# alibaba/TorchEasyRec

Measured on AMD Instinct MI355X. Metric: samples/sec DLRM-Criteo (examples/dlrm_criteo.config) training, batch 65536 global, higher is better.
Workload: dtype f32; 1 GPU; dlrm_criteo: 26 tables x dim 16 (204.2M rows, fp32), fused sparse adagrad + dense Adam, ids uniform; global_batch=65536, per_rank_batch=65536, parallelism=single GPU, all tables local (table-wise on one rank), row_layout=interleaved

## Files before the change

include/tzrec_hip.h:

```cpp
#ifndef TZREC_HIP_H_
#define TZREC_HIP_H_

#include <stddef.h>
#include <stdint.h>

#ifdef __cplusplus
extern "C" {
#endif

#define TZR_DT_F32 0
#define TZR_DT_F16 1

#define TZR_OK 0
#define TZR_ERR_INVALID (-1)
#define TZR_ERR_LAUNCH (-2)
#define TZR_ERR_WORKSPACE (-3)
#define TZR_ERR_UNSUPPORTED (-4)

#define TZR_MAX_DST 8
#define TZR_MAX_FEAT_DST 4

#define TZR_POOL_SUM 0
#define TZR_POOL_MEAN 1

// ... 442 lines not shown

#define TZR_DISTILL_MAX_PAIRS 8
#define TZR_DISTILL_MAX_W 1024
typedef struct TzrDistillLoss {
  int64_t B;
  int32_t P, C, cosine, pad_;
  int32_t W[TZR_DISTILL_MAX_PAIRS];
  uint64_t light[TZR_DISTILL_MAX_PAIRS];
  int64_t light_stride[TZR_DISTILL_MAX_PAIRS];
  uint64_t booster[TZR_DISTILL_MAX_PAIRS];
  int64_t booster_stride[TZR_DISTILL_MAX_PAIRS];
  uint64_t logits_light;
  uint64_t logits_booster;
  uint64_t w;
  uint64_t loss;
  uint64_t scale;
  uint64_t grad_sim[TZR_DISTILL_MAX_PAIRS];
  uint64_t grad_hint;
  uint64_t dlight[TZR_DISTILL_MAX_PAIRS];
  int64_t dlight_stride[TZR_DISTILL_MAX_PAIRS];
  uint64_t dlogits_light;
  uint64_t ws;
  uint64_t ws_bytes;
} TzrDistillLoss;
size_t tzr_distill_loss_workspace(const TzrDistillLoss* h_dst);
int tzr_distill_loss_fwd(const TzrDistillLoss* h_dst, void* stream);
int tzr_distill_loss_bwd(const TzrDistillLoss* h_dst, void* stream);

int tzr_skinny_linear_fwd(const float* d_x, int64_t x_stride, const float* d_w, int64_t w_stride, const float* d_bias,
                          int64_t B, int K, int n_out, float* d_y, int64_t y_stride, void* stream);
size_t tzr_skinny_linear_bwd_workspace(int64_t B, int K, int n_out);
int tzr_skinny_linear_bwd(const float* d_grad_y, int64_t grad_y_stride, const float* d_x, int64_t x_stride,
                          const float* d_w, int64_t w_stride, int64_t B, int K, int n_out, float* d_grad_x,
                          int64_t grad_x_stride, float* d_grad_wb, void* ws, size_t ws_bytes, void* stream);
int tzr_skinny_linear_bwd_parts(const float* d_grad_y, int64_t grad_y_stride, const float* d_x, int64_t x_stride,
                                const float* d_w, int64_t w_stride, int64_t B, int K, int n_out, float* d_grad_x,
                                int64_t grad_x_stride, void* ws, size_t ws_bytes, int* out_G, int* out_P, void* stream);

int tzr_linear_bwd_relu_supported(int K, int H);
size_t tzr_linear_bwd_relu_workspace(int64_t N, int H);
int tzr_linear_bwd_relu(const float* d_grad_in, int64_t grad_in_stride, const float* d_w, int64_t w_stride,
                        const float* d_y, int64_t y_stride, int64_t N, int K, int H, float* d_grad_out,
                        int64_t grad_out_stride, float* d_colsum, void* ws, size_t ws_bytes, void* stream);

int tzr_linear_rows_supported(int K, int H);
int tzr_linear_rows(const float* d_in, int64_t in_stride, const float* d_w, int64_t w_stride, int w_out_major,
                    const float* d_bias, const float* d_rowvec, int64_t rowvec_stride, const int32_t* d_row_index, int relu,
                    int64_t N, int K, int H, float* d_out, int64_t out_stride, void* stream);
int tzr_linear_rows_wgrad_supported(int H, int K);
size_t tzr_linear_rows_wgrad_workspace(int64_t N, int H, int K);
int tzr_linear_rows_wgrad(const float* d_g, int64_t g_stride, const float* d_x, int64_t x_stride, int64_t N, int H, int K,
                          float* d_dw, int64_t dw_stride, int accumulate, void* ws, size_t ws_bytes, void* stream);

#define TZR_ADAM_MAX_TENSORS 32
typedef struct TzrAdamTensor {
  uint64_t param, grad, exp_avg, exp_avg_sq;
  uint64_t state;
  int64_t numel;
} TzrAdamTensor;

int tzr_dense_adam(const TzrAdamTensor* h_tensors, int n_tensors, const float* d_lr, float lr,
                   float beta1, float beta2, float eps, float weight_decay, void* stream);

#define TZR_ADAM_FUSED_STATE 40
#define TZR_ADAM_SRC_TENSOR 0
#define TZR_ADAM_SRC_ROWS 1
#define TZR_ADAM_SRC_WGRAD 2
typedef struct TzrAdamSource {
  int32_t kind, G, P, col;
  uint64_t parts;
  uint64_t reserved;
} TzrAdamSource;
typedef struct TzrWgradParts { uint64_t opaque[24]; } TzrWgradParts;
int tzr_dense_adam_fused(const TzrAdamTensor* h_tensors, const TzrAdamSource* h_sources, int n_tensors,
                         const TzrWgradParts* h_wgrad, const float* d_lr, float lr, float beta1, float beta2, float eps,
                         float weight_decay, void* stream);
typedef struct TzrPackedW1 {
  uint64_t param;
  uint64_t fwd_packed, bwd_packed;
} TzrPackedW1;
int tzr_dense_adam_fused_w1(const TzrAdamTensor* h_tensors, const TzrAdamSource* h_sources, int n_tensors,
                            const TzrWgradParts* h_wgrad, const float* d_lr, float lr, float beta1, float beta2, float eps,
                            float weight_decay, const TzrPackedW1* h_w1, void* stream);
#define TZR_DENSE_OPT_SGD 0
#define TZR_DENSE_OPT_ADAGRAD 1
#define TZR_DENSE_OPT_ADAM 2
#define TZR_DENSE_OPT_ADAMW 3
#define TZR_DENSE_OPT_ADADELTA 4
#define TZR_DENSE_OPT_RMSPROP 5
#define TZR_DENSE_OPT_MAX_GROUPS 8
#define TZR_DENSE_OPT_NESTEROV 1
typedef struct TzrDenseOptTensor {
  uint64_t param, grad, state0, state1, state;
  int64_t numel;
  int32_t group, reserved;
} TzrDenseOptTensor;
typedef struct TzrDenseOptGroup {
  int32_t kind, flags;
  uint64_t d_lr;
  float lr, weight_decay, eps, hp0, hp1, reserved;
} TzrDenseOptGroup;
int tzr_dense_optim_fused(const TzrDenseOptTensor* h_tensors, const TzrAdamSource* h_sources, int n_tensors,
                          const TzrDenseOptGroup* h_groups, int n_groups, const TzrWgradParts* h_wgrad, void* stream);
int tzr_mlp2_bwd_parts(const float* d_dhb, int64_t dhb_stride, const float* d_hb, int64_t hb_stride, const float* d_ha,
                       int64_t ha_stride, const float* d_x, int64_t x_stride, int64_t B, int K0, int H1, int H2,
                       const float* d_Wb, void* ws, size_t ws_bytes, int* out_G, int* out_P, void* stream);
int tzr_dot_interaction_top_wgrad_parts(const float* d_dense, int64_t dense_stride, const float* d_sparse, int64_t sparse_stride,
                                        int F, int D, int64_t B, const float* d_g1, int64_t g1_stride, int H, const float* d_scale,
                                        void* d_ws, int64_t ws_bytes, TzrWgradParts* h_out, void* stream);


#define TZR_ZCH_EMPTY INT64_MAX
#define TZR_ZCH_TOMB (INT64_MAX - 1)

typedef struct TzrZchModule {
  int64_t* keys;
  int32_t* rows;
  int64_t* counts;
  int64_t* last_iter;
  int64_t capacity;
  int64_t zch_size;
  int64_t reserved[2];
} TzrZchModule;

int tzr_zch_remap(const TzrZchModule* d_modules, const int32_t* d_key_module, int n_keys,
                  const int64_t* d_values, const int64_t* d_offsets, int64_t B, int uniform_bag_len,
                  int64_t n_values, int64_t iter, int profile, int64_t* d_out_values,
                  int64_t* d_candidates, void* stream);

int tzr_zch_remap_ring(const TzrZchModule* d_modules, const int32_t* d_key_module, int n_keys,
                       const int64_t* d_values, int64_t B, int uniform_bag_len, int64_t n_values,
                       const int64_t* d_iter, int profile, int64_t* d_out_values, const int32_t* d_key_cand,
                       int n_cand_keys, int64_t* d_cand_ring, int64_t ring_slots, void* stream);

int tzr_zch_build(const TzrZchModule* h_module, const int64_t* d_ids, const int32_t* d_rows,
                  int64_t n, void* stream);

int tzr_zch_update(const TzrZchModule* h_module, const int64_t* d_old_ids, const int64_t* d_new_ids,
                   const int32_t* d_rows, int64_t n, void* stream);

int tzr_zch_select_hist(const TzrZchModule* h_module, const int64_t* d_row_ids, const int64_t* d_new_ids,
                        const int64_t* d_new_cnt, int64_t n_new, int64_t cur_iter, int policy,
                        double decay_exponent, int field, int shift, int bits, uint64_t t1, int t2,
                        uint64_t t3, uint64_t* d_bins, void* stream);
int tzr_zch_select_mark(const TzrZchModule* h_module, const int64_t* d_row_ids, const int64_t* d_new_ids,
                        const int64_t* d_new_cnt, int64_t n_new, int64_t cur_iter, int policy,
                        double decay_exponent, int drop_none, uint64_t t1, int t2, uint64_t t3,
                        uint8_t* d_row_kept, uint8_t* d_new_kept, void* stream);

size_t tzr_mlp_workspace(void);
int tzr_mlp2_fwd(const float* d_x, int64_t x_stride, int64_t B, int K0, const float* d_Wa, const float* d_ba, int H1,
                 const float* d_Wb, const float* d_bb, int H2, float* d_ha, int64_t ha_stride, float* d_hb,
                 int64_t hb_stride, void* stream);
int tzr_mlp2_bwd(const float* d_dhb, int64_t dhb_stride, const float* d_hb, int64_t hb_stride, const float* d_ha,
                 int64_t ha_stride, const float* d_x, int64_t x_stride, int64_t B, int K0, int H1, int H2,
                 const float* d_Wb, float* d_dWa, float* d_dba, float* d_dWb, float* d_dbb, void* ws, size_t ws_bytes,
                 void* stream);
int tzr_mlp_tail(const float* d_y1, int64_t y1_stride, const void* d_labels, int labels_itemsize, int labels_are_float,
                 int64_t B, int H1, const float* d_W2, const float* d_b2, int H2, const float* d_w3, const float* d_b3,
                 float* d_logits, float* d_g1, int64_t g1_stride, float* d_dW2, float* d_db2, float* d_dw3,
                 float* d_scalars, float* d_db1, void* ws, size_t ws_bytes, void* stream);


int tzr_jagged_to_padded_dense(const float* d_values, int64_t values_stride,
                               const int64_t* d_offsets, int64_t B, int64_t max_len, int dim,
                               float padding_value, float* d_out, void* stream);
int tzr_padded_dense_to_jagged(const float* d_dense, const int64_t* d_offsets, int64_t B,
                               int64_t max_len, int dim, float* d_values, int64_t values_stride,
                               void* stream);

int tzr_segment_reduce_fwd(const float* d_values, int64_t values_stride, const int64_t* d_offsets,
                           int64_t S, int dim, int mode, float* d_out, int64_t out_stride,
                           void* stream);
int tzr_segment_reduce_bwd(const float* d_grad_out, int64_t grad_out_stride,
                           const int64_t* d_offsets, int64_t S, int dim, int mode,
                           float* d_grad_values, int64_t grad_values_stride, void* stream);

int tzr_jagged_segment_ids(const int64_t* d_offsets, int64_t B, int64_t N, int32_t* d_seg, void* stream);
int tzr_din_assemble_fwd(const float* d_kv, int64_t kv_stride, const float* d_q, int64_t q_stride,
                         const int32_t* d_seg, int64_t B, int64_t N, int D, float* d_X, int64_t x_stride,
                         void* stream);
int tzr_din_assemble_bwd(const float* d_dX, int64_t x_stride, const float* d_kv, int64_t kv_stride,
                         const float* d_q, int64_t q_stride, const int32_t* d_seg, const int64_t* d_offsets,
                         int64_t B, int64_t N, int D, float* d_dkv, int64_t dkv_stride, int accumulate_dkv,
                         float* d_dq, int64_t dq_stride, void* stream);
int tzr_din_assemble2_fwd(const float* d_kv, int64_t kv_stride, const float* d_q, int64_t q_stride, const int32_t* d_seg, int64_t B,
                          int64_t N, int D, float* d_X, int64_t x_stride, void* stream);
int tzr_din_assemble2_bwd(const float* d_dX, int64_t x_stride, const float* d_kv, int64_t kv_stride, const float* d_q,
                          int64_t q_stride, const int32_t* d_seg, const int64_t* d_offsets, int64_t B, int64_t N, int D,
                          float* d_dkv, int64_t dkv_stride, int accumulate_dkv, const float* d_dq_add, int64_t dq_add_stride,
                          float* d_dq, int64_t dq_stride, void* stream);
int tzr_din_attn_fwd(const float* d_h, int64_t h_stride, int H, const float* d_w, const float* d_bias,
                     const float* d_kv, int64_t kv_stride, int D, const int64_t* d_offsets, int64_t B,
                     int64_t max_len, float* d_out, int64_t out_stride, float* d_p, void* stream);
int tzr_din_attn_bwd(const float* d_grad_out, int64_t grad_out_stride, const float* d_p, const float* d_kv,
                     int64_t kv_stride, int D, const int64_t* d_offsets, int64_t B, int64_t max_len, float* d_ds,
                     float* d_dkv, int64_t dkv_stride, void* stream);

int tzr_jagged_dot_attn_fwd(const float* d_kv, int64_t kv_stride, const float* d_q, int64_t q_stride, int D,
                            const int64_t* d_offsets, int64_t B, int64_t N, int64_t max_len, float* d_out,
                            int64_t out_stride, float* d_p, void* stream);
int tzr_jagged_dot_attn_bwd(const float* d_grad_out, int64_t grad_out_stride, const float* d_p, const float* d_kv,
                            int64_t kv_stride, const float* d_q, int64_t q_stride, int D, const int64_t* d_offsets,
                            int64_t B, int64_t N, int64_t max_len, float* d_dkv, int64_t dkv_stride, float* d_dq,
                            int64_t dq_stride, void* stream);
int tzr_jagged_pool_fwd(const float* d_kv, int64_t kv_stride, int D, const int64_t* d_offsets, int64_t B, int64_t N,
                        int64_t max_len, int mode, float* d_out, int64_t out_stride, void* stream);
int tzr_jagged_pool_bwd(const float* d_grad_out, int64_t grad_out_stride, int D, const int64_t* d_offsets, int64_t B,
                        int64_t N, int64_t max_len, int mode, float* d_dkv, int64_t dkv_stride, void* stream);

int tzr_cross_fwd(const float* d_x, int64_t x_stride, const float* const* h_w, const float* const* h_b, int L, int64_t B, int D,
                  float* d_y, int64_t y_stride, float* d_s, void* stream);
size_t tzr_cross_bwd_workspace(int64_t B, int D, int L);
int tzr_cross_bwd(const float* d_grad_y, int64_t gy_stride, const float* d_x, int64_t x_stride, const float* d_s,
                  const float* const* h_w, const float* const* h_b, int L, int64_t B, int D, float* d_dx, int64_t dx_stride,
                  float* d_dw, float* d_db, void* ws, size_t ws_size, void* stream);

int tzr_cross_v2_fwd(const float* d_x, int64_t x_stride, const float* const* h_u, const float* const* h_v, const float* const* h_c,
                     int L, int64_t B, int D, int R, float* d_y, int64_t y_stride, float* d_xs, float* d_t, void* stream);
size_t tzr_cross_v2_bwd_workspace(int64_t B, int D, int R, int L);
int tzr_cross_v2_bwd(const float* d_grad_y, int64_t gy_stride, const float* d_x, int64_t x_stride, const float* d_xs, const float* d_t,
                     const float* const* h_u, const float* const* h_v, const float* const* h_c, int L, int64_t B, int D, int R,
                     float* d_dx, int64_t dx_stride, float* d_du, float* d_dv, float* d_dc, void* ws, size_t ws_size, void* stream);

int tzr_ln_mask_fwd(const float* const* h_x, const int64_t* h_x_stride, const float* const* h_gamma, const float* const* h_beta,
                    const float* const* h_m, const int64_t* h_m_stride, float* const* h_out, const int64_t* h_out_stride, int n_out,
                    int shared_x, int relu, float eps, int64_t B, int D, float* d_stats, void* stream);
size_t tzr_ln_mask_bwd_workspace(int64_t B, int D, int n_out, int shared_x);
int tzr_ln_mask_bwd(const float* const* h_gout, const int64_t* h_gout_stride, const float* const* h_x, const int64_t* h_x_stride,
                    const float* const* h_gamma, const float* const* h_beta, const float* const* h_m, const int64_t* h_m_stride,
                    const float* d_stats, int n_out, int shared_x, int relu, int64_t B, int D, float* const* h_gx,
                    const int64_t* h_gx_stride, float* const* h_gm, const int64_t* h_gm_stride, float* d_dgamma, float* d_dbeta,
                    void* ws, size_t ws_size, void* stream);

int tzr_cin_fwd(const float* d_x, int64_t x_stride, const float* const* h_w, const float* const* h_c, const int* h_layers, int L,
                int64_t B, int F, int D, float* const* h_xs, float* d_y, int64_t y_stride, void* stream);
size_t tzr_cin_bwd_workspace(int64_t B, int F, int D, const int* h_layers, int L);
int tzr_cin_bwd(const float* d_grad_y, int64_t gy_stride, const float* d_x, int64_t x_stride, const float* const* h_w,
                const int* h_layers, int L, int64_t B, int F, int D, float* const* h_xs, float* d_gx, int64_t gx_stride,
                float* d_dwc, void* ws, size_t ws_size, void* stream);

int tzr_wukong_fm_fwd(const float* d_x, int64_t x_stride, const float* d_w, const float* d_gamma, const float* d_beta, float eps,
                      int64_t B, int F, int D, int k, float* d_out, int64_t out_stride, float* d_stats, void* stream);
size_t tzr_wukong_fm_bwd_workspace(int64_t B, int F, int D, int k);
int tzr_wukong_fm_bwd(const float* d_gout, int64_t gout_stride, const float* d_x, int64_t x_stride, const float* d_w,
                      const float* d_gamma, const float* d_stats, int64_t B, int F, int D, int k, float* d_gx, int64_t gx_stride,
                      float* d_dparams, void* ws, size_t ws_size, void* stream);
int tzr_wukong_mix_fwd(const float* d_x, int64_t x_stride, const float* d_fm, int64_t fm_stride, const float* d_wl, const float* d_wr,
                       const float* d_gamma, const float* d_beta, float eps, int64_t B, int F, int D, int Ff, int Fl, float* d_out,
                       int64_t out_stride, float* d_stats, void* stream);
size_t tzr_wukong_mix_bwd_workspace(int64_t B, int F, int D, int Ff, int Fl);
int tzr_wukong_mix_bwd(const float* d_gout, int64_t gout_stride, const float* d_x, int64_t x_stride, const float* d_fm, int64_t fm_stride,
                       const float* d_wl, const float* d_wr, const float* d_gamma, const float* d_stats, int64_t B, int F, int D, int Ff,
                       int Fl, float* d_gx, int64_t gx_stride, float* d_gfm, int64_t gfm_stride, float* d_dparams, void* ws,
                       size_t ws_size, void* stream);

int tzr_comm_available(const char* librccl_path);
int tzr_comm_version(const char* librccl_path);
int tzr_comm_unique_id(const char* librccl_path, void* out, size_t out_bytes);
int tzr_comm_create(const char* librccl_path, const void* unique_id, size_t id_bytes, int world, int rank,
                    void** out_comm);
int tzr_comm_destroy(void* comm);
int tzr_comm_all_to_all(void* comm, const void* d_send, void* d_recv, int64_t bytes_per_peer, void* stream);
int tzr_comm_all_reduce(void* comm, float* d_buf, int64_t count, int average, void* stream);
int tzr_step_create(void** out_program);
int tzr_step_destroy(void* program);
int tzr_step_add_graph(void* program, void* graph_exec );
int tzr_step_add_all_to_all(void* program, void* comm, const void* d_send, void* d_recv, int64_t bytes_per_peer, int sync);
int tzr_step_add_all_reduce(void* program, void* comm, float* d_buf, int64_t count, int average, int sync);
int tzr_step_add_wait(void* program, int collective_op);
int tzr_step_num_ops(void* program);
int tzr_step_run(void* program, void* stream);


int tzr_quantize_rows_q8f16(const void* d_w, int w_dtype, int64_t w_stride, int64_t rows, int dim,
                            uint8_t* d_out, int64_t* d_first_bad, void* stream);
int tzr_dequantize_rows_q8f16(const uint8_t* d_rows, int64_t rows, int dim, float* d_out,
                              int64_t out_stride, void* stream);


typedef struct TzrDeltaSeg {
  uint32_t* bitmap;
  int64_t rows;
  int32_t key;
  int32_t reserved;
} TzrDeltaSeg;

int tzr_delta_mark(const TzrDeltaSeg* d_segs, int n_segs, const int64_t* d_ids,
                   const int64_t* d_key_offsets, int64_t key_stride, int64_t uniform_len,
                   int64_t n_ids, int64_t* d_oob, void* stream);
size_t tzr_delta_collect_workspace(int64_t rows);
int tzr_delta_count(const uint32_t* d_bitmap, int64_t rows, int64_t* d_total, void* ws,
                    size_t ws_bytes, void* stream);
int tzr_delta_collect(uint32_t* d_bitmap, int64_t rows, int64_t id_base, int clear,
                      int64_t* d_out_ids, int64_t capacity, void* ws, size_t ws_bytes, void* stream);

int tzr_tune(const char* name, int value);


int tzr_dot_interaction_fwd(const float* d_dense, int64_t dense_stride, const float* d_sparse,
                            int64_t sparse_stride, int F, int D, int64_t B, float* d_out,
                            int64_t out_stride, int cat_dense, int cat_sparse, void* stream);
int tzr_dot_interaction_bwd(const float* d_dense, int64_t dense_stride, const float* d_sparse,
                            int64_t sparse_stride, int F, int D, int64_t B,
                            const float* d_grad_out, int64_t grad_out_stride, int cat_dense,
                            int cat_sparse, float* d_grad_dense, int64_t grad_dense_stride,
// ... 65 lines not shown
```

torcheasyrec_amd/_lib.py:

```python
from __future__ import annotations

import ctypes as C
import os
from typing import Optional

import numpy as np
import torch

_HERE = os.path.dirname(os.path.abspath(__file__))
LIB_PATH = os.path.join(_HERE, "libtzrec_hip.so")

TZR_OK = 0
TZR_ERR_INVALID, TZR_ERR_UNSUPPORTED = -1, -4
TZR_MAX_DST = 8
TZR_MAX_FEAT_DST = 4
METRIC_MAX_THRESHOLDS = 4096
POOL_SUM, POOL_MEAN = 0, 1
DT_F32, DT_F16 = 0, 1
FWD_MIXED_DTYPE = 1
OPT_SGD, OPT_ADAGRAD, OPT_ROWWISE_ADAGRAD, OPT_ACCUMULATE, OPT_ADAM = 0, 1, 2, 3, 4
OPT_PARTIAL_ROWWISE_ADAM, OPT_LAMB, OPT_PARTIAL_ROWWISE_LAMB, OPT_LARS_SGD = 5, 6, 7, 8
OPT_ADADELTA, OPT_RMSPROP = 9, 10
ABI_VERSION = 15
WD_NONE, WD_L2, WD_DECOUPLE = 0, 1, 2
# ... 128 lines not shown
        ("ws", C.c_uint64), ("ws_bytes", C.c_uint64),
    ]


assert C.sizeof(TzrCapsule) == 192
LABEL_ATTN_MAX_D, LABEL_ATTN_MAX_K = 256, 8
AMM_MAX_D = 256


class TzrAmmLoss(C.Structure):
    _fields_ = [
        ("B", C.c_int64), ("M", C.c_int64), ("D", C.c_int32), ("cosine", C.c_int32), ("c_u", C.c_float), ("c_i", C.c_float),
        ("ua", C.c_uint64), ("ua_stride", C.c_int64), ("ia", C.c_uint64), ("ia_stride", C.c_int64),
        ("ue", C.c_uint64), ("ue_stride", C.c_int64), ("ie", C.c_uint64), ("ie_stride", C.c_int64), ("w", C.c_uint64),
        ("loss", C.c_uint64), ("rows", C.c_uint64), ("scale", C.c_uint64), ("grad_u", C.c_uint64), ("grad_i", C.c_uint64),
        ("dua", C.c_uint64), ("dua_stride", C.c_int64), ("dia", C.c_uint64), ("dia_stride", C.c_int64),
        ("ws", C.c_uint64), ("ws_bytes", C.c_uint64),
    ]


assert C.sizeof(TzrAmmLoss) == 192
DISTILL_MAX_PAIRS, DISTILL_MAX_W, DISTILL_MAX_C = 8, 1024, 64


class TzrDistillLoss(C.Structure):
    _fields_ = [
        ("B", C.c_int64), ("P", C.c_int32), ("C", C.c_int32), ("cosine", C.c_int32), ("pad_", C.c_int32),
        ("W", C.c_int32 * DISTILL_MAX_PAIRS),
        ("light", C.c_uint64 * DISTILL_MAX_PAIRS), ("light_stride", C.c_int64 * DISTILL_MAX_PAIRS),
        ("booster", C.c_uint64 * DISTILL_MAX_PAIRS), ("booster_stride", C.c_int64 * DISTILL_MAX_PAIRS),
        ("logits_light", C.c_uint64), ("logits_booster", C.c_uint64), ("w", C.c_uint64), ("loss", C.c_uint64), ("scale", C.c_uint64),
        ("grad_sim", C.c_uint64 * DISTILL_MAX_PAIRS), ("grad_hint", C.c_uint64),
        ("dlight", C.c_uint64 * DISTILL_MAX_PAIRS), ("dlight_stride", C.c_int64 * DISTILL_MAX_PAIRS), ("dlogits_light", C.c_uint64),
        ("ws", C.c_uint64), ("ws_bytes", C.c_uint64),
    ]


assert C.sizeof(TzrDistillLoss) == 576


class TzrSparseOptim(C.Structure):
    _fields_ = [
        ("kind", C.c_int32),
        ("weight_decay_mode", C.c_int32),
        ("d_lr", C.c_uint64),
        ("eps", C.c_float),
        ("weight_decay", C.c_float),
        ("max_gradient", C.c_float),
        ("gradient_clipping", C.c_int32),
        ("beta1", C.c_float),
        ("beta2", C.c_float),
        ("d_adam", C.c_uint64),
    ]


class TzrAdamTensor(C.Structure):
    _fields_ = [("param", C.c_uint64), ("grad", C.c_uint64), ("exp_avg", C.c_uint64), ("exp_avg_sq", C.c_uint64),
                ("state", C.c_uint64), ("numel", C.c_int64)]


class TzrAdamSource(C.Structure):
    _fields_ = [("kind", C.c_int32), ("G", C.c_int32), ("P", C.c_int32), ("col", C.c_int32), ("parts", C.c_uint64), ("reserved", C.c_uint64)]


class TzrWgradParts(C.Structure):
    _fields_ = [("opaque", C.c_uint64 * 24)]


class TzrPackedW1(C.Structure):
    _fields_ = [("param", C.c_uint64), ("fwd_packed", C.c_uint64), ("bwd_packed", C.c_uint64)]


ADAM_SRC_TENSOR, ADAM_SRC_ROWS, ADAM_SRC_WGRAD = 0, 1, 2


class TzrDenseOptTensor(C.Structure):
    _fields_ = [("param", C.c_uint64), ("grad", C.c_uint64), ("state0", C.c_uint64), ("state1", C.c_uint64), ("state", C.c_uint64),
                ("numel", C.c_int64), ("group", C.c_int32), ("reserved", C.c_int32)]


class TzrDenseOptGroup(C.Structure):
    _fields_ = [("kind", C.c_int32), ("flags", C.c_int32), ("d_lr", C.c_uint64), ("lr", C.c_float), ("weight_decay", C.c_float),
                ("eps", C.c_float), ("hp0", C.c_float), ("hp1", C.c_float), ("reserved", C.c_float)]


DENSE_OPT_MAX_GROUPS = 8
DENSE_OPT_NESTEROV = 1


class TzrZchModule(C.Structure):
    _fields_ = [("keys", C.c_uint64), ("rows", C.c_uint64), ("counts", C.c_uint64), ("last_iter", C.c_uint64),
                ("capacity", C.c_int64), ("zch_size", C.c_int64), ("reserved", C.c_int64 * 2)]


DELTA_SEG_DT = np.dtype([("bitmap", "<u8"), ("rows", "<i8"), ("key", "<i4"), ("reserved", "<i4")])
assert DELTA_SEG_DT.itemsize == 24

ZCH_EMPTY = (1 << 63) - 1


class TzrError(RuntimeError):
    pass


_lib: Optional[C.CDLL] = None
_backend: Optional[str] = None

_vp, _i64, _i32, _sz = C.c_void_p, C.c_int64, C.c_int, C.c_size_t

_SIGNATURES = {
    "tzr_backend": (C.c_char_p, []),
    "tzr_abi_version": (_i32, []),
    "tzr_tune": (_i32, [C.c_char_p, _i32]),
    "tzr_lengths_to_offsets_workspace": (_sz, [_i64]),
    "tzr_lengths_to_offsets": (_i32, [_vp, _i32, _i64, _vp, _vp, _sz, _vp]),
    "tzr_bounds_check": (_i32, [_vp, _vp, _i32, _vp, _vp, _i64, _i32, _vp, _vp]),
    "tzr_kjt_permute_workspace": (_sz, [_i64, _i64]),
    "tzr_kjt_permute": (_i32, [_vp, _i32, _i32, _i64, _vp, _i32, _vp, _vp, _vp, _vp, _vp, _vp, _vp,
                               _i64, _vp, _sz, _vp]),
    "tzr_block_bucketize_workspace": (_sz, [_i64, _i64, _i32]),
    "tzr_block_bucketize": (_i32, [_vp, _vp, _i32, _i64, _i32, _vp, _vp, _vp, _i64, _vp, _i32, _vp, _vp,
                                   _vp, _vp, _vp, _sz, _vp]),
    "tzr_exchange_bucketize_workspace": (_sz, [_i32, _i64, _i32]),
    "tzr_exchange_bucketize": (_i32, [_vp, _i32, _vp, _vp, _i64, _i32, _i32, _vp, _vp, _vp, _vp, _vp, _sz, _vp]),
    "tzr_exchange_message_stride": (_i64, [_i32, _i64]),
    "tzr_exchange_bucketize_capped": (_i32, [_vp, _i32, _vp, _vp, _i64, _i32, _i32, _vp, _i64, _vp, _vp, _vp, _sz, _vp]),
    "tzr_exchange_pad": (_i32, [_vp, _i32, _i32, _i64, _vp, _vp, _i64, _vp, _vp, _vp]),
    "tzr_exchange_owner_segments": (_i32, [_vp, _i32, _i32, _i64, _vp, _vp, _vp]),
    "tzr_pooled_fwd": (_i32, [_vp, _vp, _i32, _vp, _i32, _vp, _vp, _vp, _i64, C.POINTER(TzrDst),
                              _i32, _i32, _vp]),
    "tzr_pooled_fwd_ex": (_i32, [_vp, _vp, _i32, _vp, _i32, _vp, _vp, _vp, _i64, C.POINTER(TzrDst),
                                 _i32, _i32, _i32, _vp]),
    "tzr_pooled_bwd_workspace": (_sz, [_i64, _i64, _i32, _i32, _i64, _i32]),
    "tzr_pooled_bwd_plan_view": (_i32, [_i64, _i64, _i32, _i32, _i32, _vp]),
    "tzr_pooled_bwd_plan": (_i32, [_vp, _i32, _vp, _i32, _i32, _i64, _i32, _vp, _vp, _i64, _i64, _i64,
                                   _i32, _vp, _sz, _vp]),
    "tzr_pooled_bwd_direct_supported": (_i32, [_i64, _i32, _i32, _i32, _i32]),
    "tzr_pooled_bwd_direct_workspace": (_sz, [_i64, _i32, _i32]),
    "tzr_pooled_bwd_direct": (_i32, [_vp, _i32, _vp, _i32, _i64, _i32, _vp, _vp, _vp, _i64, _i64, _i64, _i32, _i32,
                                     C.POINTER(TzrDst), _i32, C.POINTER(TzrSparseOptim), _vp, _sz, _vp]),
    "tzr_sparse_adam_tick": (_i32, [_vp, C.c_float, C.c_float, _vp]),
    "tzr_dense_rows_update": (_i32, [_vp, _i32, _vp, _i64, _vp, _i32, C.POINTER(TzrSparseOptim), _vp]),
    "tzr_dense_rows_update_clear": (_i32, [_vp, _i32, _vp, _i64, _vp, _i32, C.POINTER(TzrSparseOptim), _vp]),
    "tzr_rows_gather": (_i32, [_vp, _vp, _vp, _i32, _vp, _i64, _vp, _i64, _i32, _vp]),
    "tzr_lookup_grads": (_i32, [_vp, _i32, _vp, _vp, _i64, _i32, _vp, C.POINTER(TzrDst), _i32, _vp,
                                _i64, _i32, _vp]),
    "tzr_pooled_bwd_apply": (_i32, [_vp, _vp, _i32, _i32, _i32, _vp, _vp, _i64, _i64, _i64, _i32, _i32,
                                    C.POINTER(TzrDst), _i32, C.POINTER(TzrSparseOptim), _vp, _sz,
                                    _vp]),
    "tzr_bwd_cells_geometry": (_i32, [_vp, _i32, _vp, _i32, _i64, _i32, _vp, _sz, C.POINTER(C.c_int64)]),
    "tzr_pooled_bwd_cells_plan": (_i32, [_vp, _i32, _vp, _i32, _i32, _vp, _i64, _i64, _vp, _vp, _vp, _sz, _vp]),
    "tzr_pooled_fwd_cells_plan_supported": (_i32, [_i32, _i64]),
    "tzr_pooled_fwd_cells_plan": (_i32, [_vp, _vp, _i32, _vp, _i32, _vp, _i32, _vp, _i32, _vp, _i32, _i32, _vp, _i64, _i64, _vp, _vp, _vp, _sz, _vp]),
    "tzr_pooled_bwd_cells_apply": (_i32, [_vp, _vp, _i32, _i32, _i32, _vp, _i64, _i64, _i32, C.POINTER(TzrDst), _i32,
                                          C.POINTER(TzrSparseOptim), _vp, _vp, _vp, _sz, _vp]),
    "tzr_dense_adam_fused": (_i32, [C.POINTER(TzrAdamTensor), C.POINTER(TzrAdamSource), _i32, C.POINTER(TzrWgradParts), _vp, C.c_float,
                                    C.c_float, C.c_float, C.c_float, C.c_float, _vp]),
    "tzr_dense_adam_fused_w1": (_i32, [C.POINTER(TzrAdamTensor), C.POINTER(TzrAdamSource), _i32, C.POINTER(TzrWgradParts), _vp, C.c_float,
                                       C.c_float, C.c_float, C.c_float, C.c_float, C.POINTER(TzrPackedW1), _vp]),
    "tzr_dense_optim_fused": (_i32, [C.POINTER(TzrDenseOptTensor), C.POINTER(TzrAdamSource), _i32, C.POINTER(TzrDenseOptGroup), _i32,
                                     C.POINTER(TzrWgradParts), _vp]),
    "tzr_mlp2_bwd_parts": (_i32, [_vp, _i64, _vp, _i64, _vp, _i64, _vp, _i64, _i64, _i32, _i32, _i32, _vp, _vp, _sz, C.POINTER(C.c_int),
                                  C.POINTER(C.c_int), _vp]),
    "tzr_dot_interaction_top_wgrad_parts": (_i32, [_vp, _i64, _vp, _i64, _i32, _i32, _i64, _vp, _i64, _i32, _vp, _vp, _i64,
                                                   C.POINTER(TzrWgradParts), _vp]),
    "tzr_dot_interaction_fwd": (_i32, [_vp, _i64, _vp, _i64, _i32, _i32, _i64, _vp, _i64, _i32,
                                       _i32, _vp]),
    "tzr_dot_interaction_bwd": (_i32, [_vp, _i64, _vp, _i64, _i32, _i32, _i64, _vp, _i64, _i32,
                                       _i32, _vp, _i64, _vp, _i64, _vp]),
    "tzr_dot_interaction_top_supported": (_i32, [_i32, _i32, _i32, _i32]),
    "tzr_dot_interaction_top_fwd": (_i32, [_vp, _i64, _vp, _i64, _i32, _i32, _i64, _vp, _i64, _vp, _i32, _i32, _vp, _i64,
                                           _vp, _i64, _vp]),
    "tzr_dot_interaction_top_bwd": (_i32, [_vp, _i64, _vp, _i64, _i32, _i32, _i64, _vp, _i64, _i32, _vp, _i64, _vp, _vp,
                                           _i64, _vp, _i64, _vp]),
    "tzr_ia_top_packed_floats": (_i32, []),
    "tzr_ia_top_pack_w1": (_i32, [_vp, _i64, _i32, _vp, _vp, _vp]),
    "tzr_dot_interaction_top_fwd_packed": (_i32, [_vp, _i64, _vp, _i64, _i32, _i32, _i64, _vp, _i64, _vp, _i32, _i32, _vp, _i64,
                                                  _vp, _i64, _vp, _vp]),
    "tzr_dot_interaction_top_bwd_packed": (_i32, [_vp, _i64, _vp, _i64, _i32, _i32, _i64, _vp, _i64, _i32, _vp, _i64, _vp, _vp,
                                                  _i64, _vp, _i64, _vp, _vp]),
    "tzr_dot_interaction_top_fwd_mlp2": (_i32, [_vp, _i64, _i64, _i32, _vp, _vp, _i32, _vp, _vp, _i32, _vp, _i64, _vp, _i64,
                                                _vp, _i64, _vp, _i64, _i32, _i32, _vp, _i64, _vp, _i32, _i32, _vp, _i64,
                                                _vp, _i64, _vp, _vp]),
    "tzr_dot_interaction_top_bwd_wgrad_parts": (_i32, [_vp, _i64, _vp, _i64, _i32, _i32, _i64, _vp, _i64, _i32, _vp, _i64, _vp, _vp,
                                                       _i64, _vp, _i64, _vp, _vp, _i64, C.POINTER(TzrWgradParts), _vp]),
    "tzr_dot_interaction_top_wgrad_workspace": (_i64, [_i32, _i32, _i32, _i32]),
    "tzr_dot_interaction_top_wgrad": (_i32, [_vp, _i64, _vp, _i64, _i32, _i32, _i64, _vp, _i64, _i32, _vp, _vp, _i64, _vp,
                                             _i64, _vp]),
    "tzr_jagged_to_padded_dense": (_i32, [_vp, _i64, _vp, _i64, _i64, _i32, C.c_float, _vp, _vp]),
    "tzr_padded_dense_to_jagged": (_i32, [_vp, _vp, _i64, _i64, _i32, _vp, _i64, _vp]),
    "tzr_quantize_rows_q8f16": (_i32, [_vp, _i32, _i64, _i64, _i32, _vp, _vp, _vp]),
    "tzr_dequantize_rows_q8f16": (_i32, [_vp, _i64, _i32, _vp, _i64, _vp]),
    "tzr_segment_reduce_fwd": (_i32, [_vp, _i64, _vp, _i64, _i32, _i32, _vp, _i64, _vp]),
    "tzr_segment_reduce_bwd": (_i32, [_vp, _i64, _vp, _i64, _i32, _i32, _vp, _i64, _vp]),
    "tzr_jagged_segment_ids": (_i32, [_vp, _i64, _i64, _vp, _vp]),
    "tzr_din_assemble_fwd": (_i32, [_vp, _i64, _vp, _i64, _vp, _i64, _i64, _i32, _vp, _i64, _vp]),
    "tzr_din_assemble_bwd": (_i32, [_vp, _i64, _vp, _i64, _vp, _i64, _vp, _vp, _i64, _i64, _i32, _vp, _i64, _i32, _vp, _i64, _vp]),
    "tzr_din_assemble2_fwd": (_i32, [_vp, _i64, _vp, _i64, _vp, _i64, _i64, _i32, _vp, _i64, _vp]),
    "tzr_din_assemble2_bwd": (_i32, [_vp, _i64, _vp, _i64, _vp, _i64, _vp, _vp, _i64, _i64, _i32, _vp, _i64, _i32, _vp, _i64, _vp, _i64, _vp]),
    "tzr_din_attn_fwd": (_i32, [_vp, _i64, _i32, _vp, _vp, _vp, _i64, _i32, _vp, _i64, _i64, _vp, _i64, _vp, _vp]),
    "tzr_din_attn_bwd": (_i32, [_vp, _i64, _vp, _vp, _i64, _i32, _vp, _i64, _i64, _vp, _vp, _i64, _vp]),
    "tzr_jagged_dot_attn_fwd": (_i32, [_vp, _i64, _vp, _i64, _i32, _vp, _i64, _i64, _i64, _vp, _i64, _vp, _vp]),
    "tzr_jagged_dot_attn_bwd": (_i32, [_vp, _i64, _vp, _vp, _i64, _vp, _i64, _i32, _vp, _i64, _i64, _i64, _vp, _i64, _vp, _i64, _vp]),
    "tzr_jagged_pool_fwd": (_i32, [_vp, _i64, _i32, _vp, _i64, _i64, _i64, _i32, _vp, _i64, _vp]),
    "tzr_jagged_pool_bwd": (_i32, [_vp, _i64, _i32, _vp, _i64, _i64, _i64, _i32, _vp, _i64, _vp]),
    "tzr_cross_fwd": (_i32, [_vp, _i64, _vp, _vp, _i32, _i64, _i32, _vp, _i64, _vp, _vp]),
    "tzr_cross_bwd_workspace": (_sz, [_i64, _i32, _i32]),
    "tzr_cross_bwd": (_i32, [_vp, _i64, _vp, _i64, _vp, _vp, _vp, _i32, _i64, _i32, _vp, _i64, _vp, _vp, _vp, _sz, _vp]),
    "tzr_cross_v2_fwd": (_i32, [_vp, _i64, _vp, _vp, _vp, _i32, _i64, _i32, _i32, _vp, _i64, _vp, _vp, _vp]),
    "tzr_cross_v2_bwd_workspace": (_sz, [_i64, _i32, _i32, _i32]),
    "tzr_cross_v2_bwd": (_i32, [_vp, _i64, _vp, _i64, _vp, _vp, _vp, _vp, _vp, _i32, _i64, _i32, _i32, _vp, _i64, _vp, _vp, _vp, _vp, _sz,
                                _vp]),
    "tzr_cin_fwd": (_i32, [_vp, _i64, _vp, _vp, _vp, _i32, _i64, _i32, _i32, _vp, _vp, _i64, _vp]),
    "tzr_cin_bwd_workspace": (_sz, [_i64, _i32, _i32, _vp, _i32]),
    "tzr_cin_bwd": (_i32, [_vp, _i64, _vp, _i64, _vp, _vp, _i32, _i64, _i32, _i32, _vp, _vp, _i64, _vp, _vp, _sz, _vp]),
    "tzr_ln_mask_fwd": (_i32, [_vp, _vp, _vp, _vp, _vp, _vp, _vp, _vp, _i32, _i32, _i32, C.c_float, _i64, _i32, _vp, _vp]),
    "tzr_ln_mask_bwd_workspace": (_sz, [_i64, _i32, _i32, _i32]),
    "tzr_ln_mask_bwd": (_i32, [_vp, _vp, _vp, _vp, _vp, _vp, _vp, _vp, _vp, _i32, _i32, _i32, _i64, _i32, _vp, _vp, _vp, _vp, _vp, _vp,
                               _vp, _sz, _vp]),
    "tzr_wukong_fm_fwd": (_i32, [_vp, _i64, _vp, _vp, _vp, C.c_float, _i64, _i32, _i32, _i32, _vp, _i64, _vp, _vp]),
    "tzr_wukong_fm_bwd_workspace": (_sz, [_i64, _i32, _i32, _i32]),
    "tzr_wukong_fm_bwd": (_i32, [_vp, _i64, _vp, _i64, _vp, _vp, _vp, _i64, _i32, _i32, _i32, _vp, _i64, _vp, _vp, _sz, _vp]),
    "tzr_wukong_mix_fwd": (_i32, [_vp, _i64, _vp, _i64, _vp, _vp, _vp, _vp, C.c_float, _i64, _i32, _i32, _i32, _i32, _vp, _i64, _vp, _vp]),
    "tzr_wukong_mix_bwd_workspace": (_sz, [_i64, _i32, _i32, _i32, _i32]),
    "tzr_wukong_mix_bwd": (_i32, [_vp, _i64, _vp, _i64, _vp, _i64, _vp, _vp, _vp, _vp, _i64, _i32, _i32, _i32, _i32, _vp, _i64, _vp, _i64,
                                  _vp, _vp, _sz, _vp]),
    "tzr_comm_available": (_i32, [C.c_char_p]),
    "tzr_comm_version": (_i32, [C.c_char_p]),
    "tzr_comm_unique_id": (_i32, [C.c_char_p, _vp, _sz]),
    "tzr_comm_create": (_i32, [C.c_char_p, _vp, _sz, _i32, _i32, C.POINTER(C.c_void_p)]),
    "tzr_comm_destroy": (_i32, [_vp]),
    "tzr_comm_all_to_all": (_i32, [_vp, _vp, _vp, _i64, _vp]),
    "tzr_comm_all_reduce": (_i32, [_vp, _vp, _i64, _i32, _vp]),
    "tzr_step_create": (_i32, [C.POINTER(C.c_void_p)]),
    "tzr_step_destroy": (_i32, [_vp]),
    "tzr_step_add_graph": (_i32, [_vp, _vp]),
    "tzr_step_add_all_to_all": (_i32, [_vp, _vp, _vp, _vp, _i64, _i32]),
    "tzr_step_add_all_reduce": (_i32, [_vp, _vp, _vp, _i64, _i32, _i32]),
    "tzr_step_add_wait": (_i32, [_vp, _i32]),
    "tzr_step_num_ops": (_i32, [_vp]),
    "tzr_step_run": (_i32, [_vp, _vp]),
    "tzr_bce_logits_workspace": (_sz, [_i64]),
    "tzr_bce_logits": (_i32, [_vp, _vp, _i32, _i32, _vp, _i64, _vp, _vp, _vp, _sz, _vp]),
    "tzr_loss_pointwise_workspace": (_sz, [_i64]),
    "tzr_loss_pointwise": (_i32, [_i32, C.c_float, C.c_float, _vp, _vp, _i32, _i32, _vp, _vp, _i32, _i32, C.c_float, C.c_float,
                                  C.c_float, _i64, _vp, _vp, _vp, _vp, _sz, _vp]),
    "tzr_softmax_ce_workspace": (_sz, [_i64, _i32]),
    "tzr_softmax_ce": (_i32, [_vp, _i64, _i32, _vp, _i32, _i32, C.c_float, _vp, _vp, _i32, _i32, C.c_float, C.c_float, C.c_float,
                              _i64, _vp, _vp, _vp, _vp, _vp, _sz, _vp]),
    "tzr_jrc_loss_workspace": (_sz, [_i64]),
    "tzr_jrc_loss": (_i32, [_vp, _vp, _i32, _i32, _vp, _vp, C.c_float, _vp, _vp, _i32, _i32, C.c_float, C.c_float, C.c_float,
                            _i64, _vp, _vp, _vp, _vp, _sz, _vp]),
    "tzr_relu_bwd_colsum_workspace": (_sz, [_i64, _i32]),
    "tzr_relu_bwd_colsum": (_i32, [_vp, _i64, _vp, _i64, _i64, _i32, _vp, _i64, _vp, _vp, _sz, _vp]),
    "tzr_relu_bwd_colsum_parts": (_i32, [_vp, _i64, _vp, _i64, _i64, _i32, _vp, _i64, _vp, _sz, _vp, _vp]),
    "tzr_head_bwd_workspace": (_sz, [_i64, _i32]),
    "tzr_head_bwd": (_i32, [_vp, _i64, _vp, _i64, _vp, _i64, _i32, _vp, _i64, _vp, _vp, _sz, _vp]),
    "tzr_head_bwd_relu_workspace": (_sz, [_i64, _i32]),
    "tzr_head_bwd_relu": (_i32, [_vp, _i64, _vp, _i64, _vp, _i64, _i32, _vp, _i64, _vp, _vp, _sz, _vp]),
    "tzr_moe_mix_fwd": (_i32, [_vp, _vp]),
    "tzr_moe_mix_bwd": (_i32, [_vp, _vp]),
    "tzr_cgc_mix_fwd": (_i32, [_vp, _vp]),
    "tzr_cgc_mix_bwd": (_i32, [_vp, _vp]),
    "tzr_gate_scale_fwd": (_i32, [_vp, _vp]),
    "tzr_gate_scale_bwd_workspace": (_sz, [_i64, _i32, _i32]),
    "tzr_gate_scale_bwd": (_i32, [_vp, _vp]),
    "tzr_relation_chain_fwd": (_i32, [_vp, _vp]),
    "tzr_relation_chain_bwd_workspace": (_sz, [_vp]),
    "tzr_relation_chain_bwd": (_i32, [_vp, _vp]),
    "tzr_match_softmax_workspace": (_sz, [_vp]),
    "tzr_match_softmax_fwd": (_i32, [_vp, _vp]),
    "tzr_match_softmax_bwd": (_i32, [_vp, _vp]),
    "tzr_capsule_workspace": (_sz, [_vp]),
    "tzr_capsule_fwd": (_i32, [_vp, _vp]),
    "tzr_capsule_bwd": (_i32, [_vp, _vp]),
    "tzr_label_attn_fwd": (_i32, [_vp, _i64, _vp, _i64, _vp, _i64, _i32, _i32, C.c_float, _vp, _i64, _vp, _vp]),
    "tzr_label_attn_bwd": (_i32, [_vp, _i64, _vp, _i64, _vp, _i64, _vp, _vp, _i64, _i32, _i32, C.c_float, _vp, _i64, _vp, _i64, _vp]),
    "tzr_amm_loss_workspace": (_sz, [_vp]),
    "tzr_amm_loss_fwd": (_i32, [_vp, _vp]),
    "tzr_amm_loss_bwd": (_i32, [_vp, _vp]),
    "tzr_distill_loss_workspace": (_sz, [_vp]),
    "tzr_distill_loss_fwd": (_i32, [_vp, _vp]),
    "tzr_distill_loss_bwd": (_i32, [_vp, _vp]),
    "tzr_skinny_linear_fwd": (_i32, [_vp, _i64, _vp, _i64, _vp, _i64, _i32, _i32, _vp, _i64, _vp]),
    "tzr_skinny_linear_bwd_workspace": (_sz, [_i64, _i32, _i32]),
    "tzr_skinny_linear_bwd": (_i32, [_vp, _i64, _vp, _i64, _vp, _i64, _i64, _i32, _i32, _vp, _i64, _vp, _vp, _sz, _vp]),
    "tzr_skinny_linear_bwd_parts": (_i32, [_vp, _i64, _vp, _i64, _vp, _i64, _i64, _i32, _i32, _vp, _i64, _vp, _sz, _vp, _vp, _vp]),
    "tzr_linear_rows_supported": (_i32, [_i32, _i32]),
    "tzr_linear_rows": (_i32, [_vp, _i64, _vp, _i64, _i32, _vp, _vp, _i64, _vp, _i32, _i64, _i32, _i32, _vp, _i64, _vp]),
    "tzr_linear_rows_wgrad_supported": (_i32, [_i32, _i32]),
    "tzr_linear_rows_wgrad_workspace": (_sz, [_i64, _i32, _i32]),
    "tzr_linear_rows_wgrad": (_i32, [_vp, _i64, _vp, _i64, _i64, _i32, _i32, _vp, _i64, _i32, _vp, _sz, _vp]),
    "tzr_linear_bwd_relu_supported": (_i32, [_i32, _i32]),
    "tzr_linear_bwd_relu_workspace": (_sz, [_i64, _i32]),
    "tzr_linear_bwd_relu": (_i32, [_vp, _i64, _vp, _i64, _vp, _i64, _i64, _i32, _i32, _vp, _i64, _vp, _vp, _sz, _vp]),
    "tzr_mlp_workspace": (_sz, []),
    "tzr_mlp2_fwd": (_i32, [_vp, _i64, _i64, _i32, _vp, _vp, _i32, _vp, _vp, _i32, _vp, _i64, _vp, _i64, _vp]),
    "tzr_mlp2_bwd": (_i32, [_vp, _i64, _vp, _i64, _vp, _i64, _vp, _i64, _i64, _i32, _i32, _i32, _vp, _vp, _vp, _vp, _vp,
                            _vp, _sz, _vp]),
    "tzr_mlp_tail": (_i32, [_vp, _i64, _vp, _i32, _i32, _i64, _i32, _vp, _vp, _i32, _vp, _vp, _vp, _vp, _i64, _vp, _vp, _vp,
                            _vp, _vp, _vp, _sz, _vp]),
    "tzr_dense_adam": (_i32, [_vp, _i32, _vp, C.c_float, C.c_float, C.c_float, C.c_float, C.c_float, _vp]),
    "tzr_zch_remap": (_i32, [_vp, _vp, _i32, _vp, _vp, _i64, _i32, _i64, _i64, _i32, _vp, _vp, _vp]),
    "tzr_zch_remap_ring": (_i32, [_vp, _vp, _i32, _vp, _i64, _i32, _i64, _vp, _i32, _vp, _vp, _i32, _vp, _i64, _vp]),
    "tzr_zch_build": (_i32, [_vp, _vp, _vp, _i64, _vp]),
    "tzr_zch_update": (_i32, [_vp, _vp, _vp, _vp, _i64, _vp]),
# ... 210 lines not shown
```

torcheasyrec_amd/csrc/mlp2_fwd16_body.h:

```cpp
#pragma once
#include "tzr_common.h"

#define MM_TS 16
#define MT_H1 64
#define MT_P1 (MT_H1 + 4)

typedef float mm_f32x4 __attribute__((ext_vector_type(4)));

#define MB_H1 64
#define MB_H2 16
#define MB_PX 20

__device__ __forceinline__ void mb_fwd16_tiles(
    const float* __restrict__ x, int64_t xs, int64_t B, int K0, const float* __restrict__ Wa, const float* __restrict__ ba,
    const float* __restrict__ Wb, const float* __restrict__ bb, float* __restrict__ ha, int64_t has, float* __restrict__ hb,
    int64_t hbs, float* T1, int lane, int64_t t0, int64_t step) {
  const int r = lane & 15, q = lane >> 4;
  float Wfa[4][4], Wfb[16], bav[4];
#pragma unroll
  for (int hbk = 0; hbk < 4; ++hbk) {
#pragma unroll
    for (int ks = 0; ks < 4; ++ks) {
      const int k = 4 * ks + q;
      const float w = Wa[(16 * hbk + r) * K0 + (k < K0 ? k : 0)];
      Wfa[hbk][ks] = k < K0 ? w : 0.f;
    }
    bav[hbk] = ba ? ba[16 * hbk + r] : 0.f;
  }
#pragma unroll
  for (int i = 0; i < 4; ++i) {
    const float4 v = tzr_ld4(Wb + r * MB_H1 + 16 * q + 4 * i);
    Wfb[4 * i] = v.x; Wfb[4 * i + 1] = v.y; Wfb[4 * i + 2] = v.z; Wfb[4 * i + 3] = v.w;
  }
  const float bbv = bb ? bb[r] : 0.f;
  const int64_t tiles = (B + MM_TS - 1) / MM_TS;
  for (int64_t t = t0; t < tiles; t += step) {
    const int64_t b0 = t * MM_TS;
    float xa[4];
    {
      const int64_t b = b0 + r < B ? b0 + r : B - 1;
#pragma unroll
      for (int ks = 0; ks < 4; ++ks) {
        const int k = 4 * ks + q;
        const float v = x[b * xs + (k < K0 ? k : 0)];
        xa[ks] = (k < K0 && b0 + r < B) ? v : 0.f;
      }
    }
    mm_f32x4 acc[4];
#pragma unroll
    for (int hbk = 0; hbk < 4; ++hbk) acc[hbk] = mm_f32x4{0.f, 0.f, 0.f, 0.f};
#pragma unroll
    for (int ks = 0; ks < 4; ++ks)
#pragma unroll
      for (int hbk = 0; hbk < 4; ++hbk) acc[hbk] = __builtin_amdgcn_mfma_f32_16x16x4f32(xa[ks], Wfa[hbk][ks], acc[hbk], 0, 0, 0);
#pragma unroll
    for (int hbk = 0; hbk < 4; ++hbk)
#pragma unroll
      for (int j = 0; j < 4; ++j) T1[(4 * q + j) * MT_P1 + 16 * hbk + r] = fmaxf(acc[hbk][j] + bav[hbk], 0.f);
    __builtin_amdgcn_wave_barrier();
    mm_f32x4 acc2 = {0.f, 0.f, 0.f, 0.f};
#pragma unroll
    for (int i = 0; i < 4; ++i) {
      const int e = lane + TZR_WAVE * i, row = e >> 4, c4 = e & 15;
      if (b0 + row < B) tzr_st4(ha + (b0 + row) * has + 4 * c4, tzr_ld4(T1 + row * MT_P1 + 4 * c4));
      const float4 av = tzr_ld4(T1 + r * MT_P1 + 16 * q + 4 * i);
      acc2 = __builtin_amdgcn_mfma_f32_16x16x4f32(av.x, Wfb[4 * i], acc2, 0, 0, 0);
      acc2 = __builtin_amdgcn_mfma_f32_16x16x4f32(av.y, Wfb[4 * i + 1], acc2, 0, 0, 0);
      acc2 = __builtin_amdgcn_mfma_f32_16x16x4f32(av.z, Wfb[4 * i + 2], acc2, 0, 0, 0);
      acc2 = __builtin_amdgcn_mfma_f32_16x16x4f32(av.w, Wfb[4 * i + 3], acc2, 0, 0, 0);
    }
#pragma unroll
    for (int j = 0; j < 4; ++j)
      if (b0 + 4 * q + j < B) hb[(b0 + 4 * q + j) * hbs + r] = fmaxf(acc2[j] + bbv, 0.f);
    __builtin_amdgcn_wave_barrier();
  }
}

static inline bool mb_fwd16_fits(int K0, int H1, int H2, const float* d_Wb, const float* d_ha, int64_t ha_stride) {
  return K0 > 0 && K0 <= 16 && H1 == MB_H1 && H2 == MB_H2 && !(ha_stride & 3) && !(reinterpret_cast<uintptr_t>(d_ha) & 15) &&
         !(reinterpret_cast<uintptr_t>(d_Wb) & 15);
}
```

torcheasyrec_amd/csrc/pooled_bwd_cells.hip:

```cpp
#include <tzr_gfx950.h>

#include "pooled_fwd_u1.h"

#include <algorithm>
#include <cstring>
#include <vector>

#ifdef IT_PROF
#define CELLS_PROF_WGS 4096
__device__ uint64_t g_cells_prof[CELLS_PROF_WGS * 16];
#define CELLS_MARK(i) do { if (blockIdx.x < CELLS_PROF_WGS && threadIdx.x == 0) g_cells_prof[blockIdx.x * 16 + (i)] = wall_clock64(); } while (0)
#define CELLS_NOTE(i, v) do { if (blockIdx.x < CELLS_PROF_WGS && threadIdx.x == 0) g_cells_prof[blockIdx.x * 16 + (i)] = (uint64_t)(v); } while (0)
#define BWD_PROF_MARK(i) do { if ((i) == 2 && blockIdx.x < CELLS_PROF_WGS && (threadIdx.x & (TZR_WAVE - 1)) == 0) \
    g_cells_prof[blockIdx.x * 16 + 4 + threadIdx.x / TZR_WAVE] = wall_clock64(); } while (0)
extern "C" int tzr_cells_prof_dump(uint64_t* h_out, int n_wg) {
  (void)hipDeviceSynchronize();
  return hipMemcpyFromSymbol(h_out, HIP_SYMBOL(g_cells_prof), (size_t)std::min(n_wg, CELLS_PROF_WGS) * 16 * sizeof(uint64_t)) == hipSuccess ? 0 : -1;
}
#else
#define CELLS_MARK(i)
#define CELLS_NOTE(i, v)
#endif

#include "pooled_bwd_apply.h"
#include "pooled_bwd_cells.h"
#include "pooled_bwd_sort.h"

namespace {

struct HostGeo {
  BwdCellsGeo g;
  std::vector<BwdCellChunk> chunks;
  std::vector<BwdCellUnit> units;
  std::vector<uint32_t> fstart;
  std::vector<int32_t> fkey, fbo;
  std::vector<uint16_t> bnd;
};

inline int64_t align256(int64_t x) { return (x + 255) & ~int64_t(255); }

inline void bucket_params_host(int64_t rows, int* nb, uint64_t* mult) {
  if (rows <= BWD_NB) {
    *nb = rows < 1 ? 1 : (int)rows;
    *mult = 1ull << 32;
  } else {
    *nb = BWD_NB;
    *mult = ((uint64_t)BWD_NB << 32) / (uint64_t)rows;
  }
}

int build_geometry(const TzrTable* tabs, int T, const TzrFeature* feats, int F, int64_t B, int max_dim, HostGeo& H) {
  if (T <= 0 || F <= 0 || B <= 0 || max_dim <= 0 || max_dim > BWD_MAXDIM || (max_dim & 3)) return TZR_ERR_INVALID;
  H.fstart.assign(F + 1, 0);
  H.fkey.assign(F, 0);
  H.fbo.assign(F, 0);
  std::vector<int> seen(F, 0);
  for (int f = 0; f < F; ++f) {
    const TzrFeature& ft = feats[f];
    if (ft.order < 0 || ft.order >= F || seen[ft.order]) return TZR_ERR_INVALID;
    seen[ft.order] = 1;
    H.fstart[ft.order] = ft.table < 0 ? 0u : (uint32_t)B;
    H.fkey[ft.order] = ft.key;
    H.fbo[ft.order] = f;
  }
  {
    uint64_t run = 0;
    for (int o = 0; o < F; ++o) {
      const uint32_t n = H.fstart[o];
      H.fstart[o] = (uint32_t)run;
      run += n;
    }
    if (run >= (1ull << 32)) return TZR_ERR_UNSUPPORTED;
    H.fstart[F] = (uint32_t)run;
  }
  const int64_t N = H.fstart[F];
  if (N == 0) return TZR_ERR_UNSUPPORTED;
  const int ch = bwd_pick_ch(N);
  int64_t n_chunks = 0;
  std::vector<int64_t> cfirst(T + 1, 0), nt(T, 0);
  for (int t = 0; t < T; ++t) {
    const TzrTable& tb = tabs[t];
    if (tb.n_feats < 0 || (tb.n_feats > 0 && (tb.first_order < 0 || tb.first_order + tb.n_feats > F))) return TZR_ERR_INVALID;
    const int64_t n = tb.n_feats > 0 ? (int64_t)H.fstart[tb.first_order + tb.n_feats] - (int64_t)H.fstart[tb.first_order] : 0;
    const int64_t C = (n + ch - 1) / ch;
    if (C > BWD_CELLS_MAXC) return TZR_ERR_UNSUPPORTED;
    if (n > 0 && (tb.rows <= 0 || tb.rows > (1LL << 32))) return TZR_ERR_UNSUPPORTED;
    nt[t] = n;
    cfirst[t] = n_chunks;
    n_chunks += C;
  }
  cfirst[T] = n_chunks;
  if (n_chunks > bwd_max_chunks(N, T, ch)) return TZR_ERR_UNSUPPORTED;

  const int64_t target = BWD_CELLS_TARGET;
  std::vector<int64_t> U(T, 0);
  for (int t = 0; t < T; ++t) {
    if (nt[t] == 0 || tabs[t].rows <= BWD_NB) continue;
    const int64_t per = (target * BWD_NB) / nt[t];
    if (per < 1) return TZR_ERR_UNSUPPORTED;
    U[t] = (BWD_NB + per - 1) / per;
  }

  int64_t n_recs = 0, n_counters = 0;
  for (int t = 0; t < T; ++t) {
    const TzrTable& tb = tabs[t];
    const int64_t C = cfirst[t + 1] - cfirst[t];
    if (C == 0) continue;
    const int64_t ts = H.fstart[tb.first_order], te = H.fstart[tb.first_order + tb.n_feats];
    const int64_t n = te - ts;
    int nb;
    uint64_t mult;
    bucket_params_host(tb.rows, &nb, &mult);
    const int64_t fbase = tb.n_feats == 1 ? (int64_t)H.fkey[tb.first_order] * B : -1;
    const int32_t bnd0 = (int32_t)H.bnd.size();
    BwdCellUnit u;
    std::memset(&u, 0, sizeof(u));
    u.tb = tb;
    u.feat = H.fbo[tb.first_order];
    u.ts = (uint32_t)ts;
    u.rec = u.rec0 = u.counter = -1;
    u.crel0 = 0;
    u.ncell = (int32_t)C;
    if (tb.rows > BWD_NB) {
      const int64_t Ut = U[t];
      for (int64_t j = 0; j <= Ut; ++j) H.bnd.push_back((uint16_t)(j * nb / Ut));
      for (int64_t j = 0; j < Ut; ++j) {
        u.b0 = (int32_t)(j * nb / Ut);
        u.i0 = bnd0 + (int32_t)j;
        u.i1 = u.i0 + 1;
        H.units.push_back(u);
      }
    } else {
      const int64_t e = (n + tb.rows - 1) / tb.rows;
      if (e > target) {
        for (int64_t r = 0; r <= tb.rows; ++r) H.bnd.push_back((uint16_t)r);
        const int64_t m = std::max<int64_t>(1, (target * tb.rows * C) / n);
        const int64_t K = std::min<int64_t>(C, (C + m - 1) / m);
        for (int64_t r = 0; r < tb.rows; ++r) {
          for (int64_t k = 0; k < K; ++k) {
            u.crel0 = (int32_t)(k * C / K);
            u.ncell = (int32_t)((k + 1) * C / K) - u.crel0;
            u.b0 = (int32_t)r;
            u.nrows = 0;
            u.i0 = bnd0 + (int32_t)r;
            u.i1 = u.i0 + 1;
            u.split = K > 1 ? (int32_t)K : 0;
            u.rec = K > 1 ? (int32_t)(n_recs + k) : -1;
            u.rec0 = K > 1 ? (int32_t)n_recs : -1;
            u.counter = K > 1 ? (int32_t)n_counters : -1;
            H.units.push_back(u);
          }
          if (K > 1) {
            n_recs += K;
            n_counters += 1;
          }
        }
      } else {
        const int64_t rpu = std::max<int64_t>(1, (target * tb.rows) / n);
        int32_t g = 0;
        for (int64_t r = 0; r < tb.rows; r += rpu, ++g) {
          H.bnd.push_back((uint16_t)r);
          u.b0 = (int32_t)r;
          u.i0 = bnd0 + g;
          u.i1 = u.i0 + 1;
          H.units.push_back(u);
        }
        H.bnd.push_back((uint16_t)tb.rows);
      }
    }
    const int32_t nbnd = (int32_t)H.bnd.size() - bnd0;
    for (int64_t c = 0; c < C; ++c) {
      BwdCellChunk cd;
      std::memset(&cd, 0, sizeof(cd));
      cd.t = t;
      cd.nb = nb;
      cd.s = ts + c * ch;
// ... 17 lines not shown
  g.max_dim = max_dim;
  g.ch = ch;
  g.n_positions = N;
  g.n_bnd = (int64_t)H.bnd.size();
  if (g.n_bnd * BWD_CELLS_MAXC * 2 > bwd_max_chunks(N, T, ch) * (int64_t)BWD_NB * 4) return TZR_ERR_UNSUPPORTED;
  int64_t off = align256(sizeof(BwdCellsGeo));
  g.off_chunks = off;
  off = align256(off + n_chunks * (int64_t)sizeof(BwdCellChunk));
  g.off_units = off;
  off = align256(off + g.n_units * (int64_t)sizeof(BwdCellUnit));
  g.off_fstart = off;
  off = align256(off + (F + 1) * 4);
  g.off_fkey = off;
  off = align256(off + F * 4);
  g.off_fbo = off;
  off = align256(off + F * 4);
  g.off_bnd = off;
  off = align256(off + g.n_bnd * 2);
  g.off_recs = off;
  off = align256(off + std::max<int64_t>(1, n_recs) * max_dim * 4);
  g.off_rcount = off;
  off = align256(off + std::max<int64_t>(1, n_recs) * 4);
  g.off_counters = off;
  off = align256(off + std::max<int64_t>(1, n_counters) * 4);
  g.off_overflow = off;
  off = align256(off + 4 * (BWD_CELLS_OVF_LIST + 2 * g.n_units));
  g.bytes = off;
  return TZR_OK;
}

}

extern "C" int tzr_bwd_cells_geometry(const TzrTable* h_tables, int n_tables, const TzrFeature* h_feats, int n_feats, int64_t B,
                                      int max_dim, void* h_out, size_t out_bytes, int64_t* out_info8) {
  if (!h_tables || !h_feats || !out_info8) return TZR_ERR_INVALID;
  HostGeo H;
  const int rc = build_geometry(h_tables, n_tables, h_feats, n_feats, B, max_dim, H);
  if (rc != TZR_OK) return rc;
  const BwdCellsGeo& g = H.g;
  out_info8[0] = g.bytes;
  out_info8[1] = g.n_chunks;
  out_info8[2] = g.n_units;
  out_info8[3] = g.n_positions;
  out_info8[4] = g.ch;
  out_info8[5] = g.n_recs;
  out_info8[6] = g.off_overflow;
  out_info8[7] = 0;
  if (!h_out) return TZR_OK;
  if ((int64_t)out_bytes < g.bytes) return TZR_ERR_WORKSPACE;
  char* b = static_cast<char*>(h_out);
  std::memset(b, 0, (size_t)g.bytes);
  std::memcpy(b, &g, sizeof(g));
  std::memcpy(b + g.off_chunks, H.chunks.data(), H.chunks.size() * sizeof(BwdCellChunk));
  std::memcpy(b + g.off_units, H.units.data(), H.units.size() * sizeof(BwdCellUnit));
  std::memcpy(b + g.off_fstart, H.fstart.data(), H.fstart.size() * 4);
  std::memcpy(b + g.off_fkey, H.fkey.data(), H.fkey.size() * 4);
  std::memcpy(b + g.off_fbo, H.fbo.data(), H.fbo.size() * 4);
  std::memcpy(b + g.off_bnd, H.bnd.data(), H.bnd.size() * 2);
  return TZR_OK;
}

struct BwdPartLds {
  BwdRankLds<BWD_NB> L;
  uint2 stage[BWD_CH];
};

__device__ __forceinline__ void bwd_cells_partition_body(const BwdCellsView& V, const TzrTable* __restrict__ tables, const BwdSrcArgs& A,
                                                         uint2* __restrict__ slab, uint16_t* __restrict__ bnd, int ch, unsigned chunk,
                                                         BwdPartLds& PL) {
  auto& L = PL.L;
  auto& stage = PL.stage;
  const BwdCellChunk cd = V.chunks[chunk];
  if (cd.t < 0) return;
  const int n = (int)(cd.e - cd.s);
  const int lane = threadIdx.x & (TZR_WAVE - 1);
  const int wv = threadIdx.x / TZR_WAVE;
  constexpr int kRounds = BWD_CH / BWD_THREADS;
  const int pw = bwd_wave_span(n);
  const int rounds = pw / TZR_WAVE;
  uint32_t kreg[kRounds], sreg[kRounds], dig[kRounds], dest[kRounds];
  uint32_t vmask = 0;
  if (cd.fbase >= 0) {
#pragma unroll
    for (int r = 0; r < kRounds; ++r) {
      const int lp = wv * pw + r * TZR_WAVE + lane;
      const int lc = lp < n ? lp : n - 1;
      const int64_t i = cd.fbase + (cd.s - cd.ts) + lc;
      int64_t id = A.values[i];
      if ((uint64_t)id >= (uint64_t)cd.rows) id = 0;
      kreg[r] = (uint32_t)id;
      sreg[r] = (uint32_t)i;
      dig[r] = bwd_bucket(kreg[r], cd.mult);
      vmask |= (r < rounds && lp < n) ? 1u << r : 0u;
    }
  } else {
    const TzrTable tb = tables[cd.t];
    BwdGeo G;
    G.fstart = V.fstart;
    G.fkey = V.fkey;
    G.tchunk = nullptr;
#pragma unroll
    for (int r = 0; r < kRounds; ++r) {
      const int lp = wv * pw + r * TZR_WAVE + lane;
      kreg[r] = sreg[r] = dig[r] = 0u;
      if (r < rounds && lp < n) {
        vmask |= 1u << r;
        int64_t kk;
        bwd_elem0(G, tb, A, cd.s + lp, &kreg[r], &sreg[r], &kk);
        dig[r] = bwd_bucket(kreg[r], cd.mult);
      }
    }
  }
  bwd_rank_tile<BWD_NB, kRounds>(dig, vmask, rounds, bwd_bits((uint32_t)cd.nb - 1u), L, dest);
#pragma unroll
  for (int r = 0; r < kRounds; ++r)
    if ((vmask >> r) & 1u) stage[dest[r]] = make_uint2(kreg[r], sreg[r]);
  {
    const int col = (int)((cd.s - cd.ts) / (cd.e > cd.s ? (int64_t)ch : 1));
    for (int i = threadIdx.x; i < cd.nbnd; i += BWD_THREADS)
      bnd[(size_t)(cd.bnd0 + i) * BWD_CELLS_MAXC + col] = L.lstart[V.bnd_bucket[cd.bnd0 + i]];
  }
  __syncthreads();
  uint2* out = slab + cd.s;
  for (int i = threadIdx.x; i < n; i += BWD_THREADS) out[i] = stage[i];
}

__global__ __launch_bounds__(BWD_THREADS) void tzr_bwd_cells_partition_kernel(
    BwdCellsView V, const TzrTable* __restrict__ tables, BwdSrcArgs A, uint2* __restrict__ slab, uint16_t* __restrict__ bnd, int ch) {
  __shared__ BwdPartLds PL;
  bwd_cells_partition_body(V, tables, A, slab, bnd, ch, blockIdx.x, PL);
}

static_assert(FWD_THREADS == BWD_THREADS, "one workgroup size for both kinds");
struct FwdPlanArgs {
  const TzrTable* ftables;
  const TzrFeature* ffeats;
  const TzrSlot* slots;
  const int64_t* values;
  int64_t B;
  int32_t n_slots, tile_b;
  uint32_t n_fwd, n_part;
  const TzrTable* btables;
  uint2* slab;
  uint16_t* bnd;
  int32_t ch;
};

#ifndef FWD_PLAN_WAVES
#define FWD_PLAN_WAVES 7
#endif
#ifndef FWD_PLAN_UNROLL
#define FWD_PLAN_UNROLL 4
#endif
union FwdPlanLds {
  Fwd1Lds f;
  BwdPartLds p;
};

__global__ __launch_bounds__(BWD_THREADS) TZR_WAVES_PER_EU(FWD_PLAN_WAVES) void tzr_pooled_fwd_u1_cells_plan_kernel(FwdPlanArgs a, FwdDsts dsts,
                                                                                                          BwdCellsView V, BwdSrcArgs A) {
  __shared__ FwdPlanLds S;
  const uint32_t i = blockIdx.x;
  const bool part = i >= a.n_fwd;
  const uint32_t idx = part ? i - a.n_fwd : i;
  if (part)
    bwd_cells_partition_body(V, a.btables, A, a.slab, a.bnd, a.ch, idx, S.p);
  else
    fwd_u1_body<FWD_PLAN_UNROLL>(a.ftables, a.ffeats, a.slots, a.n_slots, a.values, a.B, a.tile_b, dsts, idx, 0u, S.f);
}

union BwdCellsLds {
  BwdSortLds S;
  BwdUnitLds U;
};

#define BWD_CELLS_SM 264
#define BWD_CELLS_SM_WORDS (2 * BWD_WAVES + BWD_WAVES * TZR_WAVE)
static_assert(BWD_CELLS_SM >= BWD_THREADS + 1, "sm behind the histogram of bwd_cells_next_piece");
static_assert(offsetof(BwdSortLds, pre) == offsetof(BwdSortLds, gstart) + sizeof(unsigned) * (BWD_NB + 1),
              "pre / hb directly behind gstart");
static_assert(offsetof(BwdSortLds, gstart) + sizeof(unsigned) * (BWD_CELLS_SM + BWD_CELLS_SM_WORDS) <= offsetof(BwdSortLds, pk),
              "sm fits in gstart + pre / hb");
static_assert(sizeof(BwdRankLds<BWD_NB>) >= 4096, "red: 4 KB in S.L");

__device__ __forceinline__ uint2 bwd_cells_elem(const uint2* __restrict__ slab, const uint32_t* cpre, const uint32_t* cbase,
                                                int ncell, uint32_t i) {
  int lo = 0;
#pragma unroll
  for (int step = BWD_CELLS_MAXC / 2; step > 0; step >>= 1) {
    const int cand = lo + step;
    if (cand < ncell && cpre[cand] <= i) lo = cand;
  }
  return slab[cbase[lo] + (i - cpre[lo])];
}

template <int FAM>
__device__ __forceinline__ void bwd_cells_combine(const BwdCellUnit& u, const BwdCellsView& V, const BwdOpt& opt, float lr,
                                                  int max_dim, float4 sum, uint32_t count, int lane) {
  const int lg = u.tb.dim >> 2;
  if (lane < lg) bwd_publish4(V.recs + (size_t)u.rec * max_dim + 4 * lane, sum);
  if (lane == 0) tzr_publish_u32(V.rcount + u.rec, count);
  tzr_drain_stores();
  int last = 0;
  if (lane == 0) last = tzr_arrive(V.counters + u.counter) == (uint32_t)(u.split - 1) ? 1 : 0;
  last = __shfl(last, 0, TZR_WAVE);
  if (!last) return;
  if (lane == 0) tzr_publish_u32(V.counters + u.counter, 0u);
  const int gw = TZR_WAVE / lg;
  const int gi = lane / lg, c = lane - gi * lg;
  float4 tot = tzr_zero4();
  uint32_t cnt = 0;
  for (int k0 = 0; k0 < u.split; k0 += gw) {
    const int k = k0 + gi;
    const bool in = gi < gw && k < u.split;
    float4 v = tzr_zero4();
    uint32_t cn = 0;
    if (in) {
      v = bwd_consume4(V.recs + (size_t)(u.rec0 + k) * max_dim + 4 * c);
      cn = tzr_consume_u32(V.rcount + u.rec0 + k);
    }
    const int nk = min(gw, u.split - k0);
    for (int g = 0; g < nk; ++g) {
      const float4 piece = bwd_shfl4(v, g * lg + (lane < lg ? lane : 0));
      if (lane < lg) tot = tzr_add4(tot, piece);
      cnt += (uint32_t)__shfl((int)cn, g * lg, TZR_WAVE);
    }
  }
  if (cnt) bwd_apply_row_wave<FAM>(u.tb, opt, lr, (uint32_t)u.b0, tot, lane);
}

template <bool FAST>
__device__ __forceinline__ float4 bwd_cells_stream_row(
    const BwdCellUnit& u, const BwdCellsView& V, const uint2* __restrict__ slab, const uint32_t* cpre, const uint32_t* cbase,
    int ncell, int n, uint32_t row, const TzrFeature* __restrict__ feats, const float* __restrict__ weights, int64_t B,
    int grad_mode, const TzrDst* sG, float* red, uint32_t* sm, uint32_t* count_out) {
  constexpr int UF = 4;
  const TzrTable& tb = u.tb;
  const int lane = threadIdx.x & (TZR_WAVE - 1);
  const int wv = threadIdx.x / TZR_WAVE;
  const int lg = tb.dim >> 2, gw = TZR_WAVE / lg;
  const int gi = lane / lg, c = lane - gi * lg;
  const bool lane_on = gi < gw;
  const int groups = gw * BWD_WAVES, q = wv * gw + gi;
  const bool single = tb.n_feats == 1;
  const BwdSrc one = bwd_resolve(feats + V.feat_by_order[tb.first_order], sG);
  const float* const fgp = grad_mode == 1 ? reinterpret_cast<const float*>(sG[0].ptr) : one.gp0;
  const int64_t fgs = grad_mode == 1 ? sG[0].stride : one.gs0;
  const uint32_t fkb = grad_mode == 0 ? (uint32_t)feats[V.feat_by_order[tb.first_order]].key * (uint32_t)B : 0u;
  float4 acc = tzr_zero4();
  uint32_t cnt = 0;
  const int trips = (n + groups * UF - 1) / (groups * UF);
  uint2 e[UF];
#pragma unroll
  for (int k = 0; k < UF; ++k) {
    const int i = k * groups + q;
    e[k] = bwd_cells_elem(slab, cpre, cbase, ncell, (uint32_t)(i < n ? i : n - 1));
  }
  for (int j = 0; j < trips; ++j) {
    float4 g[UF];
#pragma unroll
    for (int k = 0; k < UF; ++k) {
      if constexpr (FAST) g[k] = tzr_ldg4(fgp + (int64_t)(e[k].y - fkb) * fgs + 4 * c);
      else g[k] = bwd_lookup_grad(feats, tb, V.feat_by_order, sG, one, single, grad_mode, nullptr, weights, nullptr, B, 1, e[k].y, c);
    }
    uint2 en[UF];
#pragma unroll
    for (int k = 0; k < UF; ++k) {
      const int i = ((j + 1) * UF + k) * groups + q;
      en[k] = bwd_cells_elem(slab, cpre, cbase, ncell, (uint32_t)(i < n ? i : n - 1));
    }
#pragma unroll
    for (int k = 0; k < UF; ++k) {
      const int i = (j * UF + k) * groups + q;
      if (lane_on && i < n && (row == BWD_SENT || e[k].x == row)) {
        acc = tzr_add4(acc, g[k]);
        cnt += 1;
      }
      e[k] = en[k];
    }
  }
  __syncthreads();
  if (lane_on) {
    float* r = red + (size_t)(q * lg + c) * 4;
    r[0] = acc.x; r[1] = acc.y; r[2] = acc.z; r[3] = acc.w;
    if (c == 0) sm[2 * BWD_WAVES + q] = cnt;
  }
  __syncthreads();
  float4 tot = tzr_zero4();
  uint32_t ct = 0;
  if (wv == 0) {
    for (int g2 = 0; g2 < groups; ++g2) {
      if (lane < lg) {
        const float* r = red + (size_t)(g2 * lg + lane) * 4;
        tot = tzr_add4(tot, make_float4(r[0], r[1], r[2], r[3]));
      }
      ct += sm[2 * BWD_WAVES + g2];
    }
  }
  *count_out = ct;
  return tot;
}

template <int FAM>
__device__ __forceinline__ int bwd_cells_next_piece(
    const BwdCellUnit& u, const BwdCellsView& V, const uint2* __restrict__ slab, const uint32_t* cpre, const uint32_t* cbase,
    int ncell, int n, uint32_t& cur, uint32_t khi, const TzrFeature* __restrict__ feats, const float* __restrict__ weights, int64_t B,
    int grad_mode, const BwdOpt& opt, float lr, BwdCellsLds& L, const TzrDst* sG) {
  const TzrTable& tb = u.tb;
  const int lane = threadIdx.x & (TZR_WAVE - 1);
  const int wv = threadIdx.x / TZR_WAVE;
  float* const red = reinterpret_cast<float*>(&L.S.L);
  uint32_t* const hist = L.S.gstart;
  uint32_t* const sm = L.S.gstart + BWD_CELLS_SM;
  constexpr int SB = BWD_THREADS;
  while (cur < khi) {
// ... 203 lines not shown
      const int rounds = pw / TZR_WAVE;
      uint32_t kreg[kRounds], sreg[kRounds];
      uint32_t vmask = 0, kmin = 0xFFFFFFFFu, kmax = 0u;
#pragma unroll
      for (int r = 0; r < kRounds; ++r) {
        const int lp = wv * pw + r * TZR_WAVE + lane;
        const bool in = r < rounds && lp < np;
        kreg[r] = in ? L.S.pk[lp] : 0u;
        sreg[r] = in ? L.S.ps[lp] : 0u;
        if (in) {
          vmask |= 1u << r;
          kmin = min(kmin, kreg[r]);
          kmax = max(kmax, kreg[r]);
        }
      }
      __syncthreads();
      bwd_cells_sort_reduce<FAM, 0, 1, kRounds>(u, V, kreg, sreg, vmask, kmin, kmax, np, ft_dst, feats, weights, B, grad_mode, opt, lr,
                                                 max_dim, L, sG);
      __syncthreads();
    }
  }
  if (threadIdx.x == 0 && tzr_arrive(ov + BWD_CELLS_OVF_DONE) == (uint32_t)BWD_CELLS_WORKERS - 1u) {
    if (len) atomicAdd(ov + BWD_CELLS_OVF_TOTAL, len);
    tzr_publish_u32(ov + BWD_CELLS_OVF_LEN, 0u);
    tzr_publish_u32(ov + BWD_CELLS_OVF_CURSOR, 0u);
    tzr_publish_u32(ov + BWD_CELLS_OVF_DONE, 0u);
    tzr_publish_u32(ov + BWD_CELLS_OVF_EPOCH, tzr_consume_u32(ov + BWD_CELLS_OVF_EPOCH) + 1u);
  }
}

template <int FAM, int FK, int NT>
__device__ __forceinline__ void bwd_cells_apply_body(
    BwdCellsView V, int n_units, const TzrFeature* __restrict__ feats, const float* __restrict__ weights, int64_t B, int grad_mode,
    const BwdGrads& G, const BwdOpt& opt, int max_dim, const uint2* __restrict__ slab, const uint16_t* __restrict__ bnd, int ch) {
  __shared__ BwdCellsLds L;
  __shared__ TzrDst sG[TZR_MAX_DST];
  __shared__ uint32_t xcell[2 * BWD_CELLS_MAXC + 8];
  if (threadIdx.x == 0) {
#pragma unroll
    for (int i = 0; i < TZR_MAX_DST; ++i) sG[i] = G.d[i];
  }
  if ((int)blockIdx.x >= n_units) {
    __syncthreads();
#ifndef CELLS_NO_WORKER
    bwd_cells_worker<FAM>(V, n_units, feats, weights, B, grad_mode, opt, max_dim, slab, bnd, ch, L, sG, xcell);
#endif
    return;
  }
  CELLS_MARK(0);
#ifndef CELLS_NO_PRIO
  tzr_prio_by_slot(blockIdx.x);
  if ((blockIdx.x >> 8) >= 4u) __builtin_amdgcn_s_sleep(64);
#endif
  const BwdCellUnit u = V.units[blockIdx.x];
  const uint32_t epoch = V.overflow[BWD_CELLS_OVF_EPOCH];
  const int lane = threadIdx.x & (TZR_WAVE - 1);
  const int wv = threadIdx.x / TZR_WAVE;
  const int ncell = u.ncell;
  const int ft_dst = feats[u.feat].n_dst;
  uint32_t* const cpre = xcell;
  uint32_t* const cbase = xcell + BWD_CELLS_MAXC + 8;
  const float lr = *opt.lr;
  const int n = bwd_cells_bounds(u, u.i0, u.i1, bnd, ch, cpre, cbase, L.S.wtot);
  CELLS_MARK(1);
  CELLS_NOTE(9, n);
  if (threadIdx.x == 0) {
    if (n > BWD_UMAX) {
      const uint32_t at = atomicAdd(V.overflow + BWD_CELLS_OVF_LEN, 1u);
      tzr_publish_u32(V.overflow + BWD_CELLS_OVF_LIST + at, (uint32_t)blockIdx.x);
      tzr_drain_stores();
    }
    tzr_publish_u32(V.overflow + BWD_CELLS_OVF_LIST + n_units + blockIdx.x, epoch + 1u);
  }
  if (n > BWD_UMAX || n == 0) return;
  constexpr int kRounds = BWD_UMAX / BWD_THREADS;
  const int pw = bwd_wave_span(n);
  const int rounds = pw / TZR_WAVE;
  uint32_t kreg[kRounds], sreg[kRounds];
  uint32_t vmask = 0, kmin = 0xFFFFFFFFu, kmax = 0u;
#pragma unroll
  for (int r = 0; r < kRounds; ++r) {
    const int lp = wv * pw + r * TZR_WAVE + lane;
    const bool in = r < rounds && lp < n;
#ifdef CELLS_EXP_CONTIG
    const uint2 v = slab[cbase[0] + (uint32_t)(lp < n ? lp : n - 1)];
#else
    const uint2 v = bwd_cells_elem(slab, cpre, cbase, ncell, (uint32_t)(lp < n ? lp : n - 1));
#endif
    kreg[r] = in ? v.x : 0u;
    sreg[r] = in ? v.y : 0u;
    if (in) {
      vmask |= 1u << r;
      kmin = min(kmin, v.x);
      kmax = max(kmax, v.x);
    }
  }
  CELLS_MARK(2);
  bwd_cells_sort_reduce<FAM, FK, NT, kRounds>(u, V, kreg, sreg, vmask, kmin, kmax, n, ft_dst, feats, weights, B, grad_mode, opt, lr,
                                               max_dim, L, sG);
  CELLS_MARK(8);
}

#define TZR_CELLS_APPLY_KERNEL(NAME, FAM_, FK_, ATTR)                                                                         \
  __global__ __launch_bounds__(BWD_THREADS) ATTR void NAME(BwdCellsView V, int n_units, const TzrFeature* __restrict__ feats,  \
                                                          const float* __restrict__ weights, int64_t B, int grad_mode,         \
                                                          BwdGrads G, BwdOpt opt, int max_dim, const uint2* __restrict__ slab, \
                                                          const uint16_t* __restrict__ bnd, int ch) {                          \
    bwd_cells_apply_body<FAM_, FK_, 1>(V, n_units, feats, weights, B, grad_mode, G, opt, max_dim, slab, bnd, ch);             \
  }
TZR_CELLS_APPLY_KERNEL(tzr_bwd_cells_apply_adagrad_kernel, BWD_FAM_LEGACY, TZR_OPT_ADAGRAD, TZR_WAVES_PER_EU(7))
TZR_CELLS_APPLY_KERNEL(tzr_bwd_cells_apply_rowwise_kernel, BWD_FAM_LEGACY, TZR_OPT_ROWWISE_ADAGRAD, TZR_WAVES_PER_EU(7))
TZR_CELLS_APPLY_KERNEL(tzr_bwd_cells_apply_sgd_kernel, BWD_FAM_LEGACY, TZR_OPT_SGD, TZR_WAVES_PER_EU(7))
TZR_CELLS_APPLY_KERNEL(tzr_bwd_cells_apply_general_kernel, BWD_FAM_LEGACY, 0, TZR_WAVES_PER_EU(7))
TZR_CELLS_APPLY_KERNEL(tzr_bwd_cells_apply_adam_kernel, BWD_FAM_ADAM, 0, )
TZR_CELLS_APPLY_KERNEL(tzr_bwd_cells_apply_norm_kernel, BWD_FAM_NORM, 0, )
TZR_CELLS_APPLY_KERNEL(tzr_bwd_cells_apply_elem_kernel, BWD_FAM_ELEM, 0, )

static int cells_common(const void* h_geo, void* d_geo, void* ws, size_t ws_bytes, int64_t n_values, int n_feats, int n_tables,
                        int max_dim, BwdCellsGeo* g, BwdCellsView* V, BwdPlan* P) {
  if (!h_geo || !d_geo || (reinterpret_cast<uintptr_t>(d_geo) & 255)) return TZR_ERR_INVALID;
  std::memcpy(g, h_geo, sizeof(BwdCellsGeo));
  if (g->n_feats != n_feats || g->max_dim != max_dim || g->n_chunks <= 0 || g->n_units <= 0) return TZR_ERR_INVALID;
  if (!ws || (reinterpret_cast<uintptr_t>(ws) & 255)) return TZR_ERR_WORKSPACE;
  if (bwd_layout(P, ws, n_values, g->n_positions, n_feats, n_tables, max_dim) > ws_bytes) return TZR_ERR_WORKSPACE;
  if (P->ch != (int)g->ch || g->n_chunks > P->max_chunks) return TZR_ERR_INVALID;
  *V = bwd_cells_view(d_geo, *g);
  return TZR_OK;
}

extern "C" int tzr_pooled_bwd_cells_plan(const TzrTable* d_tables, int n_tables, const TzrFeature* d_feats, int n_feats,
                                         int max_dim, const int64_t* d_values, int64_t n_values, int64_t B, const void* h_geo,
                                         void* d_geo, void* ws, size_t ws_bytes, void* stream) {
  if (!d_tables || !d_feats || n_tables <= 0 || n_feats <= 0 || n_values < 0 || B <= 0) return TZR_ERR_INVALID;
  BwdCellsGeo g;
  BwdCellsView V;
  BwdPlan P;
  const int rc = cells_common(h_geo, d_geo, ws, ws_bytes, n_values, n_feats, n_tables, max_dim, &g, &V, &P);
  if (rc != TZR_OK) return rc;
  if (!d_values) return TZR_ERR_INVALID;
  if (n_values >= (1LL << 32)) return TZR_ERR_UNSUPPORTED;
  BwdSrcArgs A;
  A.feats = d_feats;
  A.values = d_values;
  A.offsets = nullptr;
  A.B = B;
  A.uniform = 1;
  hipLaunchKernelGGL(tzr_bwd_cells_partition_kernel, dim3((unsigned)g.n_chunks), dim3(BWD_THREADS), 0, static_cast<hipStream_t>(stream), V,
                     d_tables, A, P.ks[1], reinterpret_cast<uint16_t*>(P.hist), (int)g.ch);
  TZR_CHECK_LAUNCH();
  return TZR_OK;
}

extern int g_tzr_fwd_tile_b;
int g_tzr_fwd_plan = 1;

extern "C" int tzr_pooled_fwd_cells_plan_supported(int n_slots, int64_t B) {
  return (g_tzr_fwd_plan != 0 && n_slots > 0 && n_slots <= FWD1_SLOTS && B > 0 && (B >= 32768 || g_tzr_fwd_plan == 2)) ? 1 : 0;
}

extern "C" int tzr_pooled_fwd_cells_plan(const TzrTable* d_ftables, const TzrFeature* d_ffeats, int n_ffeats, const TzrSlot* d_slots,
                                         int n_slots, const TzrDst* h_dsts, int n_dst, const TzrTable* d_tables, int n_tables,
                                         const TzrFeature* d_feats, int n_feats, int max_dim, const int64_t* d_values, int64_t n_values,
                                         int64_t B, const void* h_geo, void* d_geo, void* ws, size_t ws_bytes, void* stream) {
  if (!d_ftables || !d_ffeats || !d_slots || !h_dsts || n_ffeats <= 0 || n_slots <= 0 || n_dst <= 0 || n_dst > TZR_MAX_DST ||
      !d_tables || !d_feats || n_tables <= 0 || n_feats <= 0 || n_values < 0 || B <= 0)
    return TZR_ERR_INVALID;
  if (!tzr_pooled_fwd_cells_plan_supported(n_slots, B)) return TZR_ERR_UNSUPPORTED;
  BwdCellsGeo g;
  BwdCellsView V;
  BwdPlan P;
  const int rc = cells_common(h_geo, d_geo, ws, ws_bytes, n_values, n_feats, n_tables, max_dim, &g, &V, &P);
  if (rc != TZR_OK) return rc;
  if (!d_values) return TZR_ERR_INVALID;
  if (n_values >= (1LL << 32)) return TZR_ERR_UNSUPPORTED;
  FwdDsts dsts;
  for (int i = 0; i < TZR_MAX_DST; ++i) {
    dsts.d[i].ptr = 0;
    dsts.d[i].stride = 0;
  }
  for (int i = 0; i < n_dst; ++i) {
    if (!h_dsts[i].ptr || (h_dsts[i].stride & 3) || (h_dsts[i].ptr & 15)) return TZR_ERR_INVALID;
    if (h_dsts[i].stride > 0x7fffffffLL) return TZR_ERR_UNSUPPORTED;
    dsts.d[i] = h_dsts[i];
  }
  BwdSrcArgs A;
  A.feats = d_feats;
  A.values = d_values;
  A.offsets = nullptr;
  A.B = B;
  A.uniform = 1;
  FwdPlanArgs a;
  a.ftables = d_ftables;
  a.ffeats = d_ffeats;
  a.slots = d_slots;
  a.values = d_values;
  a.B = B;
  a.n_slots = n_slots;
  a.tile_b = g_tzr_fwd_tile_b > 0 ? g_tzr_fwd_tile_b : (B >= 32768 ? 64 : (B >= 8192 ? 16 : 8));
  a.n_fwd = (uint32_t)((B + a.tile_b - 1) / a.tile_b);
  a.n_part = (uint32_t)g.n_chunks;
  a.btables = d_tables;
  a.slab = P.ks[1];
  a.bnd = reinterpret_cast<uint16_t*>(P.hist);
  a.ch = (int)g.ch;
  hipLaunchKernelGGL(tzr_pooled_fwd_u1_cells_plan_kernel, dim3(a.n_fwd + a.n_part), dim3(BWD_THREADS), 0, static_cast<hipStream_t>(stream),
                     a, dsts, V, A);
  TZR_CHECK_LAUNCH();
  return TZR_OK;
}

extern "C" int tzr_pooled_bwd_cells_apply(const TzrTable* d_tables, const TzrFeature* d_feats, int n_feats, int n_tables, int max_dim,
                                          const float* d_weights, int64_t n_values, int64_t B, int grad_mode, const TzrDst* h_grads,
                                          int n_dst, const TzrSparseOptim* h_optim, const void* h_geo, void* d_geo, void* ws,
                                          size_t ws_bytes, void* stream) {
  if (!d_tables || !d_feats || !h_grads || !h_optim || n_tables <= 0 || n_feats <= 0 || n_values < 0 || B <= 0 || n_dst <= 0 ||
      n_dst > TZR_MAX_DST || max_dim <= 0 || max_dim > BWD_MAXDIM || (max_dim & 3) || (grad_mode != 0 && grad_mode != 1))
    return TZR_ERR_INVALID;
  BwdOpt opt;
  if (const int rc = bwd_opt_from(h_optim, true, &opt)) return rc;
  BwdCellsGeo g;
  BwdCellsView V;
  BwdPlan P;
  const int rc = cells_common(h_geo, d_geo, ws, ws_bytes, n_values, n_feats, n_tables, max_dim, &g, &V, &P);
  if (rc != TZR_OK) return rc;
  BwdGrads G;
  if (const int rc = bwd_grads_from(h_grads, n_dst, &G)) return rc;
  hipStream_t s = static_cast<hipStream_t>(stream);
  static constexpr decltype(&tzr_bwd_cells_apply_general_kernel) kernels[BWD_VAR_COUNT] = {
      tzr_bwd_cells_apply_general_kernel, tzr_bwd_cells_apply_sgd_kernel,  tzr_bwd_cells_apply_adagrad_kernel,
      tzr_bwd_cells_apply_rowwise_kernel, tzr_bwd_cells_apply_adam_kernel, tzr_bwd_cells_apply_norm_kernel,
      tzr_bwd_cells_apply_elem_kernel};
  hipLaunchKernelGGL(kernels[bwd_variant(opt.kind, !d_weights)], dim3((unsigned)g.n_units + BWD_CELLS_WORKERS),
                     dim3(BWD_THREADS), 0, s, V, (int)g.n_units, d_feats, d_weights, B, grad_mode, G, opt, max_dim,
                     (const uint2*)P.ks[1], (const uint16_t*)reinterpret_cast<uint16_t*>(P.hist), (int)g.ch);
  TZR_CHECK_LAUNCH();
  return TZR_OK;
}
```

torcheasyrec_amd/dense.py:

```python
from __future__ import annotations

import collections
import contextlib
import dataclasses
import os
import weakref
from typing import Iterable, List, Optional, Tuple

import ctypes as C

import torch

from . import _lib


class _BceLogitsFn(torch.autograd.Function):
    @staticmethod
    def forward(ctx, logits, labels, sample_weight):
        x = logits.contiguous().float()
        y = labels.contiguous()
        if y.dtype not in (torch.float32, torch.int32, torch.int64):
            y = y.float()
        loss = torch.empty((), dtype=torch.float32, device=x.device)
        grad = torch.empty_like(x)
# ... 540 lines not shown
    return fwd, bwd


def repack_w1(p: torch.Tensor) -> None:
    e = _packed_entry(p)
    if e is None:
        return
    q = e.ref()
    _lib.check(_lib.lib().tzr_ia_top_pack_w1(_lib.ptr(q.data), q.stride(0), 27, _lib.ptr(e.fwd), _lib.ptr(e.bwd), _lib.stream_ptr(q.device)),
               "tzr_ia_top_pack_w1")
    e.version = q._version


def _fresh_packed_w1(W1: torch.Tensor) -> Optional["_PackedW1"]:
    e = _packed_entry(W1)
    if e is None:
        return None
    if e.version != e.ref()._version:
        repack_w1(W1)
    return e


class _InteractionTopLossFn(torch.autograd.Function):

    @staticmethod
    def forward(ctx, dense, sparse, D, W1, b1, W2, b2, w3, b3, labels):
        B = sparse.shape[0]
        F = sparse.shape[1] // D
        sparse = sparse.contiguous()
        dense = dense.contiguous()
        n = F + 1
        width = n * (n - 1) // 2 + D * n
        H1 = W1.shape[0]
        dev = sparse.device
        y1 = torch.empty(B, H1, dtype=torch.float32, device=dev)
        z = None if _owned_wgrad(B, sparse.shape[1]) else torch.empty(B, width, dtype=torch.float32, device=dev)
        W1_, b1_ = _f32c(W1), _f32c(b1)
        pk = _fresh_packed_w1(W1_) if (n == 27 and D == 16 and H1 == 64) else None
        head, tail = _ia_top_fwd_args(dense, sparse, F, D, W1_, b1_, z, width, y1, pk)
        _lib.check(_lib.lib().tzr_dot_interaction_top_fwd_packed(*head, B, *tail, _lib.stream_ptr(dev)), "tzr_dot_interaction_top_fwd_packed")
        ctx.w1_packed = pk
        logits, g1, dW2, db2, dw3, scal, db1 = _mlp_tail(y1, labels, W2, b2, w3, b3)
        ctx.save_for_backward(dense, sparse, W1_, g1, dW2, db2, dw3, scal, db1)
        ctx.z = z
        ctx.cfg = (F, D)
        ctx.w1_ref = W1
        ctx.mark_non_differentiable(logits)
        ctx.set_materialize_grads(False)
        return scal[1], logits

    @staticmethod
    def backward(ctx, gl, _glogits):
        dense, sparse, W1, g1, dW2, db2, dw3, scal, db1 = ctx.saved_tensors
        F, D = ctx.cfg
        B = sparse.shape[0]
        root = _loss_is_root(gl)
        gl32 = None if root else gl.reshape(1).to(torch.float32)
        gd = gs = None
        if ctx.needs_input_grad[0] or ctx.needs_input_grad[1]:
            gs = torch.empty_like(sparse)
            gd = torch.empty_like(dense)
            _lib.check(_lib.lib().tzr_dot_interaction_top_bwd_packed(
                *_ia_top_bwd_args(dense, sparse, F, D, g1, W1, gl32, gd, gs, ctx.w1_packed), _lib.stream_ptr(sparse.device)),
                "tzr_dot_interaction_top_bwd_packed")
        if not ctx.needs_input_grad[3]:
            dW1 = None
        elif ctx.z is None:
            dW1 = interaction_top_wgrad(dense, sparse, D, g1, gl32, defer_for=(ctx.w1_ref,))
        else:
            dW1 = weight_grad(g1, ctx.z) if root else weight_grad(g1, ctx.z) * gl
        if root:
            return (gd, gs, None, dW1, db1, dW2, db2, dw3, scal[0:1], None)
        outs = torch._foreach_mul([db1, dW2, db2, dw3, scal[0:1]], gl)
        return (gd, gs, None, dW1, *outs, None)


def _ia_top_fwd_args(dense, sparse, F, D, W1_, b1_, z, width, y1, pk) -> Tuple[tuple, tuple]:
    return ((_lib.ptr(dense), dense.stride(0), _lib.ptr(sparse), sparse.stride(0), F, D),
            (_lib.ptr(W1_), W1_.stride(0), _lib.ptr(b1_), W1_.shape[0], 1, _lib.ptr(z), width, _lib.ptr(y1), y1.stride(0),
             _lib.ptr(pk.fwd) if pk is not None else None))


def _ia_top_bwd_args(dense, sparse, F, D, g1, W1, gl32, gd, gs, pk) -> tuple:
    return (_lib.ptr(dense), dense.stride(0), _lib.ptr(sparse), sparse.stride(0), F, D, sparse.shape[0], _lib.ptr(g1), g1.stride(0),
            g1.shape[1], _lib.ptr(W1), W1.stride(0), _lib.ptr(gl32), _lib.ptr(gd), gd.stride(0), _lib.ptr(gs), gs.stride(0),
            _lib.ptr(pk.bwd) if pk is not None else None)


def interaction_top_wgrad(dense: torch.Tensor, sparse: torch.Tensor, D: int, g1: torch.Tensor,
                          scale: Optional[torch.Tensor] = None, defer_for=None) -> torch.Tensor:
    B = sparse.shape[0]
    F = sparse.shape[1] // D
    n = F + 1
    width = n * (n - 1) // 2 + D * n
    H = g1.shape[1]
    if B == 0:
        return torch.zeros(H, width, dtype=torch.float32, device=sparse.device)
    dW = torch.empty(H, width, dtype=torch.float32, device=sparse.device)
    L = _lib.lib()
    ws = _lib.workspace(L.tzr_dot_interaction_top_wgrad_workspace(F, D, 1, H), sparse.device)
    if defer_for is not None and _defer_finish(sparse.device, defer_for):
        blob = _lib.TzrWgradParts()
        _lib.check(L.tzr_dot_interaction_top_wgrad_parts(
            _lib.ptr(dense), dense.stride(0), _lib.ptr(sparse), sparse.stride(0), F, D, B, _lib.ptr(g1), g1.stride(0), H,
            _lib.ptr(scale), _lib.ptr(ws), ws.numel(), C.byref(blob), _lib.stream_ptr(sparse.device)), "tzr_dot_interaction_top_wgrad_parts")
        _defer(dW, "wgrad", (ws, scale), blob, defer_for)
        return dW
    _lib.check(L.tzr_dot_interaction_top_wgrad(
        _lib.ptr(dense), dense.stride(0), _lib.ptr(sparse), sparse.stride(0), F, D, B, _lib.ptr(g1), g1.stride(0), H,
        _lib.ptr(scale), _lib.ptr(dW), dW.stride(0), _lib.ptr(ws), ws.numel(), _lib.stream_ptr(sparse.device)),
        "tzr_dot_interaction_top_wgrad")
    return dW


def interaction_top_fits(dense: torch.Tensor, sparse: torch.Tensor, D: int, first_linear) -> bool:
    if dense is None or dense.dim() != 2:
        return False
    return _ia_top_fits(dense.shape[1], dense.dtype, sparse, D, first_linear)


def _ia_top_fits(dense_width: int, dense_dtype, sparse: torch.Tensor, D: int, first_linear) -> bool:
    if sparse.dim() != 2 or dense_width != D or sparse.shape[1] % D:
        return False
    if sparse.dtype != torch.float32 or dense_dtype != torch.float32 or first_linear.weight.dtype != torch.float32:
        return False
    F = sparse.shape[1] // D
    n = F + 1
    if first_linear.in_features != n * (n - 1) // 2 + D * n or sparse.shape[0] > (1 << 30):
        return False
    return bool(_lib.lib().tzr_dot_interaction_top_supported(F, D, 1, first_linear.out_features))


def interaction_first_layer(dense, sparse, D, l1) -> torch.Tensor:
    B = sparse.shape[0]
    F = sparse.shape[1] // D
    sparse = sparse.detach().contiguous()
    dense = dense.detach().contiguous()
    W1, b1 = _f32c(l1.weight.detach()), _f32c(l1.bias.detach())
    y1 = torch.empty(B, W1.shape[0], dtype=torch.float32, device=sparse.device)
    _lib.check(_lib.lib().tzr_dot_interaction_top_fwd(
        _lib.ptr(dense), dense.stride(0), _lib.ptr(sparse), sparse.stride(0), F, D, B, _lib.ptr(W1), W1.stride(0), _lib.ptr(b1),
        W1.shape[0], 1, None, 0, _lib.ptr(y1), y1.stride(0), _lib.stream_ptr(sparse.device)), "tzr_dot_interaction_top_fwd")
    return y1


def interaction_top_loss(dense, sparse, D, l1, l2, out_linear, labels):
    return _InteractionTopLossFn.apply(dense, sparse, D, l1.weight, l1.bias, l2.weight, l2.bias, out_linear.weight,
                                       out_linear.bias, labels)


PHASE_MLP2_FWD = os.environ.get("TZR_PHASE_MLP2_FWD", "1") == "1"
PHASE_WGRAD = os.environ.get("TZR_PHASE_WGRAD", "1") == "1"
PHASE_LAUNCHES = [0, 0]


class _HeadLossFn(torch.autograd.Function):

    @staticmethod
    def forward(ctx, x, Wa, ba, Wb, bb, sparse, D, W1, b1, W2, b2, w3, b3, labels):
        xs, ha, hb, Wa_, ba_, Wb_, bb_ = _mlp2_operands(x, Wa, ba, Wb, bb)
        B = sparse.shape[0]
        F = sparse.shape[1] // D
        sparse = sparse.contiguous()
        n = F + 1
        width = n * (n - 1) // 2 + D * n
        H1 = W1.shape[0]
        dev = sparse.device
        y1 = torch.empty(B, H1, dtype=torch.float32, device=dev)
        z = None if _owned_wgrad(B, sparse.shape[1]) else torch.empty(B, width, dtype=torch.float32, device=dev)
        W1_, b1_ = _f32c(W1), _f32c(b1)
        pk = _fresh_packed_w1(W1_) if (n == 27 and D == 16 and H1 == 64) else None
        L = _lib.lib()
        mlp2_args = _mlp2_fwd_args(xs, ha, hb, Wa_, ba_, Wb_, bb_)
        head, tail = _ia_top_fwd_args(hb, sparse, F, D, W1_, b1_, z, width, y1, pk)
        rc = _lib.TZR_ERR_UNSUPPORTED
        if PHASE_MLP2_FWD and pk is not None and z is None:
            rc = L.tzr_dot_interaction_top_fwd_mlp2(*mlp2_args, *head, *tail, _lib.stream_ptr(dev))
        if rc == _lib.TZR_ERR_UNSUPPORTED:
            _lib.check(L.tzr_mlp2_fwd(*mlp2_args, _lib.stream_ptr(dev)), "tzr_mlp2_fwd")
            _lib.check(L.tzr_dot_interaction_top_fwd_packed(*head, B, *tail, _lib.stream_ptr(dev)), "tzr_dot_interaction_top_fwd_packed")
        else:
            _lib.check(rc, "tzr_dot_interaction_top_fwd_mlp2")
            PHASE_LAUNCHES[0] += 1
        logits, g1, dW2, db2, dw3, scal, db1 = _mlp_tail(y1, labels, W2, b2, w3, b3)
        ctx.save_for_backward(xs, ha, hb, Wb_, sparse, W1_, g1, dW2, db2, dw3, scal, db1)
        ctx.z = z
        ctx.cfg = (F, D)
        ctx.w1_packed = pk
        ctx.w1_ref = W1
        ctx.bottom_refs = (Wa, ba, Wb, bb)
        ctx.mark_non_differentiable(logits)
        ctx.set_materialize_grads(False)
        return scal[1], logits

    @staticmethod
    def backward(ctx, gl, _glogits):
        xs, ha, hb, Wb_, sparse, W1, g1, dW2, db2, dw3, scal, db1 = ctx.saved_tensors
        F, D = ctx.cfg
        B = sparse.shape[0]
        dev = sparse.device
        root = _loss_is_root(gl)
        gl32 = None if root else gl.reshape(1).to(torch.float32)
        need_bottom = any(ctx.needs_input_grad[1:5])
        need_x = need_bottom or ctx.needs_input_grad[5]
        need_w1 = ctx.needs_input_grad[7]
        gd = gs = dW1 = None
        L = _lib.lib()
        if need_x:
            gs = torch.empty_like(sparse)
            gd = torch.empty_like(hb)
        one = (PHASE_WGRAD and need_x and need_w1 and ctx.z is None and B > 0 and F == 26 and D == 16 and g1.shape[1] == 64
               and _defer_finish(dev, (ctx.w1_ref,)))
        if one:
            dW1 = torch.empty(g1.shape[1], W1.shape[1], dtype=torch.float32, device=dev)
            ws = _lib.workspace(L.tzr_dot_interaction_top_wgrad_workspace(F, D, 1, g1.shape[1]), dev)
            blob = _lib.TzrWgradParts()
            _lib.check(L.tzr_dot_interaction_top_bwd_wgrad_parts(
                *_ia_top_bwd_args(hb, sparse, F, D, g1, W1, gl32, gd, gs, ctx.w1_packed), _lib.ptr(ws), ws.numel(), C.byref(blob),
                _lib.stream_ptr(dev)), "tzr_dot_interaction_top_bwd_wgrad_parts")
            _defer(dW1, "wgrad", (ws, gl32), blob, (ctx.w1_ref,))
            PHASE_LAUNCHES[1] += 1
        else:
            if need_x:
                _lib.check(L.tzr_dot_interaction_top_bwd_packed(
                    *_ia_top_bwd_args(hb, sparse, F, D, g1, W1, gl32, gd, gs, ctx.w1_packed), _lib.stream_ptr(dev)),
                    "tzr_dot_interaction_top_bwd_packed")
            if need_w1 and ctx.z is None:
                dW1 = interaction_top_wgrad(hb, sparse, D, g1, gl32, defer_for=(ctx.w1_ref,))
            elif need_w1:
                dW1 = weight_grad(g1, ctx.z) if root else weight_grad(g1, ctx.z) * gl
        bottom = _mlp2_backward(xs, ha, hb, Wb_, ctx.bottom_refs, gd) if need_bottom else (None, None, None, None)
        if root:
            return (None, *bottom, gs, None, dW1, db1, dW2, db2, dw3, scal[0:1], None)
        outs = torch._foreach_mul([db1, dW2, db2, dw3, scal[0:1]], gl)
        return (None, *bottom, gs, None, dW1, *outs, None)


def head_phases_fit(x: torch.Tensor, bottom_linears, sparse: torch.Tensor, D: int, first_linear) -> bool:
    if not (PHASE_MLP2_FWD or PHASE_WGRAD) or not mlp2_fits(x, bottom_linears) or bottom_linears[1].out_features != D:
        return False
    return x.shape[0] == sparse.shape[0] and _ia_top_fits(D, torch.float32, sparse, D, first_linear)


def head_phases_loss(x, a, b, sparse, D, l1, l2, out_linear, labels):
    return _HeadLossFn.apply(x, a.weight, a.bias, b.weight, b.bias, sparse, D, l1.weight, l1.bias, l2.weight, l2.bias,
                             out_linear.weight, out_linear.bias, labels)


def _register_fused(opt, fuse_finish: bool) -> torch.device:
    if fuse_finish:
        global FUSE_FINISH
        FUSE_FINISH = True
    name = type(opt).__name__
    if not opt.params:
        raise ValueError("no parameters")
    _OPTIMIZERS.add(opt)
    if fuse_finish:
        me = weakref.ref(opt)
        for k in [k for k, e in _FUSED_OWNER.items() if e[0]() is None or e[1]() is None]:
            del _FUSED_OWNER[k]
        for p in opt.params:
            _FUSED_OWNER[id(p)] = (weakref.ref(p), me)
    dev = opt.params[0].device
    for p in opt.params:
        if p.dtype != torch.float32 or p.device != dev or not p.is_contiguous():
            raise ValueError(f"{name} needs contiguous float32 parameters on one device")
    return dev


def _zero_grad(params, set_to_none: bool = True) -> None:
    _forget({id(p) for p in params if _DEFERRED.pop(id(p), None) is not None})
    for p in params:
        if set_to_none:
            p.grad = None
        elif p.grad is not None:
            p.grad.zero_()


def _check_lr_synced(opt, stale: bool) -> None:
    if not (opt.device.type == "cuda" and torch.cuda.is_current_stream_capturing()):
        opt.sync_lr()
    elif stale:
        raise RuntimeError("learning rate changed since the last sync and a hipGraph capture is open: call "
                           "dense.sync_learning_rates(model, optimizer) before capturing / replaying (INTEGRATION.md)")


def _launch_fused(rows, tables, launch) -> None:
    for base in range(0, len(rows), 32):
        part = rows[base:base + 32]
        grads = [r.grad for r in part]
        materialize_pending(grads[_one_launch(grads):])
        tab, src, wg, keep = tables(part)
        launch(tab, src, wg)
        del keep


def _after_fused_step(opt, packed_written=()) -> None:
    name = type(opt).__name__
    for p in opt.params:
        _DEFERRED.pop(id(p), None)
    if _W1_PACKED:
        for p in opt.params:
            e = _W1_PACKED.get(p.data_ptr())
            if e is not None and e not in packed_written:
                e.version = -1
    if any(e.owner == id(opt) and e.generation == _GENERATION[0] for e in _PENDING.values()):
        raise RuntimeError(f"{name}(fuse_finish=True): a gradient left as partial sums did not reach its parameter's .grad "
                           "as the tensor the backward returned (it was copied on the way); construct the optimizer with "
                           "fuse_finish=False for this model")
    if _PENDING:
        _GENERATION[0] += 1
        for ptr in [q for q, e in _PENDING.items() if e.generation < _GENERATION[0] - 2]:
            del _PENDING[ptr]


class FusedDenseAdam:

    def __init__(self, params: Iterable[torch.nn.Parameter], lr: float = 1e-3, betas=(0.9, 0.999), eps: float = 1e-8,
                 weight_decay: float = 0.0, fuse_finish: bool = False) -> None:
        self.params: List[torch.nn.Parameter] = [p for p in params]
        dev = _register_fused(self, fuse_finish)
        self.param_groups = [{"lr": float(lr), "betas": tuple(betas), "eps": float(eps), "weight_decay": float(weight_decay),
                              "params": self.params}]
        self.device = dev
        self.exp_avg = [torch.zeros_like(p) for p in self.params]
        self.exp_avg_sq = [torch.zeros_like(p) for p in self.params]
        self._state = torch.zeros(len(self.params), 40, dtype=torch.float32, device=dev)
        self._lr_dev = torch.full((1,), float(lr), dtype=torch.float32, device=dev)
        self._lr_host = float(lr)
        for p in self.params:
            register_packed_w1(p)

    def zero_grad(self, set_to_none: bool = True) -> None:
        _zero_grad(self.params, set_to_none)

    def sync_lr(self) -> None:
        g = self.param_groups[0]
        if g["lr"] != self._lr_host:
            self._lr_dev.fill_(g["lr"])
            self._lr_host = g["lr"]

    def step(self, grads: Optional[List[torch.Tensor]] = None) -> None:
        g = self.param_groups[0]
        _check_lr_synced(self, g["lr"] != self._lr_host)
        rows = [_Row(self.params[i].data, gr, self.exp_avg[i], self.exp_avg_sq[i], self._state[i]) for i, gr in _step_grads(self.params, grads)]
        if not rows:
            return
        b1, b2 = g["betas"]
        written = []

        def launch(tab, src, wg):
            w1 = None
            if _W1_PACKED:
                for i in range(len(tab)):
                    e = _W1_PACKED.get(tab[i].param) if tab[i].param else None
                    if e is not None and e.ref() is not None and e.ref().data_ptr() == tab[i].param:
                        w1 = _lib.TzrPackedW1(tab[i].param, _lib.ptr(e.fwd), _lib.ptr(e.bwd))
                        written.append(e)
                        break
            _lib.check(_lib.lib().tzr_dense_adam_fused_w1(
                tab, src, len(tab), C.byref(wg) if wg is not None else None, _lib.ptr(self._lr_dev), g["lr"], b1, b2, g["eps"],
                g["weight_decay"], C.byref(w1) if w1 is not None else None, _lib.stream_ptr(self.device)), "tzr_dense_adam_fused_w1")

        _launch_fused(rows, _adam_tables, launch)
        for e in written:
            torch.autograd.graph.increment_version(e.ref())
            e.version = e.ref()._version
        _after_fused_step(self, written)

    def state_dict(self) -> dict:
        return {"state": {i: {"step": self._state[i, 0].clone(), "exp_avg": m, "exp_avg_sq": v}
                          for i, (m, v) in enumerate(zip(self.exp_avg, self.exp_avg_sq))},
                "param_groups": [{k: v for k, v in self.param_groups[0].items() if k != "params"}]}

    def load_state_dict(self, sd: dict) -> None:
        self._state[:, 1:].zero_()
        for i, st in sd["state"].items():
            self.exp_avg[int(i)].copy_(st["exp_avg"])
            self.exp_avg_sq[int(i)].copy_(st["exp_avg_sq"])
            self._state[int(i), 0] = float(st["step"])
        for k, v in sd["param_groups"][0].items():
            self.param_groups[0][k] = v


def lr_sync_targets(model, optimizer=None) -> list:
    out, seen = [], set()

    def add(o):
        if o is not None and id(o) not in seen and hasattr(o, "sync_lr"):
            seen.add(id(o))
            out.append(o)

    for m in (list(model.modules()) if hasattr(model, "modules") else []):
        try:
            add(getattr(m, "fused_optimizer", None))
        except Exception:
            pass
        for lane in ("local", "replica"):
            sub = getattr(m, lane, None)
# ... 23 lines not shown
```

torcheasyrec_amd/dlrm.py:

```python
from __future__ import annotations

from typing import Dict, List, Optional, Sequence

import torch
from torch import nn

from . import _lib
from .embedding import EmbeddingBagCollection, EmbeddingBagConfig, SparseOptimizerConfig
from .interaction import FactorizationMachine, dot_interaction
from .sparse import KeyedJaggedTensor


import os

_GEMV_OUTPUT = os.environ.get("TZR_OUTPUT_GEMV", "1") == "1"
_FUSED_HEAD_BWD = os.environ.get("TZR_FUSED_HEAD_BWD", "1") == "1"
_FUSED_RELU_BWD = os.environ.get("TZR_MLP_FUSED_RELU_BWD", "1") == "1"
_FUSED_RELU = os.environ.get("TZR_MLP_FUSED_RELU", "1") == "1"
_FUSED_MLP2 = os.environ.get("TZR_FUSED_MLP2", "1") == "1"
_FUSED_TOP_LOSS = os.environ.get("TZR_FUSED_TOP_LOSS", "1") == "1"
_FUSED_IA_TOP = os.environ.get("TZR_FUSED_IA_TOP", "1") == "1"
_FUSED_IA_TOP_MIN_B = int(os.environ.get("TZR_FUSED_IA_TOP_MIN_B", "0"))


# ... 13 lines not shown
            from .dense import relu_bwd_colsum

            g, gb = relu_bwd_colsum(gy, y, defer_for=(ctx.bias_ref,))
        else:
            g = torch.ops.aten.threshold_backward(gy, y, 0.0)
            gb = g.sum(0)
        gx = g @ weight if ctx.needs_input_grad[0] else None
        from .dense import weight_grad

        return gx, weight_grad(g, x), gb


class _Linear1Fn(torch.autograd.Function):

    @staticmethod
    def forward(ctx, x, weight, bias):
        ctx.save_for_backward(x, weight)
        return torch.nn.functional.linear(x, weight, bias)

    @staticmethod
    def backward(ctx, gy):
        x, weight = ctx.saved_tensors
        if _FUSED_HEAD_BWD and x.shape[1] % 4 == 0 and x.shape[1] <= 1024 and x.dtype == torch.float32:
            from .dense import head_bwd

            return head_bwd(gy, x, weight, ctx.needs_input_grad[0])
        gx = gy @ weight if ctx.needs_input_grad[0] else None
        return gx, (x * gy).sum(0, keepdim=True), gy.sum(0)


class _SkinnyLinearFn(torch.autograd.Function):

    @staticmethod
    def forward(ctx, x, weight, bias):
        from .dense import skinny_linear_fwd

        ctx.save_for_backward(x, weight)
        ctx.has_bias = bias is not None
        ctx.param_refs = (weight, bias) if bias is not None else None
        return skinny_linear_fwd(x, weight.detach(), None if bias is None else bias.detach())

    @staticmethod
    def backward(ctx, gy):
        from .dense import skinny_linear_bwd

        x, weight = ctx.saved_tensors
        gx, gw, gb = skinny_linear_bwd(gy.float(), x, weight, ctx.needs_input_grad[0], defer_for=ctx.param_refs)
        return gx, gw, (gb if ctx.has_bias else None)


_SKINNY_LINEAR = os.environ.get("TZR_SKINNY_LINEAR", "1") == "1"


class OutputLinear(nn.Linear):

    def forward(self, x: torch.Tensor) -> torch.Tensor:
        if _SKINNY_LINEAR and (x.is_cuda or _lib.emulated()) and x.dim() == 2:
            from .dense import skinny_linear_ok

            if skinny_linear_ok(x, self.weight):
                return _SkinnyLinearFn.apply(x, self.weight, self.bias)
        if _GEMV_OUTPUT and self.out_features == 1 and x.is_cuda and x.dim() == 2 and self.bias is not None:
            return _Linear1Fn.apply(x, self.weight, self.bias)
        return super().forward(x)


def _activation(name: Optional[str]) -> Optional[nn.Module]:
    if not name:
        return None
    cls = getattr(nn, name[3:], None) if name.startswith("nn.") else None
    if cls is None:
        raise NotImplementedError(f"MLP activation {name!r}: only torch.nn activations (\"nn.ReLU\", \"nn.GELU\", ...) are built")
    return cls()


class MLP(nn.Module):

    def __init__(self, in_features: int, hidden_units: Sequence[int], bias: bool = True, activation: Optional[str] = "nn.ReLU",
                 use_bn: bool = False, dropout_ratio=None, use_ln: bool = False, return_hidden_layer_feature: bool = False) -> None:
        super().__init__()
        self.hidden_units = list(hidden_units)
        self.return_hidden_layer_feature = bool(return_hidden_layer_feature)
        if use_bn and use_ln:
            raise ValueError("Could not use_bn and use_ln at the same time in Perceptron.")
        if dropout_ratio is None or (isinstance(dropout_ratio, (list, tuple)) and len(dropout_ratio) == 0):
            drops = [0.0] * len(self.hidden_units)
        elif isinstance(dropout_ratio, (list, tuple)):
            drops = [float(x) for x in dropout_ratio]
            if len(drops) == 1:
                drops = drops * len(self.hidden_units)
            if len(drops) != len(self.hidden_units):
                raise ValueError("length of dropout_ratio and hidden_units must be same")
        else:
            drops = [float(dropout_ratio)] * len(self.hidden_units)
        self._plain = bias and activation == "nn.ReLU" and not use_bn and not use_ln and not any(d > 0 for d in drops)
        layers: List[nn.Module] = []
        ends: List[int] = []
        d = in_features
        for h, dr in zip(self.hidden_units, drops):
            layers.append(nn.Linear(d, h, bias=False if use_bn else bias))
            if use_bn:
                layers.append(nn.BatchNorm1d(h))
            if use_ln:
                layers.append(nn.LayerNorm(h))
            act = _activation(activation)
            if act is not None:
                layers.append(act)
            if dr > 0.0:
                layers.append(nn.Dropout(dr))
            d = h
            ends.append(len(layers))
        self.mlp = nn.Sequential(*layers)
        self._layer_ends = ends

    def output_dim(self) -> int:
        return self.hidden_units[-1]

    def linears(self) -> List[nn.Linear]:
        return [m for m in self.mlp if isinstance(m, nn.Linear)]

    def _hidden_features(self, x: torch.Tensor) -> Dict[str, torch.Tensor]:
        fused = self._plain and _FUSED_RELU and x.is_cuda and x.dim() == 2
        out: Dict[str, torch.Tensor] = {}
        start = 0
        for i, end in enumerate(self._layer_ends):
            if fused:
                x = _LinearReluFn.apply(x, self.mlp[start].weight, self.mlp[start].bias)
            else:
                for m in self.mlp[start:end]:
                    x = m(x)
            out[f"hidden_layer{i}"] = x
            start = end
        if self._layer_ends:
            out["hidden_layer_end"] = x
        return out

    def forward(self, x: torch.Tensor):
        if self.return_hidden_layer_feature:
            return self._hidden_features(x)
        if self._plain and _FUSED_MLP2 and x.dim() == 2 and (x.is_cuda or _lib.emulated()):
            from .dense import mlp2, mlp2_fits

            lin = self.linears()
            if mlp2_fits(x, lin):
                return mlp2(x, lin[0].weight, lin[0].bias, lin[1].weight, lin[1].bias)
        if self._plain and _FUSED_RELU and x.is_cuda and x.dim() == 2:
            for m in self.mlp:
                if isinstance(m, nn.Linear):
                    x = _LinearReluFn.apply(x, m.weight, m.bias)
            return x
        return self.mlp(x)


def head_loss(model, dense: torch.Tensor, sparse: torch.Tensor, labels: torch.Tensor, d: Optional[torch.Tensor] = None):
    fused = _FUSED_TOP_LOSS and model.final_mlp._plain and (sparse.is_cuda or _lib.emulated())
    if (d is None and fused and _FUSED_IA_TOP and _FUSED_MLP2 and model.arch_with_sparse and sparse.shape[0] >= _FUSED_IA_TOP_MIN_B
            and getattr(model.dense_mlp, "_plain", False) and dense.dim() == 2 and (dense.is_cuda or _lib.emulated())):
        from .dense import head_phases_fit, head_phases_loss, top_loss_fits

        bot, lin = model.dense_mlp.linears(), model.final_mlp.linears()
        if head_phases_fit(dense, bot, sparse, model.dim, lin[0]) and top_loss_fits(sparse, lin, model.output_mlp):
            return head_phases_loss(dense, bot[0], bot[1], sparse, model.dim, lin[0], lin[1], model.output_mlp, labels)
    if d is None:
        d = model.dense_mlp(dense)
    if fused and _FUSED_IA_TOP and model.arch_with_sparse and sparse.shape[0] >= _FUSED_IA_TOP_MIN_B:
        from .dense import interaction_top_fits, interaction_top_loss, top_loss_fits

        lin = model.final_mlp.linears()
        if interaction_top_fits(d, sparse, model.dim, lin[0]) and top_loss_fits(sparse, lin, model.output_mlp):
            return interaction_top_loss(d, sparse, model.dim, lin[0], lin[1], model.output_mlp, labels)
    allf = dot_interaction(d, sparse, model.dim, cat_dense=True, cat_sparse=model.arch_with_sparse)
    if fused:
        from .dense import top_loss, top_loss_fits

        lin = model.final_mlp.linears()
        if top_loss_fits(allf, lin, model.output_mlp):
            return top_loss(allf, lin[0], lin[1], model.output_mlp, labels)
    logits = model.output_mlp(model.final_mlp(allf)).squeeze(1)
    return bce_with_logits(logits, labels), logits.detach()


class DLRM(nn.Module):

    def __init__(
        self,
        tables: Sequence[EmbeddingBagConfig],
        sparse_features: Sequence[str],
        dense_dim: int,
        dense_mlp: Sequence[int] = (64, 16),
        final_mlp: Sequence[int] = (64, 32),
        arch_with_sparse: bool = True,
        num_class: int = 1,
        device: Optional[torch.device] = None,
        sparse_optimizer: Optional[SparseOptimizerConfig] = None,
        row_layout: str = "interleaved",
    ) -> None:
        super().__init__()
        dims = {f: t.embedding_dim for t in tables for f in t.feature_names}
        dset = {dims[f] for f in sparse_features}
        if len(dset) != 1:
            raise ValueError(f"sparse group feature dims must be the same, but we find {dset}")
        self.dim = dset.pop()
        if dense_mlp[-1] != self.dim:
            raise ValueError("dense mlp last hidden_unit must be the same sparse feature dim")
        self.num_sparse = len(sparse_features)
        self.arch_with_sparse = arch_with_sparse
        self.ebc = EmbeddingBagCollection(
            tables, device=device, optimizer=sparse_optimizer, groups={"sparse": list(sparse_features)},
            row_layout=row_layout,
        )
        self.dense_mlp = MLP(dense_dim, dense_mlp)
        n = self.num_sparse + 1
        feat = n * (n - 1) // 2 + self.dim + (self.num_sparse * self.dim if arch_with_sparse else 0)
        self.final_mlp = MLP(feat, final_mlp)
        self.output_mlp = OutputLinear(self.final_mlp.output_dim(), num_class)
        if device is not None:
            self.dense_mlp.to(device)
            self.final_mlp.to(device)
            self.output_mlp.to(device)

    def dense_parameters(self):
        for m in (self.dense_mlp, self.final_mlp, self.output_mlp):
            yield from m.parameters()

    def predict_from_embeddings(self, dense: torch.Tensor, sparse: torch.Tensor) -> torch.Tensor:
        d = self.dense_mlp(dense)
        if (not torch.is_grad_enabled() and _FUSED_IA_TOP and self.final_mlp._plain and self.arch_with_sparse
                and (sparse.is_cuda or _lib.emulated()) and sparse.shape[0] >= _FUSED_IA_TOP_MIN_B):
            from .dense import interaction_first_layer, interaction_top_fits

            lin = self.final_mlp.linears()
            if interaction_top_fits(d, sparse, self.dim, lin[0]):
                y = interaction_first_layer(d, sparse, self.dim, lin[0])
                for l in lin[1:]:
                    y = torch.relu(l(y))
                return self.output_mlp(y).squeeze(1)
        allf = dot_interaction(d, sparse, self.dim, cat_dense=True, cat_sparse=self.arch_with_sparse)
        return self.output_mlp(self.final_mlp(allf)).squeeze(1)

    def forward(self, dense: torch.Tensor, sparse_features: KeyedJaggedTensor) -> torch.Tensor:
        sparse = self.ebc.forward_grouped(sparse_features)["sparse"]
        return self.predict_from_embeddings(dense, sparse)

    def loss_from_embeddings(self, dense: torch.Tensor, sparse: torch.Tensor, labels: torch.Tensor):
        return head_loss(self, dense, sparse, labels)

    def forward_loss(self, dense: torch.Tensor, sparse_features: KeyedJaggedTensor, labels: torch.Tensor):
        sparse = self.ebc.forward_grouped(sparse_features)["sparse"]
        return self.loss_from_embeddings(dense, sparse, labels)


class DeepFM(nn.Module):

    def __init__(
        self,
        tables: Sequence[EmbeddingBagConfig],
        groups: Dict[str, List[str]],
        dense_dim: int,
        fm_dim: int,
        deep_mlp: Sequence[int] = (512, 256, 128),
        final_mlp: Optional[Sequence[int]] = (64,),
        num_class: int = 1,
        device: Optional[torch.device] = None,
        sparse_optimizer: Optional[SparseOptimizerConfig] = None,
    ) -> None:
        super().__init__()
        self.ebc = EmbeddingBagCollection(tables, device=device, optimizer=sparse_optimizer, groups=groups)
        self.has_fm_group = "fm" in groups
        self.fm_dim = fm_dim
        dims = self.ebc._out_dim
        deep_in = sum(dims[k] for k in groups["deep"]) + dense_dim
        self.deep_mlp = MLP(deep_in, deep_mlp)
        self.fm = FactorizationMachine()
        final_dim = self.deep_mlp.output_dim()
        self.final_mlp = None
        if final_mlp:
            self.final_mlp = MLP(1 + fm_dim + final_dim, final_mlp)
            final_dim = self.final_mlp.output_dim()
        self.output_mlp = OutputLinear(final_dim, num_class)
        if device is not None:
            self.to(device)

    def dense_parameters(self):
        mods = [self.deep_mlp, self.output_mlp] + ([self.final_mlp] if self.final_mlp is not None else [])
        for m in mods:
            yield from m.parameters()

    def forward(self, dense: torch.Tensor, sparse_features: KeyedJaggedTensor) -> torch.Tensor:
        g = self.ebc.forward_grouped(sparse_features)
        y_wide = g["wide"].sum(dim=1, keepdim=True)
        deep = torch.cat([dense, g["deep"]], dim=1)
        y_deep = self.deep_mlp(deep)
        fm_in = g["fm"] if self.has_fm_group else g["deep"]
        y_fm = self.fm(fm_in.reshape(fm_in.shape[0], -1, self.fm_dim))
        if self.final_mlp is not None:
            y = self.output_mlp(self.final_mlp(torch.cat([y_wide, y_fm, y_deep], dim=1)))
        else:
            y = y_wide + y_fm.sum(dim=1, keepdim=True) + self.output_mlp(y_deep)
        return y.squeeze(1)


def bce_with_logits(logits: torch.Tensor, labels: torch.Tensor) -> torch.Tensor:
    from .dense import bce_with_logits as fused

    return fused(logits, labels)
```

torcheasyrec_amd/embedding.py:

```python
from __future__ import annotations

import math
import os
from dataclasses import dataclass, field
from typing import Callable, Dict, List, Optional, Sequence, Tuple

import numpy as np
import torch
from torch import nn

from . import _lib, opt_kinds
from .sparse import KeyedJaggedTensor, KeyedTensor
from .sparse_bwd import SparseBackward, cells_geometry, direct_supported, grad_dsts


@dataclass
class EmbeddingBagConfig:

    name: str
    embedding_dim: int
    num_embeddings: int
    feature_names: List[str] = field(default_factory=list)
    pooling: str = "sum"
    init_fn: Optional[Callable[[torch.Tensor], None]] = None
# ... 57 lines not shown

    def adam_state(self, device: torch.device) -> torch.Tensor:
        if self._adam is None or self._adam.device != device:
            self._adam = torch.zeros(4, dtype=torch.float32, device=device)
        return self._adam

    def begin_step(self, device: torch.device) -> None:
        if self.cfg.kind in TICKING_KINDS:
            _lib.check(_lib.lib().tzr_sparse_adam_tick(_lib.ptr(self.adam_state(device)), self.cfg.beta1, self.cfg.beta2,
                                                       _lib.stream_ptr(device)), "tzr_sparse_adam_tick")

    def optim_struct(self, device: torch.device, kind: Optional[int] = None) -> "_lib.TzrSparseOptim":
        cfg = self.cfg
        opt = _lib.TzrSparseOptim()
        opt.kind = _OPT_KIND[cfg.kind] if kind is None else kind
        opt.weight_decay_mode = _WD_MODE[cfg.weight_decay_mode.lower()]
        opt.d_lr = _lib.ptr(self.lr_device(device))
        opt.eps, opt.weight_decay, opt.max_gradient = cfg.eps, cfg.weight_decay, cfg.max_gradient
        opt.gradient_clipping = 1 if cfg.gradient_clipping else 0
        opt.beta1, opt.beta2 = (getattr(cfg, name) for name in opt_kinds.of(cfg.kind).slots)
        opt.d_adam = _lib.ptr(self.adam_state(device)) if cfg.kind in TICKING_KINDS else 0
        return opt

    @property
    def params(self) -> Dict[str, torch.Tensor]:
        return self._ebc.table_weights()

    def lr_device(self, device: torch.device) -> torch.Tensor:
        capturing = device.type == "cuda" and torch.cuda.is_current_stream_capturing()
        if self._lr_dev is None or self._lr_dev.device != device:
            if capturing:
                raise RuntimeError("the fused sparse optimizer's device learning rate does not exist yet: run one eager step "
                                   "(or call fused_optimizer.sync_lr(device)) before capturing a graph with update kernels")
            lr = float(self.param_groups[0]["lr"])
            self._lr_dev = torch.full((1,), lr, dtype=torch.float32, device=device)
            self._lr_host = lr
        elif not capturing:
            self.sync_lr(device)
        elif float(self.param_groups[0]["lr"]) != self._lr_host:
            raise RuntimeError("learning rate changed since the last sync and a hipGraph capture is open: call "
                               "dense.sync_learning_rates(model, optimizer) before capturing / replaying (INTEGRATION.md)")
        return self._lr_dev

    def sync_lr(self, device: Optional[torch.device] = None) -> None:
        if self._lr_dev is None:
            if device is None:
                return
            self.lr_device(device)
            return
        lr = float(self.param_groups[0]["lr"])
        if lr != self._lr_host:
            self._lr_dev.fill_(lr)
            self._lr_host = lr

    def zero_grad(self, set_to_none: bool = True) -> None:
        pass

    def step(self, closure=None) -> None:
        pass

    def state_dict(self) -> Dict[str, object]:
        return {
            "state": {n: {"momentum1": s} for n, s in self._ebc.table_states().items()},
            "param_groups": [{"lr": self.param_groups[0]["lr"]}],
            "adam_step": None if self._adam is None else float(self._adam[0]),
        }

    def load_state_dict(self, sd: Dict[str, object]) -> None:
        for n, st in sd.get("state", {}).items():
            dst = self._ebc.table_states().get(n)
            if dst is not None:
                dst.copy_(st["momentum1"])
        if sd.get("param_groups"):
            self.param_groups[0]["lr"] = sd["param_groups"][0]["lr"]
        if sd.get("adam_step") is not None and self.cfg.kind in TICKING_KINDS:
            self.set_adam_step(float(sd["adam_step"]))

    def set_adam_step(self, t: float, device: Optional[torch.device] = None) -> None:
        st = self.adam_state(device or self._ebc._device)
        st.copy_(torch.tensor([t, 1.0 - self.cfg.beta1 ** t, 1.0 - self.cfg.beta2 ** t, 0.0], dtype=torch.float32))


class _Table(nn.Module):
    def __init__(self, weight: torch.Tensor) -> None:
        super().__init__()
        self.weight = nn.Parameter(weight, requires_grad=False)


@dataclass
class _Lookup:
    key: str
    table: int
    out_key: str


class _Meta:

    def __init__(self) -> None:
        self.tables_np = self.feats_np = self.slots_np = None
        self.d_tables = self.d_feats = self.d_slots = None
        self.d_bwd_tables = self.d_bwd_feats = None
        self.bwd_tables_np = self.bwd_feats_np = None
        self.n_keys = 0
        self.cells: Dict[int, Optional["_CellsGeo"]] = {}


class _CellsGeo:

    def __init__(self, image: np.ndarray, info, device: torch.device) -> None:
        self.h_img = image
        self.h_ptr = image.ctypes.data
        self.n_chunks, self.n_units = int(info[1]), int(info[2])
        self.d_img = _lib.workspace(image.nbytes, device)[:image.nbytes]
        self.d_img.copy_(torch.from_numpy(image))
        off = int(info[6])
        self.d_overflow = self.d_img[off:off + 4].view(torch.int32)
        pin = device.type == "cuda"
        self.h_overflow = torch.zeros(1, dtype=torch.int32, pin_memory=pin)
        self.seen = 0
        self.copied = None
        self.launches = 0
        self.demoted = False


@dataclass(slots=True)
class _Plan:

    owner: int
    dst_names: Tuple[str, ...]
    ws: torch.Tensor
    ready: Optional["torch.cuda.Event"]
    geo: Optional[_CellsGeo]
    origin: str


def mask_frozen_descriptors(tables: np.ndarray, feats: np.ndarray, frozen: Sequence[bool]):
    bt, bf = tables.copy(), feats.copy()
    by_order = np.argsort(feats["order"], kind="stable")
    live = [int(i) for i in by_order if feats[i]["table"] >= 0 and not frozen[int(feats[i]["table"])]]
    dead = [int(i) for i in by_order if not (feats[i]["table"] >= 0 and not frozen[int(feats[i]["table"])])]
    for o, i in enumerate(live + dead):
        bf[i]["order"] = o
    for i in dead:
        bf[i]["table"] = -1
    for t in range(len(bt)):
        mine = [i for i in live if int(feats[i]["table"]) == t]
        bt[t]["first_order"] = int(bf[mine[0]]["order"]) if mine else 0
        bt[t]["n_feats"] = len(mine)
    return bt, bf


class _PooledLookupFn(torch.autograd.Function):
    @staticmethod
    def forward(ctx, ebc, kjt, dst_names, hook):
        outs = ebc._launch_forward(kjt, dst_names, with_plan=True)
        ctx.ebc, ctx.kjt, ctx.dst_names = ebc, kjt, dst_names
        return tuple(outs)

    @staticmethod
    def backward(ctx, *grads):
        ctx.ebc._launch_backward(ctx.kjt, ctx.dst_names, grads)
        return None, None, None, None


class EmbeddingBagCollection(nn.Module):

    def __init__(
        self,
        tables: Sequence[EmbeddingBagConfig],
        device: Optional[torch.device] = None,
        optimizer: Optional[SparseOptimizerConfig] = None,
        groups: Optional[Dict[str, List[str]]] = None,
        row_layout: str = "interleaved",
    ) -> None:
        super().__init__()
        device = torch.device(device) if device is not None else torch.device("cpu")
        self._device = device
        self._configs = list(tables)
        self._opt_cfg = optimizer
        self._row_layout = row_layout
        self.embedding_bags = nn.ModuleDict()
        self._storage: List[torch.Tensor] = []
        self._states: Dict[str, torch.Tensor] = {}
        self._lookups: List[_Lookup] = []
        names = set()
        feat_tables: Dict[str, List[int]] = {}
        for t, cfg in enumerate(self._configs):
            if cfg.name in names:
                raise ValueError(f"duplicate table name {cfg.name}")
            names.add(cfg.name)
            if cfg.embedding_dim % 4 or cfg.embedding_dim > 256:
                raise ValueError(f"{cfg.name}: embedding_dim must be a multiple of 4, <= 256")
            for f in cfg.feature_names:
                feat_tables.setdefault(f, []).append(t)
        for t, cfg in enumerate(self._configs):
            for f in cfg.feature_names:
                out_key = f if len(feat_tables[f]) == 1 else f"{f}@{cfg.name}"
                self._lookups.append(_Lookup(f, t, out_key))
        self._out_dim = {lk.out_key: self._configs[lk.table].embedding_dim for lk in self._lookups}
        self._allocate()
        self._has_fp16 = any(m.weight.dtype == torch.float16 for m in self.embedding_bags.values())
        self._groups = groups
        self._dst_layouts: Dict[Tuple[str, ...], List[Tuple[str, List[str]]]] = {}
        self._meta_cache: Dict[Tuple, _Meta] = {}
        self.fused_optimizer = FusedSparseOptimizer(optimizer, self) if optimizer is not None else None
        self._hook = torch.zeros(0, requires_grad=True, device=device)
        self._timers = None
        self._side_stream = None
        self._lookup_trackers: list = []
        self._track_segs: Dict[Tuple[str, ...], tuple] = {}
        self.async_plan = False
        self.forward_plan = os.environ.get("TZR_FWD_PLAN", "1") != "0"
        self.forward_plans = 0
        self.expect_hot_rows = False
        self._dims = (max(c.num_embeddings for c in self._configs), max(c.embedding_dim for c in self._configs))
        self._direct_ws: Dict[int, torch.Tensor] = {}
        self.plan_mode = os.environ.get("TZR_BWD_PLAN", "auto")
        if self.plan_mode not in ("auto", "cells", "exact"):
            raise ValueError("TZR_BWD_PLAN: auto | cells | exact")

    CELLS_PROBATION = 4

    def _cells_geometry(self, meta: _Meta, B: int) -> Optional[_CellsGeo]:
        if B in meta.cells:
            return meta.cells[B]
        made = cells_geometry(meta.bwd_tables_np, meta.bwd_feats_np, B, self._bwd_dims()[1])
        geo = None if made is None else _CellsGeo(*made, self._device)
        meta.cells[B] = geo
        return geo

    def reset_plan_mode(self) -> None:
        for meta in self._meta_cache.values():
            for geo in meta.cells.values():
                if geo is not None:
                    if geo.copied is not None:
                        geo.copied.synchronize()
                    geo.seen, geo.demoted, geo.launches = int(geo.h_overflow[0]), False, 0

    def _cells_for(self, kjt: KeyedJaggedTensor, meta: _Meta) -> Optional[_CellsGeo]:
        if self.plan_mode == "exact" or kjt.uniform_length() != 1 or kjt.weights_or_none() is not None:
            return None
        geo = self._cells_geometry(meta, kjt.stride())
        if geo is None or self.plan_mode == "cells":
            return geo
        if geo.demoted:
            return None
        capturing = self._device.type == "cuda" and torch.cuda.is_current_stream_capturing()
        if geo.copied is not None and geo.launches <= self.CELLS_PROBATION and not capturing:
            geo.copied.synchronize()
        if int(geo.h_overflow[0]) != geo.seen:
            geo.demoted = True
            return None
        return geo

    def _allocate(self) -> None:
        kind = self._opt_cfg.kind if self._opt_cfg is not None else None
        init_m = self._opt_cfg.initial_accumulator_value if self._opt_cfg is not None else 0.0
        for cfg in self._configs:
            rows, D = cfg.num_embeddings, cfg.embedding_dim
            dt = cfg.data_type.upper()
            if dt not in ("FP32", "FP16"):
                raise ValueError(f"{cfg.name}: data_type {cfg.data_type!r} not supported (FP32 | FP16)")
            shape = _state_shape(kind, rows, D)
            if shape is not None:
                store = torch.empty(rows, D, dtype=torch.float16 if dt == "FP16" else torch.float32, device=self._device)
                weight = store
                state = torch.zeros(*shape, dtype=torch.float32, device=self._device)
            elif dt == "FP16":
                store = torch.empty(rows, D, dtype=torch.float16, device=self._device)
                weight = store
                state = (torch.full((rows, D), init_m, dtype=torch.float32, device=self._device) if kind == "adagrad"
                         else torch.zeros(rows, dtype=torch.float32, device=self._device) if kind == "rowwise_adagrad"
                         else None)
            elif kind == "adagrad" and self._row_layout == "interleaved":
                store = torch.empty(rows, 2 * D, dtype=torch.float32, device=self._device)
                weight, state = store[:, :D], store[:, D:]
                state.fill_(init_m)
            elif kind == "rowwise_adagrad" and self._row_layout == "interleaved":
                store = torch.zeros(rows, 2 * D, dtype=torch.float32, device=self._device)
                weight, state = store[:, :D], store[:, D]
            else:
                store = torch.empty(rows, D, dtype=torch.float32, device=self._device)
                weight = store
                if kind == "adagrad":
                    state = torch.full((rows, D), init_m, dtype=torch.float32, device=self._device)
                elif kind == "rowwise_adagrad":
                    state = torch.zeros(rows, dtype=torch.float32, device=self._device)
                else:
                    state = None
            if cfg.init_fn is not None:
                cfg.init_fn(weight)
            else:
                a = math.sqrt(1.0 / max(rows, 1))
                weight.uniform_(-a, a)
            self._storage.append(store)
            self.embedding_bags[cfg.name] = _Table(weight)
            if state is not None:
                self._states[cfg.name] = state

    def table_weights(self) -> Dict[str, torch.Tensor]:
        return {n: m.weight for n, m in self.embedding_bags.items()}

    def table_states(self) -> Dict[str, torch.Tensor]:
        return self._states

    def embedding_bag_configs(self) -> List[EmbeddingBagConfig]:
        return self._configs

    @property
    def device(self) -> torch.device:
        return self._device

    def _default_layout(self) -> List[Tuple[str, List[str]]]:
        return [("__all__", [lk.out_key for lk in self._lookups])]

    def _meta(self, kjt_keys: Sequence[str], layout: List[Tuple[str, List[str]]]) -> _Meta:
        ck = (tuple(kjt_keys), tuple((n, tuple(ks)) for n, ks in layout),
              tuple(m.weight.data_ptr() for m in self.embedding_bags.values()))
        meta = self._meta_cache.get(ck)
        if meta is not None:
            return meta
        if len(layout) > _lib.TZR_MAX_DST:
            raise ValueError(f"at most {_lib.TZR_MAX_DST} feature groups per lookup")
        key_index = {k: i for i, k in enumerate(kjt_keys)}
        T, Fn = len(self._configs), len(self._lookups)
        feats = np.zeros(Fn, dtype=_lib.FEATURE_DT)
        feats["dst"] = -1
        by_out = {lk.out_key: i for i, lk in enumerate(self._lookups)}
        for i, lk in enumerate(self._lookups):
            if lk.key not in key_index:
                raise KeyError(f"KeyedJaggedTensor has no key {lk.key!r} needed by table "
                               f"{self._configs[lk.table].name!r}")
            feats[i]["table"] = lk.table
            feats[i]["key"] = key_index[lk.key]
            feats[i]["pooling"] = _lib.POOL_MEAN if self._configs[lk.table].pooling.lower() == "mean" else _lib.POOL_SUM
        feats["order"] = np.arange(Fn, dtype=np.int32)
        slots = []
        for d, (_, out_keys) in enumerate(layout):
            col = 0
            for ok in out_keys:
                i = by_out[ok]
                n = int(feats[i]["n_dst"])
                if n >= _lib.TZR_MAX_FEAT_DST:
                    raise ValueError(f"{ok}: a lookup can be copied into at most {_lib.TZR_MAX_FEAT_DST} groups")
                feats[i]["dst"][n] = d
                feats[i]["col"][n] = col
                feats[i]["n_dst"] = n + 1
                D = self._configs[self._lookups[i].table].embedding_dim
                for c in range(D // 4):
                    slots.append((i, c, d, col + 4 * c))
                col += D
        tables = np.zeros(T, dtype=_lib.TABLE_DT)
        kind = self._opt_cfg.kind if self._opt_cfg is not None else None
        for t, cfg in enumerate(self._configs):
            w = self.embedding_bags[cfg.name].weight
            st = self._states.get(cfg.name)
            tables[t]["w"] = w.data_ptr()
            tables[t]["m"] = st.data_ptr() if st is not None else 0
            tables[t]["rows"] = cfg.num_embeddings
            tables[t]["dim"] = cfg.embedding_dim
            tables[t]["w_stride"] = w.stride(0)
            tables[t]["w_dtype"] = _lib.DT_F16 if w.dtype == torch.float16 else _lib.DT_F32
            tables[t]["m_stride"] = st.stride(0) if st is not None else 0
            if st is not None:
                check_state_stride(kind, cfg.embedding_dim, st.stride(0))
            mine = [i for i, lk in enumerate(self._lookups) if lk.table == t]
            tables[t]["first_order"] = mine[0] if mine else 0
            tables[t]["n_feats"] = len(mine)
        meta = _Meta()
        meta.tables_np, meta.feats_np = tables, feats
        meta.slots_np = np.array(slots, dtype=_lib.SLOT_DT)
        meta.d_tables = _lib.upload_struct(tables, self._device)
        meta.d_feats = _lib.upload_struct(feats, self._device)
        frozen = [not cfg.trainable for cfg in self._configs]
        meta.d_bwd_tables, meta.d_bwd_feats = meta.d_tables, meta.d_feats
        meta.bwd_tables_np, meta.bwd_feats_np = tables, feats
        if any(frozen):
            bt, bf = mask_frozen_descriptors(tables, feats, frozen)
            meta.bwd_tables_np, meta.bwd_feats_np = bt, bf
            meta.d_bwd_tables = _lib.upload_struct(bt, self._device)
            meta.d_bwd_feats = _lib.upload_struct(bf, self._device)
        meta.d_slots = _lib.upload_struct(meta.slots_np, self._device)
        meta.n_keys = len(kjt_keys)
        self._meta_cache[ck] = meta
        return meta

    def _layout_for(self, dst_names: Tuple[str, ...]) -> List[Tuple[str, List[str]]]:
        if dst_names == ("__all__",):
            return self._default_layout()
        assert self._groups is not None
        return [(g, self._groups[g]) for g in dst_names]

    def _kjt_args(self, kjt: KeyedJaggedTensor):
        uniform = kjt.uniform_length() == 1
        offsets = None if uniform else kjt.offsets()
        return uniform, offsets

    def _forward_carries_plan(self, kjt: KeyedJaggedTensor, meta: _Meta) -> Optional[Tuple["_CellsGeo", SparseBackward]]:
        if not self.forward_plan or self._has_fp16 or kjt.uniform_length() != 1 or kjt.weights_or_none() is not None:
            return None
        left = getattr(kjt, "_tzr_plan", None)
        if left is not None and left.origin == "caller":
            return None
        p = self._problem(kjt, meta)
        if p.direct_supported():
            return None
        if not _lib.lib().tzr_pooled_fwd_cells_plan_supported(len(meta.slots_np), kjt.stride()):
            return None
        geo = self._cells_for(kjt, meta)
        return None if geo is None else (geo, p)

    def _launch_forward(self, kjt: KeyedJaggedTensor, dst_names: Tuple[str, ...], with_plan: bool = False) -> List[torch.Tensor]:
        layout = self._layout_for(dst_names)
        meta = self._meta(kjt.keys(), layout)
        B = kjt.stride()
        uniform, offsets = self._kjt_args(kjt)
        widths = [sum(self._out_dim[k] for k in ks) for _, ks in layout]
        outs = [torch.empty(B, w, dtype=torch.float32, device=self._device) for w in widths]
        dsts = grad_dsts(outs)
        carried = None
        if with_plan:
            left = getattr(kjt, "_tzr_plan", None)
            if left is not None and left.origin == "forward" and left.owner == id(self):
                kjt._tzr_plan = None
            carried = self._forward_carries_plan(kjt, meta)
        if carried is not None:
            geo, p = carried
            ws = _lib.workspace(p.plan_bytes(), self._device)
            ev = self._timers.start("fwd+plan") if self._timers is not None else None
            rc = _lib.lib().tzr_pooled_fwd_cells_plan(
                _lib.ptr(meta.d_tables), _lib.ptr(meta.d_feats), len(self._lookups), _lib.ptr(meta.d_slots), len(meta.slots_np), dsts,
                len(outs), _lib.ptr(p.d_tables), p.n_tables, _lib.ptr(p.d_feats), p.n_feats, p.max_dim,
                _lib.ptr(p.values), p.n_values, p.B, geo.h_ptr, _lib.ptr(geo.d_img), _lib.ptr(ws), ws.numel(), _lib.stream_ptr(self._device))
            if rc != _lib.TZR_ERR_UNSUPPORTED:
                if ev is not None:
                    ev.record()
                _lib.check(rc, "tzr_pooled_fwd_cells_plan")
                if self._device.type == "cuda" and not torch.cuda.is_current_stream_capturing():
                    ws.record_stream(torch.cuda.current_stream(self._device))
                kjt._tzr_plan = _Plan(id(self), dst_names, ws, None, geo, "forward")
                self.forward_plans += 1
                return outs
            if self._timers is not None:
                self._timers.pairs["fwd+plan"].pop()
        ev = self._timers.start("fwd") if self._timers is not None else None
        rc = _lib.lib().tzr_pooled_fwd_ex(
            _lib.ptr(meta.d_tables), _lib.ptr(meta.d_feats), len(self._lookups),
            _lib.ptr(meta.d_slots), len(meta.slots_np), _lib.ptr(kjt.values()), _lib.ptr(offsets),
            _lib.ptr(kjt.weights_or_none()), B, dsts, len(outs), 1 if uniform else 0,
            _lib.FWD_MIXED_DTYPE if self._has_fp16 else 0, _lib.stream_ptr(self._device),
        )
        if ev is not None:
            ev.record()
        _lib.check(rc, "tzr_pooled_fwd")
        return outs

    def _bwd_dims(self) -> Tuple[int, int]:
        return self._dims

    def _n_positions(self, kjt: KeyedJaggedTensor) -> int:
        if kjt.uniform_length() is not None:
            return len(self._lookups) * kjt.stride() * kjt.uniform_length()
        mult: Dict[str, int] = {}
        for lk in self._lookups:
            mult[lk.key] = mult.get(lk.key, 0) + 1
        return kjt.values().numel() * max(mult.values())

    def _problem(self, kjt: KeyedJaggedTensor, meta: _Meta) -> SparseBackward:
        _, offsets = self._kjt_args(kjt)
        max_rows, max_dim = self._bwd_dims()
        values = kjt.values()
        return SparseBackward(self._device, meta.d_bwd_tables, meta.d_bwd_feats, len(self._configs), len(self._lookups), meta.n_keys,
                              max_rows, max_dim, values, offsets, kjt.weights_or_none(), values.numel(), self._n_positions(kjt),
                              kjt.stride())

    def _direct_workspace(self, p: SparseBackward) -> torch.Tensor:
        ws = self._direct_ws.get(p.n_positions)
        if ws is None:
            ws = self._direct_ws[p.n_positions] = _lib.zeroed_workspace(p.direct_bytes(), self._device)
        return ws

    def backward_is_direct(self, kjt: KeyedJaggedTensor) -> bool:
        return direct_supported(self._n_positions(kjt), len(self._lookups), len(self._configs), kjt.uniform_length() == 1)

    def backward_form(self, kjt: KeyedJaggedTensor, dst_names: Tuple[str, ...] = ("__all__",)) -> str:
        if self.backward_is_direct(kjt):
            return "direct"
        meta = self._meta(kjt.keys(), self._layout_for(dst_names))
        return "cells" if self._cells_for(kjt, meta) is not None else "exact"

    def _plan(self, kjt: KeyedJaggedTensor, meta: _Meta, p: SparseBackward) -> Tuple[torch.Tensor, Optional[_CellsGeo]]:
        ws = _lib.workspace(p.plan_bytes(), self._device)
        geo = self._cells_for(kjt, meta)
        ev = self._timers.start("plan") if self._timers is not None else None
        if geo is not None:
            p.cells_plan(geo, ws)
        else:
            p.plan(ws)
        if ev is not None:
            ev.record()
        if self._device.type == "cuda" and not torch.cuda.is_current_stream_capturing():
            ws.record_stream(torch.cuda.current_stream(self._device))
        return ws, geo

    def plan_backward(self, kjt: KeyedJaggedTensor, dst_names: Tuple[str, ...] = ("__all__",)) -> Optional[torch.Tensor]:
        meta = self._meta(kjt.keys(), self._layout_for(dst_names))
        p = self._problem(kjt, meta)
        if p.direct_supported():
            return None
        ws, geo = self._plan(kjt, meta, p)
        kjt._tzr_plan = _Plan(id(self), dst_names, ws, None, geo, "caller")
        return ws

    def plan_backward_async(self, kjt: KeyedJaggedTensor, dst_names: Tuple[str, ...] = ("__all__",)) -> None:
        if self._device.type != "cuda" or self.backward_is_direct(kjt):
            self.plan_backward(kjt, dst_names)
            return
        if self._side_stream is None:
            self._side_stream = torch.cuda.Stream(device=self._device)
        cur = torch.cuda.current_stream(self._device)
        self._side_stream.wait_stream(cur)
        with torch.cuda.stream(self._side_stream):
            self.plan_backward(kjt, dst_names)
            ev = torch.cuda.Event()
            ev.record()
        if not torch.cuda.is_current_stream_capturing():
            for t in (kjt.values(), kjt.offsets_or_none()):
                if t is not None:
                    t.record_stream(self._side_stream)
        kjt._tzr_plan.ready = ev

    def _claim(self, kjt: KeyedJaggedTensor, dst_names: Tuple[str, ...], use: bool = True) -> Optional[_Plan]:
        plan = getattr(kjt, "_tzr_plan", None)
        kjt._tzr_plan = None
        if not use or plan is None or plan.owner != id(self) or plan.dst_names != dst_names:
            return None
        if plan.ready is not None:
            cur = torch.cuda.current_stream(self._device)
            cur.wait_event(plan.ready)
            if not torch.cuda.is_current_stream_capturing():
                plan.ws.record_stream(cur)
        return plan

    def _launch_backward(self, kjt: KeyedJaggedTensor, dst_names: Tuple[str, ...], grads) -> None:
        if self.fused_optimizer is None:
            return
        layout = self._layout_for(dst_names)
        meta = self._meta(kjt.keys(), layout)
        p = self._problem(kjt, meta)
        direct = p.direct_supported()
        plan = self._claim(kjt, dst_names, use=not direct)
        if plan is not None:
            ws, geo = plan.ws, plan.geo
        else:
            ws, geo = (None, None) if direct else self._plan(kjt, meta, p)
        widths = [sum(self._out_dim[k] for k in ks) for _, ks in layout]
        gl = []
        for g, w in zip(grads, widths):
            if g is None:
                g = torch.zeros(p.B, w, dtype=torch.float32, device=self._device)
            g = g.contiguous()
            if g.dtype != torch.float32:
                g = g.float()
            gl.append(g)
        gd = grad_dsts(gl)
        self.fused_optimizer.begin_step(self._device)
        opt = self.fused_optimizer.optim_struct(self._device)
        ev = self._timers.start("apply") if self._timers is not None else None
        if direct:
            p.direct(self._direct_workspace(p), gd, opt, hot_rows=self.expect_hot_rows)
        elif geo is not None:
            p.cells_apply(geo, ws, gd, opt)
        else:
            p.apply(ws, gd, opt)
        if ev is not None:
            ev.record()
        if geo is not None and self.plan_mode == "auto":
            geo.launches += 1
            geo.h_overflow.copy_(geo.d_overflow, non_blocking=True)
            if self._device.type == "cuda" and not torch.cuda.is_current_stream_capturing():
                geo.copied = torch.cuda.Event()
                geo.copied.record(torch.cuda.current_stream(self._device))

    def register_post_lookup_tracker_fn(self, fn) -> None:
        self._lookup_trackers.append(fn)

    def _notify_trackers(self, kjt: KeyedJaggedTensor) -> None:
        keys = tuple(kjt.keys())
        segs = self._track_segs.get(keys)
        if segs is None:
            index = {k: i for i, k in enumerate(keys)}
            segs = tuple((self._configs[lk.table].name, index[lk.key]) for lk in self._lookups if lk.key in index)
            self._track_segs[keys] = segs
        uniform, offsets = self._kjt_args(kjt)
        for fn in self._lookup_trackers:
            fn(self, segs, kjt.values(), offsets, kjt.stride(), 1 if uniform else 0)

    def _run(self, kjt: KeyedJaggedTensor, dst_names: Tuple[str, ...]) -> List[torch.Tensor]:
        if kjt.uniform_length() is None and getattr(kjt, "_uniform_keys", None):
            view = kjt.uniform_prefix([lk.key for lk in self._lookups])
            if view is not None:
                kjt = view
        if self._lookup_trackers:
            self._notify_trackers(kjt)
        if torch.is_grad_enabled() and self.fused_optimizer is not None and self.training:
            if self.async_plan and getattr(kjt, "_tzr_plan", None) is None:
                self.plan_backward_async(kjt, dst_names)
            return list(_PooledLookupFn.apply(self, kjt, dst_names, self._hook))
        return self._launch_forward(kjt, dst_names)

    def forward(self, features: KeyedJaggedTensor) -> KeyedTensor:
        (out,) = self._run(features, ("__all__",))
        keys = [lk.out_key for lk in self._lookups]
        return KeyedTensor(keys, [self._out_dim[k] for k in keys], out)

    def forward_grouped(self, features: KeyedJaggedTensor, group_names: Optional[Sequence[str]] = None) -> Dict[str, torch.Tensor]:
        if self._groups is None:
            raise ValueError("EmbeddingBagCollection was built without groups")
        names = tuple(group_names) if group_names is not None else tuple(self._groups)
        outs = self._run(features, names)
        return dict(zip(names, outs))

    def bounds_check(self, features: KeyedJaggedTensor, mode: int = _lib.BOUNDS_WARNING) -> torch.Tensor:
        meta = self._meta(features.keys(), self._default_layout())
        cnt = torch.zeros(1, dtype=torch.int64, device=self._device)
        rc = _lib.lib().tzr_bounds_check(
            _lib.ptr(meta.d_tables), _lib.ptr(meta.d_feats), len(self._lookups),
            _lib.ptr(features.values()), _lib.ptr(features.offsets()), features.stride(), mode,
            _lib.ptr(cnt), _lib.stream_ptr(self._device),
        )
        _lib.check(rc, "tzr_bounds_check")
        return cnt
```

Before: 144.6 million samples/s.

## Run bottom MLP forward inside embedding forward+plan kernel as extra workgroups

Adds extra workgroups to the pooled embedding forward/backward-plan kernel that compute the two-layer bottom MLP (dense features to 64 to 16) with MFMA. Wb and the biases are staged in LDS that the union already reserves. The head then reuses the precomputed ha/hb instead of launching a separate MLP2 forward. This removes one kernel launch and lets the compute-bound MLP overlap with the memory-bound embedding gather, at the cost of more coupling between the embedding and head paths and extra workgroups competing for the GPU.

```diff
diff --git a/include/tzrec_hip.h b/include/tzrec_hip.h
--- a/include/tzrec_hip.h
+++ b/include/tzrec_hip.h
@@ -618,6 +618,13 @@
 int tzr_mlp2_fwd(const float* d_x, int64_t x_stride, int64_t B, int K0, const float* d_Wa, const float* d_ba, int H1,
                  const float* d_Wb, const float* d_bb, int H2, float* d_ha, int64_t ha_stride, float* d_hb,
                  int64_t hb_stride, void* stream);
+int tzr_pooled_fwd_cells_plan_mlp2(const TzrTable* d_ftables, const TzrFeature* d_ffeats, int n_ffeats, const TzrSlot* d_slots,
+                                   int n_slots, const TzrDst* h_dsts, int n_dst, const TzrTable* d_tables, int n_tables,
+                                   const TzrFeature* d_feats, int n_feats, int max_dim, const int64_t* d_values, int64_t n_values,
+                                   int64_t B, const void* h_geo, void* d_geo, void* ws, size_t ws_bytes, const float* d_x,
+                                   int64_t x_stride, int K0, const float* d_Wa, const float* d_ba, int H1, const float* d_Wb,
+                                   const float* d_bb, int H2, float* d_ha, int64_t ha_stride, float* d_hb, int64_t hb_stride,
+                                   void* stream);
 int tzr_mlp2_bwd(const float* d_dhb, int64_t dhb_stride, const float* d_hb, int64_t hb_stride, const float* d_ha,
                  int64_t ha_stride, const float* d_x, int64_t x_stride, int64_t B, int K0, int H1, int H2,
                  const float* d_Wb, float* d_dWa, float* d_dba, float* d_dWb, float* d_dbb, void* ws, size_t ws_bytes,
diff --git a/torcheasyrec_amd/_lib.py b/torcheasyrec_amd/_lib.py
--- a/torcheasyrec_amd/_lib.py
+++ b/torcheasyrec_amd/_lib.py
@@ -304,6 +304,8 @@
     "tzr_pooled_bwd_cells_plan": (_i32, [_vp, _i32, _vp, _i32, _i32, _vp, _i64, _i64, _vp, _vp, _vp, _sz, _vp]),
     "tzr_pooled_fwd_cells_plan_supported": (_i32, [_i32, _i64]),
     "tzr_pooled_fwd_cells_plan": (_i32, [_vp, _vp, _i32, _vp, _i32, _vp, _i32, _vp, _i32, _vp, _i32, _i32, _vp, _i64, _i64, _vp, _vp, _vp, _sz, _vp]),
+    "tzr_pooled_fwd_cells_plan_mlp2": (_i32, [_vp, _vp, _i32, _vp, _i32, _vp, _i32, _vp, _i32, _vp, _i32, _i32, _vp, _i64, _i64, _vp, _vp, _vp, _sz,
+                                              _vp, _i64, _i32, _vp, _vp, _i32, _vp, _vp, _i32, _vp, _i64, _vp, _i64, _vp]),
     "tzr_pooled_bwd_cells_apply": (_i32, [_vp, _vp, _i32, _i32, _i32, _vp, _i64, _i64, _i32, C.POINTER(TzrDst), _i32,
                                           C.POINTER(TzrSparseOptim), _vp, _vp, _vp, _sz, _vp]),
     "tzr_dense_adam_fused": (_i32, [C.POINTER(TzrAdamTensor), C.POINTER(TzrAdamSource), _i32, C.POINTER(TzrWgradParts), _vp, C.c_float,
diff --git a/torcheasyrec_amd/csrc/mlp2_fwd16_body.h b/torcheasyrec_amd/csrc/mlp2_fwd16_body.h
--- a/torcheasyrec_amd/csrc/mlp2_fwd16_body.h
+++ b/torcheasyrec_amd/csrc/mlp2_fwd16_body.h
@@ -11,12 +11,34 @@
 #define MB_H2 16
 #define MB_PX 20
 
-__device__ __forceinline__ void mb_fwd16_tiles(
+#define MB_WS_BIAS (MB_H2 * MT_P1)
+#define MB_WS_FLOATS (MB_WS_BIAS + MB_H1 + MB_H2)
+__device__ __forceinline__ void mb_stage_wb(const float* __restrict__ Wb, const float* __restrict__ ba, const float* __restrict__ bb,
+                                            float* Ws, int tid, int nthreads) {
+  for (int e = tid; e < MB_H2 * (MB_H1 / 4); e += nthreads) {
+    const int row = e >> 4, c4 = e & 15;
+    tzr_st4(Ws + row * MT_P1 + 4 * c4, tzr_ld4(Wb + row * MB_H1 + 4 * c4));
+  }
+  for (int e = tid; e < MB_H1 + MB_H2; e += nthreads) {
+    const float* b = e < MB_H1 ? ba : bb;
+    Ws[MB_WS_BIAS + e] = b ? b[e < MB_H1 ? e : e - MB_H1] : 0.f;
+  }
+}
+
+__device__ __forceinline__ int mb_lane_again(int lane) {
+#ifdef __AMDGCN__
+  asm volatile("" : "+v"(lane));
+#endif
+  return lane;
+}
+
+template <bool WB_LDS>
+__device__ __forceinline__ void mb_fwd16_tiles_t(
     const float* __restrict__ x, int64_t xs, int64_t B, int K0, const float* __restrict__ Wa, const float* __restrict__ ba,
     const float* __restrict__ Wb, const float* __restrict__ bb, float* __restrict__ ha, int64_t has, float* __restrict__ hb,
-    int64_t hbs, float* T1, int lane, int64_t t0, int64_t step) {
+    int64_t hbs, float* T1, const float* Ws, int lane, int64_t t0, int64_t step) {
   const int r = lane & 15, q = lane >> 4;
-  float Wfa[4][4], Wfb[16], bav[4];
+  float Wfa[4][4], Wfb[WB_LDS ? 1 : 16], bav[WB_LDS ? 1 : 4];
 #pragma unroll
   for (int hbk = 0; hbk < 4; ++hbk) {
 #pragma unroll
@@ -25,14 +47,17 @@
       const float w = Wa[(16 * hbk + r) * K0 + (k < K0 ? k : 0)];
       Wfa[hbk][ks] = k < K0 ? w : 0.f;
     }
-    bav[hbk] = ba ? ba[16 * hbk + r] : 0.f;
+    if constexpr (!WB_LDS) bav[hbk] = ba ? ba[16 * hbk + r] : 0.f;
   }
+  if constexpr (!WB_LDS) {
 #pragma unroll
-  for (int i = 0; i < 4; ++i) {
-    const float4 v = tzr_ld4(Wb + r * MB_H1 + 16 * q + 4 * i);
-    Wfb[4 * i] = v.x; Wfb[4 * i + 1] = v.y; Wfb[4 * i + 2] = v.z; Wfb[4 * i + 3] = v.w;
+    for (int i = 0; i < 4; ++i) {
+      const float4 v = tzr_ld4(Wb + r * MB_H1 + 16 * q + 4 * i);
+      Wfb[4 * i] = v.x; Wfb[4 * i + 1] = v.y; Wfb[4 * i + 2] = v.z; Wfb[4 * i + 3] = v.w;
+    }
   }
-  const float bbv = bb ? bb[r] : 0.f;
+  float bbv = 0.f;
+  if constexpr (!WB_LDS) bbv = bb ? bb[r] : 0.f;
   const int64_t tiles = (B + MM_TS - 1) / MM_TS;
   for (int64_t t = t0; t < tiles; t += step) {
     const int64_t b0 = t * MM_TS;
@@ -54,26 +79,42 @@
 #pragma unroll
       for (int hbk = 0; hbk < 4; ++hbk) acc[hbk] = __builtin_amdgcn_mfma_f32_16x16x4f32(xa[ks], Wfa[hbk][ks], acc[hbk], 0, 0, 0);
 #pragma unroll
-    for (int hbk = 0; hbk < 4; ++hbk)
+    for (int hbk = 0; hbk < 4; ++hbk) {
+      const float bv = WB_LDS ? Ws[MB_WS_BIAS + 16 * hbk + r] : bav[hbk];
 #pragma unroll
-      for (int j = 0; j < 4; ++j) T1[(4 * q + j) * MT_P1 + 16 * hbk + r] = fmaxf(acc[hbk][j] + bav[hbk], 0.f);
+      for (int j = 0; j < 4; ++j) T1[(4 * q + j) * MT_P1 + 16 * hbk + r] = fmaxf(acc[hbk][j] + bv, 0.f);
+    }
     __builtin_amdgcn_wave_barrier();
     mm_f32x4 acc2 = {0.f, 0.f, 0.f, 0.f};
+    const int sl = WB_LDS ? mb_lane_again(lane) : lane;
 #pragma unroll
     for (int i = 0; i < 4; ++i) {
-      const int e = lane + TZR_WAVE * i, row = e >> 4, c4 = e & 15;
+      const int e = sl + TZR_WAVE * i, row = e >> 4, c4 = e & 15;
       if (b0 + row < B) tzr_st4(ha + (b0 + row) * has + 4 * c4, tzr_ld4(T1 + row * MT_P1 + 4 * c4));
       const float4 av = tzr_ld4(T1 + r * MT_P1 + 16 * q + 4 * i);
-      acc2 = __builtin_amdgcn_mfma_f32_16x16x4f32(av.x, Wfb[4 * i], acc2, 0, 0, 0);
-      acc2 = __builtin_amdgcn_mfma_f32_16x16x4f32(av.y, Wfb[4 * i + 1], acc2, 0, 0, 0);
-      acc2 = __builtin_amdgcn_mfma_f32_16x16x4f32(av.z, Wfb[4 * i + 2], acc2, 0, 0, 0);
-      acc2 = __builtin_amdgcn_mfma_f32_16x16x4f32(av.w, Wfb[4 * i + 3], acc2, 0, 0, 0);
+      float4 wv;
+      if constexpr (WB_LDS)
+        wv = tzr_ld4(Ws + r * MT_P1 + 16 * q + 4 * i);
+      else
+        wv = make_float4(Wfb[4 * i], Wfb[4 * i + 1], Wfb[4 * i + 2], Wfb[4 * i + 3]);
+      acc2 = __builtin_amdgcn_mfma_f32_16x16x4f32(av.x, wv.x, acc2, 0, 0, 0);
+      acc2 = __builtin_amdgcn_mfma_f32_16x16x4f32(av.y, wv.y, acc2, 0, 0, 0);
+      acc2 = __builtin_amdgcn_mfma_f32_16x16x4f32(av.z, wv.z, acc2, 0, 0, 0);
+      acc2 = __builtin_amdgcn_mfma_f32_16x16x4f32(av.w, wv.w, acc2, 0, 0, 0);
     }
+    if constexpr (WB_LDS) bbv = Ws[MB_WS_BIAS + MB_H1 + r];
 #pragma unroll
     for (int j = 0; j < 4; ++j)
-      if (b0 + 4 * q + j < B) hb[(b0 + 4 * q + j) * hbs + r] = fmaxf(acc2[j] + bbv, 0.f);
+      if (b0 + 4 * (sl >> 4) + j < B) hb[(b0 + 4 * (sl >> 4) + j) * hbs + (sl & 15)] = fmaxf(acc2[j] + bbv, 0.f);
     __builtin_amdgcn_wave_barrier();
   }
+}
+
+__device__ __forceinline__ void mb_fwd16_tiles(
+    const float* __restrict__ x, int64_t xs, int64_t B, int K0, const float* __restrict__ Wa, const float* __restrict__ ba,
+    const float* __restrict__ Wb, const float* __restrict__ bb, float* __restrict__ ha, int64_t has, float* __restrict__ hb,
+    int64_t hbs, float* T1, int lane, int64_t t0, int64_t step) {
+  mb_fwd16_tiles_t<false>(x, xs, B, K0, Wa, ba, Wb, bb, ha, has, hb, hbs, T1, nullptr, lane, t0, step);
 }
 
 static inline bool mb_fwd16_fits(int K0, int H1, int H2, const float* d_Wb, const float* d_ha, int64_t ha_stride) {
diff --git a/torcheasyrec_amd/csrc/pooled_bwd_cells.hip b/torcheasyrec_amd/csrc/pooled_bwd_cells.hip
--- a/torcheasyrec_amd/csrc/pooled_bwd_cells.hip
+++ b/torcheasyrec_amd/csrc/pooled_bwd_cells.hip
@@ -22,6 +22,7 @@
 #define CELLS_NOTE(i, v)
 #endif
 
+#include "mlp2_fwd16_body.h"
 #include "pooled_bwd_apply.h"
 #include "pooled_bwd_cells.h"
 #include "pooled_bwd_sort.h"
@@ -345,15 +346,44 @@
 #ifndef FWD_PLAN_UNROLL
 #define FWD_PLAN_UNROLL 4
 #endif
+
+struct FwdMlpArgs {
+  const float *x, *Wa, *ba, *Wb, *bb;
+  float *ha, *hb;
+  int64_t xs, has, hbs;
+  int32_t K0;
+  uint32_t n_mlp, first;
+};
+#ifndef FWD_MLP_WGS
+#define FWD_MLP_WGS 256
+#endif
+#ifndef FWD_MLP_POS
+#define FWD_MLP_POS 0
+#endif
+static_assert(BWD_THREADS / TZR_WAVE == 4, "a rider is four waves, one ha tile each");
+
 union FwdPlanLds {
   Fwd1Lds f;
   BwdPartLds p;
+  float m[4 * MM_TS * MT_P1 + MB_WS_FLOATS];
 };
+static_assert(sizeof(FwdPlanLds) == sizeof(Fwd1Lds), "the riders' tiles fit in the forward's LDS: no byte more per workgroup");
 
 __global__ __launch_bounds__(BWD_THREADS) TZR_WAVES_PER_EU(FWD_PLAN_WAVES) void tzr_pooled_fwd_u1_cells_plan_kernel(FwdPlanArgs a, FwdDsts dsts,
-                                                                                                          BwdCellsView V, BwdSrcArgs A) {
-  __shared__ FwdPlanLds S;
-  const uint32_t i = blockIdx.x;
+                                                                                                          BwdCellsView V, BwdSrcArgs A,
+                                                                                                          FwdMlpArgs m) {
+  __shared__ __attribute__((aligned(16))) FwdPlanLds S;
+  uint32_t i = blockIdx.x;
+  if (i - m.first < m.n_mlp) {
+    float* Ws = S.m + 4 * MM_TS * MT_P1;
+    mb_stage_wb(m.Wb, m.ba, m.bb, Ws, (int)threadIdx.x, BWD_THREADS);
+    __syncthreads();
+    const int wv = __builtin_amdgcn_readfirstlane((int)(threadIdx.x / TZR_WAVE));
+    mb_fwd16_tiles_t<true>(m.x, m.xs, a.B, m.K0, m.Wa, m.ba, m.Wb, m.bb, m.ha, m.has, m.hb, m.hbs, S.m + wv * (MM_TS * MT_P1), Ws,
+                           (int)(threadIdx.x & (TZR_WAVE - 1)), (int64_t)(i - m.first) * 4 + wv, (int64_t)m.n_mlp * 4);
+    return;
+  }
+  if (i >= m.first) i -= m.n_mlp;
   const bool part = i >= a.n_fwd;
   const uint32_t idx = part ? i - a.n_fwd : i;
   if (part)
@@ -863,16 +893,18 @@
 }
 
 extern int g_tzr_fwd_tile_b;
+extern int g_tzr_mlp_mfma;
 int g_tzr_fwd_plan = 1;
 
 extern "C" int tzr_pooled_fwd_cells_plan_supported(int n_slots, int64_t B) {
   return (g_tzr_fwd_plan != 0 && n_slots > 0 && n_slots <= FWD1_SLOTS && B > 0 && (B >= 32768 || g_tzr_fwd_plan == 2)) ? 1 : 0;
 }
 
-extern "C" int tzr_pooled_fwd_cells_plan(const TzrTable* d_ftables, const TzrFeature* d_ffeats, int n_ffeats, const TzrSlot* d_slots,
-                                         int n_slots, const TzrDst* h_dsts, int n_dst, const TzrTable* d_tables, int n_tables,
-                                         const TzrFeature* d_feats, int n_feats, int max_dim, const int64_t* d_values, int64_t n_values,
-                                         int64_t B, const void* h_geo, void* d_geo, void* ws, size_t ws_bytes, void* stream) {
+static int fwd_cells_plan_launch(const TzrTable* d_ftables, const TzrFeature* d_ffeats, int n_ffeats, const TzrSlot* d_slots,
+                                 int n_slots, const TzrDst* h_dsts, int n_dst, const TzrTable* d_tables, int n_tables,
+                                 const TzrFeature* d_feats, int n_feats, int max_dim, const int64_t* d_values, int64_t n_values,
+                                 int64_t B, const void* h_geo, void* d_geo, void* ws, size_t ws_bytes, FwdMlpArgs m, bool ride,
+                                 void* stream) {
   if (!d_ftables || !d_ffeats || !d_slots || !h_dsts || n_ffeats <= 0 || n_slots <= 0 || n_dst <= 0 || n_dst > TZR_MAX_DST ||
       !d_tables || !d_feats || n_tables <= 0 || n_feats <= 0 || n_values < 0 || B <= 0)
     return TZR_ERR_INVALID;
@@ -914,10 +946,40 @@
   a.slab = P.ks[1];
   a.bnd = reinterpret_cast<uint16_t*>(P.hist);
   a.ch = (int)g.ch;
-  hipLaunchKernelGGL(tzr_pooled_fwd_u1_cells_plan_kernel, dim3(a.n_fwd + a.n_part), dim3(BWD_THREADS), 0, static_cast<hipStream_t>(stream),
-                     a, dsts, V, A);
+  m.n_mlp = m.first = 0u;
+  if (ride) {
+    const int64_t tiles = (B + MM_TS - 1) / MM_TS;
+    m.n_mlp = (uint32_t)std::min<int64_t>((tiles + 3) / 4, g_tzr_mlp_mfma > 0 ? std::min(g_tzr_mlp_mfma, FWD_MLP_WGS) : FWD_MLP_WGS);
+    m.first = FWD_MLP_POS == 0 ? 0u : (FWD_MLP_POS == 1 ? a.n_fwd : a.n_fwd + a.n_part);
+  }
+  hipLaunchKernelGGL(tzr_pooled_fwd_u1_cells_plan_kernel, dim3(a.n_fwd + a.n_part + m.n_mlp), dim3(BWD_THREADS), 0,
+                     static_cast<hipStream_t>(stream), a, dsts, V, A, m);
   TZR_CHECK_LAUNCH();
   return TZR_OK;
+}
+
+extern "C" int tzr_pooled_fwd_cells_plan(const TzrTable* d_ftables, const TzrFeature* d_ffeats, int n_ffeats, const TzrSlot* d_slots,
+                                         int n_slots, const TzrDst* h_dsts, int n_dst, const TzrTable* d_tables, int n_tables,
+                                         const TzrFeature* d_feats, int n_feats, int max_dim, const int64_t* d_values, int64_t n_values,
+                                         int64_t B, const void* h_geo, void* d_geo, void* ws, size_t ws_bytes, void* stream) {
+  return fwd_cells_plan_launch(d_ftables, d_ffeats, n_ffeats, d_slots, n_slots, h_dsts, n_dst, d_tables, n_tables, d_feats, n_feats, max_dim,
+                               d_values, n_values, B, h_geo, d_geo, ws, ws_bytes, FwdMlpArgs{}, false, stream);
+}
+
+extern "C" int tzr_pooled_fwd_cells_plan_mlp2(const TzrTable* d_ftables, const TzrFeature* d_ffeats, int n_ffeats, const TzrSlot* d_slots,
+                                              int n_slots, const TzrDst* h_dsts, int n_dst, const TzrTable* d_tables, int n_tables,
+                                              const TzrFeature* d_feats, int n_feats, int max_dim, const int64_t* d_values,
+                                              int64_t n_values, int64_t B, const void* h_geo, void* d_geo, void* ws, size_t ws_bytes,
+                                              const float* d_x, int64_t x_stride, int K0, const float* d_Wa, const float* d_ba, int H1,
+                                              const float* d_Wb, const float* d_bb, int H2, float* d_ha, int64_t ha_stride, float* d_hb,
+                                              int64_t hb_stride, void* stream) {
+  if (!d_x || !d_Wa || !d_Wb || !d_ha || !d_hb || K0 <= 0 || H1 <= 0 || H2 <= 0) return TZR_ERR_INVALID;
+  if (g_tzr_mlp_mfma < 0 || !mb_fwd16_fits(K0, H1, H2, d_Wb, d_ha, ha_stride)) return TZR_ERR_UNSUPPORTED;
+  FwdMlpArgs m{};
+  m.x = d_x; m.Wa = d_Wa; m.ba = d_ba; m.Wb = d_Wb; m.bb = d_bb; m.ha = d_ha; m.hb = d_hb;
+  m.xs = x_stride; m.has = ha_stride; m.hbs = hb_stride; m.K0 = K0;
+  return fwd_cells_plan_launch(d_ftables, d_ffeats, n_ffeats, d_slots, n_slots, h_dsts, n_dst, d_tables, n_tables, d_feats, n_feats, max_dim,
+                               d_values, n_values, B, h_geo, d_geo, ws, ws_bytes, m, true, stream);
 }
 
 extern "C" int tzr_pooled_bwd_cells_apply(const TzrTable* d_tables, const TzrFeature* d_feats, int n_feats, int n_tables, int max_dim,
diff --git a/torcheasyrec_amd/dense.py b/torcheasyrec_amd/dense.py
--- a/torcheasyrec_amd/dense.py
+++ b/torcheasyrec_amd/dense.py
@@ -716,13 +716,40 @@
 PHASE_MLP2_FWD = os.environ.get("TZR_PHASE_MLP2_FWD", "1") == "1"
 PHASE_WGRAD = os.environ.get("TZR_PHASE_WGRAD", "1") == "1"
 PHASE_LAUNCHES = [0, 0]
+FWD_RIDE_MLP2 = os.environ.get("TZR_FWD_RIDE_MLP2", "1") == "1"
+RIDE_LAUNCHES = [0]
+
+
+class Mlp2Rider:
+
+    __slots__ = ("x", "params", "batch", "ops", "taken")
+
+    def __init__(self, x, a, b):
+        self.x, self.params, self.batch = x, (a.weight, a.bias, b.weight, b.bias), x.shape[0]
+        self.ops = None
+        self.taken = False
+
+    def launch_args(self) -> tuple:
+        if self.ops is None:
+            self.ops = _mlp2_operands(self.x, *self.params)
+        a = _mlp2_fwd_args(*self.ops)
+        return a[:2] + a[3:]
+
+
+def mlp2_rider(x: torch.Tensor, bottom_linears, first_linear) -> Optional[Mlp2Rider]:
+    a, b = bottom_linears
+    if not FWD_RIDE_MLP2 or a.in_features > 16 or a.out_features != 64 or b.out_features != 16:
+        return None
+    if _packed_entry(first_linear.weight) is None:
+        return None
+    return Mlp2Rider(x, a, b)
 
 
 class _HeadLossFn(torch.autograd.Function):
 
     @staticmethod
-    def forward(ctx, x, Wa, ba, Wb, bb, sparse, D, W1, b1, W2, b2, w3, b3, labels):
-        xs, ha, hb, Wa_, ba_, Wb_, bb_ = _mlp2_operands(x, Wa, ba, Wb, bb)
+    def forward(ctx, x, Wa, ba, Wb, bb, sparse, D, W1, b1, W2, b2, w3, b3, labels, rider=None):
+        xs, ha, hb, Wa_, ba_, Wb_, bb_ = rider.ops if rider is not None else _mlp2_operands(x, Wa, ba, Wb, bb)
         B = sparse.shape[0]
         F = sparse.shape[1] // D
         sparse = sparse.contiguous()
@@ -738,9 +765,12 @@
         mlp2_args = _mlp2_fwd_args(xs, ha, hb, Wa_, ba_, Wb_, bb_)
         head, tail = _ia_top_fwd_args(hb, sparse, F, D, W1_, b1_, z, width, y1, pk)
         rc = _lib.TZR_ERR_UNSUPPORTED
-        if PHASE_MLP2_FWD and pk is not None and z is None:
+        if rider is None and PHASE_MLP2_FWD and pk is not None and z is None:
             rc = L.tzr_dot_interaction_top_fwd_mlp2(*mlp2_args, *head, *tail, _lib.stream_ptr(dev))
-        if rc == _lib.TZR_ERR_UNSUPPORTED:
+        if rider is not None:
+            _lib.check(L.tzr_dot_interaction_top_fwd_packed(*head, B, *tail, _lib.stream_ptr(dev)), "tzr_dot_interaction_top_fwd_packed")
+            RIDE_LAUNCHES[0] += 1
+        elif rc == _lib.TZR_ERR_UNSUPPORTED:
             _lib.check(L.tzr_mlp2_fwd(*mlp2_args, _lib.stream_ptr(dev)), "tzr_mlp2_fwd")
             _lib.check(L.tzr_dot_interaction_top_fwd_packed(*head, B, *tail, _lib.stream_ptr(dev)), "tzr_dot_interaction_top_fwd_packed")
         else:
@@ -795,9 +825,9 @@
                 dW1 = weight_grad(g1, ctx.z) if root else weight_grad(g1, ctx.z) * gl
         bottom = _mlp2_backward(xs, ha, hb, Wb_, ctx.bottom_refs, gd) if need_bottom else (None, None, None, None)
         if root:
-            return (None, *bottom, gs, None, dW1, db1, dW2, db2, dw3, scal[0:1], None)
+            return (None, *bottom, gs, None, dW1, db1, dW2, db2, dw3, scal[0:1], None, None)
         outs = torch._foreach_mul([db1, dW2, db2, dw3, scal[0:1]], gl)
-        return (None, *bottom, gs, None, dW1, *outs, None)
+        return (None, *bottom, gs, None, dW1, *outs, None, None)
 
 
 def head_phases_fit(x: torch.Tensor, bottom_linears, sparse: torch.Tensor, D: int, first_linear) -> bool:
@@ -806,9 +836,9 @@
     return x.shape[0] == sparse.shape[0] and _ia_top_fits(D, torch.float32, sparse, D, first_linear)
 
 
-def head_phases_loss(x, a, b, sparse, D, l1, l2, out_linear, labels):
+def head_phases_loss(x, a, b, sparse, D, l1, l2, out_linear, labels, rider: Optional[Mlp2Rider] = None):
     return _HeadLossFn.apply(x, a.weight, a.bias, b.weight, b.bias, sparse, D, l1.weight, l1.bias, l2.weight, l2.bias,
-                             out_linear.weight, out_linear.bias, labels)
+                             out_linear.weight, out_linear.bias, labels, rider)
 
 
 def _register_fused(opt, fuse_finish: bool) -> torch.device:
diff --git a/torcheasyrec_amd/dlrm.py b/torcheasyrec_amd/dlrm.py
--- a/torcheasyrec_amd/dlrm.py
+++ b/torcheasyrec_amd/dlrm.py
@@ -189,15 +189,35 @@
         return self.mlp(x)
 
 
-def head_loss(model, dense: torch.Tensor, sparse: torch.Tensor, labels: torch.Tensor, d: Optional[torch.Tensor] = None):
+def _head_is_phases(model, dense: torch.Tensor, sparse: torch.Tensor) -> bool:
+    if not (_FUSED_TOP_LOSS and model.final_mlp._plain and _FUSED_IA_TOP and _FUSED_MLP2 and model.arch_with_sparse
+            and sparse.shape[0] >= _FUSED_IA_TOP_MIN_B and getattr(model.dense_mlp, "_plain", False) and dense.dim() == 2
+            and (dense.is_cuda or _lib.emulated())):
+        return False
+    from .dense import head_phases_fit, top_loss_fits
+
+    bot, lin = model.dense_mlp.linears(), model.final_mlp.linears()
+    return head_phases_fit(dense, bot, sparse, model.dim, lin[0]) and top_loss_fits(dense, lin, model.output_mlp)
+
+
+def head_rider(model, dense: torch.Tensor):
+    sparse = torch.empty(dense.shape[0], model.num_sparse * model.dim, dtype=torch.float32, device="meta")
+    if not _head_is_phases(model, dense, sparse):
+        return None
+    from .dense import mlp2_rider
+
+    return mlp2_rider(dense, model.dense_mlp.linears(), model.final_mlp.linears()[0])
+
+
+def head_loss(model, dense: torch.Tensor, sparse: torch.Tensor, labels: torch.Tensor, d: Optional[torch.Tensor] = None, rider=None):
     fused = _FUSED_TOP_LOSS and model.final_mlp._plain and (sparse.is_cuda or _lib.emulated())
-    if (d is None and fused and _FUSED_IA_TOP and _FUSED_MLP2 and model.arch_with_sparse and sparse.shape[0] >= _FUSED_IA_TOP_MIN_B
-            and getattr(model.dense_mlp, "_plain", False) and dense.dim() == 2 and (dense.is_cuda or _lib.emulated())):
-        from .dense import head_phases_fit, head_phases_loss, top_loss_fits
+    if d is None and fused and _head_is_phases(model, dense, sparse):
+        from .dense import head_phases_loss
 
         bot, lin = model.dense_mlp.linears(), model.final_mlp.linears()
-        if head_phases_fit(dense, bot, sparse, model.dim, lin[0]) and top_loss_fits(sparse, lin, model.output_mlp):
-            return head_phases_loss(dense, bot[0], bot[1], sparse, model.dim, lin[0], lin[1], model.output_mlp, labels)
+        return head_phases_loss(dense, bot[0], bot[1], sparse, model.dim, lin[0], lin[1], model.output_mlp, labels, rider)
+    if rider is not None:
+        raise RuntimeError("a bottom MLP run ahead by the embedding forward, and a head that does not start from it")
     if d is None:
         d = model.dense_mlp(dense)
     if fused and _FUSED_IA_TOP and model.arch_with_sparse and sparse.shape[0] >= _FUSED_IA_TOP_MIN_B:
@@ -283,8 +303,9 @@
         return head_loss(self, dense, sparse, labels)
 
     def forward_loss(self, dense: torch.Tensor, sparse_features: KeyedJaggedTensor, labels: torch.Tensor):
-        sparse = self.ebc.forward_grouped(sparse_features)["sparse"]
-        return self.loss_from_embeddings(dense, sparse, labels)
+        rider = head_rider(self, dense) if torch.is_grad_enabled() else None
+        sparse = self.ebc.forward_grouped(sparse_features, rider=rider)["sparse"]
+        return head_loss(self, dense, sparse, labels, rider=rider if rider is not None and rider.taken else None)
 
 
 class DeepFM(nn.Module):
diff --git a/torcheasyrec_amd/embedding.py b/torcheasyrec_amd/embedding.py
--- a/torcheasyrec_amd/embedding.py
+++ b/torcheasyrec_amd/embedding.py
@@ -233,15 +233,15 @@
 
 class _PooledLookupFn(torch.autograd.Function):
     @staticmethod
-    def forward(ctx, ebc, kjt, dst_names, hook):
-        outs = ebc._launch_forward(kjt, dst_names, with_plan=True)
+    def forward(ctx, ebc, kjt, dst_names, hook, rider=None):
+        outs = ebc._launch_forward(kjt, dst_names, with_plan=True, rider=rider)
         ctx.ebc, ctx.kjt, ctx.dst_names = ebc, kjt, dst_names
         return tuple(outs)
 
     @staticmethod
     def backward(ctx, *grads):
         ctx.ebc._launch_backward(ctx.kjt, ctx.dst_names, grads)
-        return None, None, None, None
+        return None, None, None, None, None
 
 
 class EmbeddingBagCollection(nn.Module):
@@ -491,7 +491,8 @@
         geo = self._cells_for(kjt, meta)
         return None if geo is None else (geo, p)
 
-    def _launch_forward(self, kjt: KeyedJaggedTensor, dst_names: Tuple[str, ...], with_plan: bool = False) -> List[torch.Tensor]:
+    def _launch_forward(self, kjt: KeyedJaggedTensor, dst_names: Tuple[str, ...], with_plan: bool = False,
+                        rider=None) -> List[torch.Tensor]:
         layout = self._layout_for(dst_names)
         meta = self._meta(kjt.keys(), layout)
         B = kjt.stride()
@@ -509,10 +510,15 @@
             geo, p = carried
             ws = _lib.workspace(p.plan_bytes(), self._device)
             ev = self._timers.start("fwd+plan") if self._timers is not None else None
-            rc = _lib.lib().tzr_pooled_fwd_cells_plan(
-                _lib.ptr(meta.d_tables), _lib.ptr(meta.d_feats), len(self._lookups), _lib.ptr(meta.d_slots), len(meta.slots_np), dsts,
-                len(outs), _lib.ptr(p.d_tables), p.n_tables, _lib.ptr(p.d_feats), p.n_feats, p.max_dim,
-                _lib.ptr(p.values), p.n_values, p.B, geo.h_ptr, _lib.ptr(geo.d_img), _lib.ptr(ws), ws.numel(), _lib.stream_ptr(self._device))
+            args = (_lib.ptr(meta.d_tables), _lib.ptr(meta.d_feats), len(self._lookups), _lib.ptr(meta.d_slots), len(meta.slots_np), dsts,
+                    len(outs), _lib.ptr(p.d_tables), p.n_tables, _lib.ptr(p.d_feats), p.n_feats, p.max_dim,
+                    _lib.ptr(p.values), p.n_values, p.B, geo.h_ptr, _lib.ptr(geo.d_img), _lib.ptr(ws), ws.numel())
+            rc = _lib.TZR_ERR_UNSUPPORTED
+            if rider is not None and rider.batch == p.B:
+                rc = _lib.lib().tzr_pooled_fwd_cells_plan_mlp2(*args, *rider.launch_args(), _lib.stream_ptr(self._device))
+                rider.taken = rc == _lib.TZR_OK
+            if rc == _lib.TZR_ERR_UNSUPPORTED:
+                rc = _lib.lib().tzr_pooled_fwd_cells_plan(*args, _lib.stream_ptr(self._device))
             if rc != _lib.TZR_ERR_UNSUPPORTED:
                 if ev is not None:
                     ev.record()
@@ -677,7 +683,7 @@
         for fn in self._lookup_trackers:
             fn(self, segs, kjt.values(), offsets, kjt.stride(), 1 if uniform else 0)
 
-    def _run(self, kjt: KeyedJaggedTensor, dst_names: Tuple[str, ...]) -> List[torch.Tensor]:
+    def _run(self, kjt: KeyedJaggedTensor, dst_names: Tuple[str, ...], rider=None) -> List[torch.Tensor]:
         if kjt.uniform_length() is None and getattr(kjt, "_uniform_keys", None):
             view = kjt.uniform_prefix([lk.key for lk in self._lookups])
             if view is not None:
@@ -687,7 +693,7 @@
         if torch.is_grad_enabled() and self.fused_optimizer is not None and self.training:
             if self.async_plan and getattr(kjt, "_tzr_plan", None) is None:
                 self.plan_backward_async(kjt, dst_names)
-            return list(_PooledLookupFn.apply(self, kjt, dst_names, self._hook))
+            return list(_PooledLookupFn.apply(self, kjt, dst_names, self._hook, rider))
         return self._launch_forward(kjt, dst_names)
 
     def forward(self, features: KeyedJaggedTensor) -> KeyedTensor:
@@ -695,11 +701,12 @@
         keys = [lk.out_key for lk in self._lookups]
         return KeyedTensor(keys, [self._out_dim[k] for k in keys], out)
 
-    def forward_grouped(self, features: KeyedJaggedTensor, group_names: Optional[Sequence[str]] = None) -> Dict[str, torch.Tensor]:
+    def forward_grouped(self, features: KeyedJaggedTensor, group_names: Optional[Sequence[str]] = None,
+                        rider=None) -> Dict[str, torch.Tensor]:
         if self._groups is None:
             raise ValueError("EmbeddingBagCollection was built without groups")
         names = tuple(group_names) if group_names is not None else tuple(self._groups)
-        outs = self._run(features, names)
+        outs = self._run(features, names, rider)
         return dict(zip(names, outs))
 
     def bounds_check(self, features: KeyedJaggedTensor, mode: int = _lib.BOUNDS_WARNING) -> torch.Tensor:
```

After: 146.0 million samples/s, median of 6. About the same (+1.0%).
